# at-cg/PHI

Measured on AMD Instinct MI355X. Metric: read Gbases/s scored (49-hap MHC graph stand-in synMHC-49); reads resident in HBM, parsing and H2D excluded, higher is better.
Workload: dtype u64

## Files before the change

include/phi_amd.h:

```cpp
#ifndef PHI_AMD_H
#define PHI_AMD_H

#include <stddef.h>
#include <stdint.h>

#ifdef __cplusplus
extern "C" {
#endif

typedef struct phi_ctx phi_ctx;

typedef enum {
    PHI_OK = 0,
    PHI_ERR_INVALID = -1,
    PHI_ERR_NOMEM = -2,
    PHI_ERR_DEVICE = -3,
    PHI_ERR_STATE = -4,
    PHI_ERR_UNSUPPORTED = -5,
    PHI_ERR_WALK = -6,
    PHI_ERR_OVERFLOW = -7
} phi_status;

const char *phi_strerror(int status);
const char *phi_last_error(const phi_ctx *ctx);
// ... 144 lines not shown
    int64_t spectrum_size;
    int64_t filtered;
    int64_t retained;
    int64_t n_in_model;
} phi_result;

int phi_set_solve_budget(phi_ctx *ctx, int64_t max_dp_runs);

int phi_solve(phi_ctx *ctx, phi_result *out);

int phi_path_sequence(phi_ctx *ctx, char *buf, int64_t cap);

int phi_sketch(phi_ctx *ctx, const char *bases, const int64_t *seq_off, int64_t n_seq, int32_t k,
               int32_t w, uint64_t *out_hash, int64_t *out_pos, int32_t *out_seq, int64_t cap,
               int64_t *n_out);
typedef struct {
    int64_t n_entries, walk_bases;
    int64_t n_classes, class_bases, n_class_records;
    int64_t n_walk_minimizers, n_distinct_minimizers;
    double sketch_gpu_ms;
} phi_index_info;
int phi_index_stats(phi_ctx *ctx, phi_index_info *out);

typedef struct {
    int64_t n_dp_anchors, n_events;
    int32_t n_steps, n_blocks, dp_mode, max_classes;
    double mean_classes;
} phi_solve_info;
int phi_solve_stats(phi_ctx *ctx, phi_solve_info *out);

int phi_walk_minimizers(phi_ctx *ctx, int32_t walk, uint64_t *out_hash, int64_t *out_pos,
                        int64_t cap, int64_t *n_out);
int phi_walk_sharing(phi_ctx *ctx, int64_t *hist, int32_t cap, int64_t *n_distinct);

int phi_kept_anchors(phi_ctx *ctx, uint64_t *out_hash, int32_t *out_walk, int32_t *out_t0,
                     int32_t *out_t1, int64_t cap, int64_t *n_out);

int phi_host_register(phi_ctx *ctx, void *p, size_t bytes);
int phi_host_unregister(phi_ctx *ctx, void *p);

int phi_prof_enable(phi_ctx *ctx, int on);
int phi_prof_read(phi_ctx *ctx, int64_t *n_launches, double *total_ms, int64_t *total_bases);

typedef struct { const char *text; int64_t n; } phi_walk_text;
int phi_walk_text_upload(phi_ctx *ctx, const phi_walk_text *walks, int32_t n_walks);
int phi_walk_text_resolve(phi_ctx *ctx, const char *prefix, int32_t prefix_n, const int32_t *num2id, int64_t n_num, int32_t n_seg,
                          int64_t *walk_off_out, uint32_t *irregular);
int phi_walk_entries(phi_ctx *ctx, int32_t *out, int64_t cap, int64_t *n);

int phi_device_synchronize(phi_ctx *ctx);

int phi_prefix_sums(phi_ctx *ctx, int32_t kind, const void *d_in, int64_t n, void *d_out);

int phi_edit_distances(phi_ctx *ctx, const char *a, const int64_t *a_off, const char *b, const int64_t *b_off,
                       int64_t n_pairs, int64_t max_distance, int64_t *out);

int phi_edit_alignments(phi_ctx *ctx, const char *a, const int64_t *a_off, const char *b, const int64_t *b_off,
                        int64_t n_pairs, const int64_t *dist, int64_t *counts, char *cigar, const int64_t *cigar_off);


#define PHI_INFLATE_CHUNK_DEFAULT (64 << 10)
#define PHI_INFLATE_NO_FINDER 1
typedef struct {
    int64_t in_bytes;
    int64_t out_bytes;
    int64_t members;
    int64_t chunks;
    int64_t confirmed;
    int64_t redecoded;
    int64_t marker_bytes;
    double device_ms;
    char detail[192];
} phi_inflate_info;
int phi_inflate(int32_t device, const void *in, int64_t n, void *out, int64_t cap, int64_t chunk_bytes, int32_t flags,
                int64_t *out_size, phi_inflate_info *info);
int phi_inflate_alloc(int32_t device, const void *in, int64_t n, int64_t chunk_bytes, int32_t flags, void **out, int64_t *out_size,
                      phi_inflate_info *info);
void phi_inflate_free(void *p);
int phi_text_park_gzip_begin(phi_text_park *park, int64_t piece_bytes);
int phi_text_park_gzip_add(phi_text_park *park, const void *data, int64_t n);
int phi_text_park_gzip_end(phi_text_park *park, int32_t *first, int32_t *count, phi_inflate_info *info);
int phi_gzip_header(const void *data, int64_t n, int64_t pos, int64_t *deflate_start);
uint32_t phi_crc32_combine(uint32_t crc_a, uint32_t crc_b, int64_t len_b);

typedef struct {
    int64_t text_bytes;
    int64_t host_bytes;
    int64_t walk_bytes;
    int32_t n_walks;
    phi_inflate_info inflate;
} phi_gfa_gzip_info;
int phi_gfa_gzip_split(phi_ctx *ctx, const void *gz, int64_t n, int64_t chunk_bytes, char **host_text, int64_t *host_n,
                       phi_gfa_gzip_info *info);
void phi_gfa_gzip_free(char *host_text);

#define PHI_LADDER_MAX_LEVELS 16
typedef struct {
    int32_t n_levels;
    int32_t one_length;
    int64_t n_reads, n_bases;
    int64_t n_kept_reads, n_kept_bases;
    int64_t band_reads[PHI_LADDER_MAX_LEVELS], band_bases[PHI_LADDER_MAX_LEVELS];
    uint64_t threshold[PHI_LADDER_MAX_LEVELS];
    double count_gpu_ms, scan_gpu_ms, scatter_gpu_ms, copy_gpu_ms;
} phi_ladder_info;
int phi_reads_collect_begin(phi_ctx *ctx, int64_t first_ordinal);
// ... 53 lines not shown
```

phi_amd/_capi.py:

```python
import ctypes as C
import os

_HERE = os.path.dirname(os.path.abspath(__file__))
LIB_PATH = os.environ.get("PHI_AMD_LIB") or os.path.join(_HERE, "libphi_amd.so")

PHI_OK = 0
PHI_ERR_INVALID, PHI_ERR_NOMEM, PHI_ERR_DEVICE, PHI_ERR_STATE = -1, -2, -3, -4
PHI_ERR_UNSUPPORTED, PHI_ERR_WALK, PHI_ERR_OVERFLOW = -5, -6, -7
PHI_FLAG_QCLP, PHI_FLAG_MIXED = 1, 2
PHI_COMM_ID_BYTES = 128

SYMBOLS = [
    "phi_strerror", "phi_last_error", "phi_ctx_create", "phi_ctx_destroy", "phi_set_stream", "phi_set_params",
    "phi_set_graph", "phi_add_reads", "phi_add_reads_device", "phi_reset_reads", "phi_reads_stats", "phi_hits_buffer", "phi_read_table",
    "phi_spectrum_export", "phi_spectrum_import", "phi_spectrum_set_size", "phi_solve", "phi_path_sequence",
    "phi_sketch", "phi_walk_minimizers", "phi_walk_sharing", "phi_kept_anchors", "phi_prof_enable", "phi_prof_read",
    "phi_host_register", "phi_host_unregister", "phi_set_solve_budget", "phi_device_synchronize", "phi_walk_text_upload", "phi_walk_text_resolve", "phi_walk_entries",
    "phi_index_stats", "phi_solve_stats", "phi_comm_unique_id", "phi_comm_init", "phi_comm_info", "phi_comm_allreduce_hits", "phi_comm_exchange", "phi_comm_destroy",
    "phi_reads_text_begin", "phi_add_reads_text", "phi_reads_text_end", "phi_reads_text_detach_carry", "phi_reads_text_last_batch",
    "phi_text_park_create", "phi_text_park_pin", "phi_text_park_add", "phi_text_park_add_async", "phi_text_park_wait", "phi_text_park_bytes", "phi_text_park_fetch", "phi_text_park_release", "phi_text_park_destroy",
    "phi_add_reads_text_parked",
    "phi_peers_create", "phi_peers_join", "phi_peers_allreduce_hits", "phi_peers_exchange", "phi_peers_destroy",
    "phi_ipc_unique_id", "phi_ipc_init", "phi_ipc_info", "phi_ipc_allreduce_hits", "phi_ipc_flush", "phi_ipc_exchange", "phi_ipc_check", "phi_ipc_destroy",
    "phi_edit_distances", "phi_edit_alignments",
    "phi_inflate", "phi_inflate_alloc", "phi_inflate_free", "phi_gzip_header", "phi_crc32_combine",
    "phi_text_park_gzip_begin", "phi_text_park_gzip_add", "phi_text_park_gzip_end",
    "phi_gfa_gzip_split", "phi_gfa_gzip_free",
    "phi_set_graph_chopped", "phi_chop_origin", "phi_chop_stats",
    "phi_vcf_genotypes", "phi_vcf_walks", "phi_vcf_stats",
    "phi_reads_collect_begin", "phi_reads_collect_end", "phi_reads_collect_release", "phi_ladder_plan", "phi_ladder_advance", "phi_ladder_band",
    "phi_set_graph_panel", "phi_panel_origin", "phi_panel_walks", "phi_panel_stats", "phi_panel_release",
    "phi_scout_graph", "phi_scout_scores", "phi_scout_choose", "phi_reads_collect_score", "phi_vcf_walks_wide",
    "phi_prefix_sums",
    "phi_reads_bam_begin", "phi_add_reads_bam", "phi_add_reads_bam_parked", "phi_reads_bam_end", "phi_reads_bam_last_batch",
    "phi_calls_path", "phi_calls_walk", "phi_calls_stats",
]
PHI_PANEL_RETAIN = 1
PHI_PANEL_KEEP_READS = 2
PHI_SCOUT_MAX_WALKS = 65535
PHI_LADDER_MAX_LEVELS = 16
PHI_INFLATE_NO_FINDER = 1
PHI_INFLATE_CHUNK_DEFAULT = 64 << 10


class PhiIndexInfo(C.Structure):
    _fields_ = [(n, C.c_int64) for n in ("n_entries", "walk_bases", "n_classes", "class_bases", "n_class_records",
                                         "n_walk_minimizers", "n_distinct_minimizers")] + [("sketch_gpu_ms", C.c_double)]


class PhiSolveInfo(C.Structure):
    _fields_ = [("n_dp_anchors", C.c_int64), ("n_events", C.c_int64), ("n_steps", C.c_int32), ("n_blocks", C.c_int32),
                ("dp_mode", C.c_int32), ("max_classes", C.c_int32), ("mean_classes", C.c_double)]


class PhiChopInfo(C.Structure):
    _fields_ = [("n_vtx_in", C.c_int64), ("n_vtx_out", C.c_int64), ("n_entries_in", C.c_int64), ("n_entries_out", C.c_int64),
                ("max_len", C.c_int32), ("expand_gpu_ms", C.c_double)]


class PhiPanelInfo(C.Structure):
    _fields_ = [("n_walks_in", C.c_int32), ("n_walks_out", C.c_int32), ("n_vtx_in", C.c_int64), ("n_vtx_out", C.c_int64),
                ("n_edges_in", C.c_int64), ("n_edges_out", C.c_int64), ("n_entries_in", C.c_int64), ("n_entries_out", C.c_int64),
                ("mark_gpu_ms", C.c_double), ("scan_gpu_ms", C.c_double), ("remap_gpu_ms", C.c_double),
                ("reduce_host_s", C.c_double), ("kahn_host_s", C.c_double)]


class PhiScoutInfo(C.Structure):
    _fields_ = [("n_blocks", C.c_int32), ("n_walks", C.c_int32), ("n_classes_flagged", C.c_int64), ("n_nonzero", C.c_int64),
                ("record_gpu_ms", C.c_double), ("class_gpu_ms", C.c_double), ("entry_gpu_ms", C.c_double), ("walk_sum_gpu_ms", C.c_double)]


class PhiVcfInfo(C.Structure):
    _fields_ = [("text_bytes", C.c_int64), ("n_records", C.c_int64), ("n_samples", C.c_int32), ("n_flagged", C.c_int64),
                ("n_units", C.c_int64), ("n_entries", C.c_int64), ("genotype_gpu_ms", C.c_double), ("walks_gpu_ms", C.c_double)]


class PhiLadderInfo(C.Structure):
    _fields_ = [("n_levels", C.c_int32), ("one_length", C.c_int32), ("n_reads", C.c_int64), ("n_bases", C.c_int64),
                ("n_kept_reads", C.c_int64), ("n_kept_bases", C.c_int64),
                ("band_reads", C.c_int64 * PHI_LADDER_MAX_LEVELS), ("band_bases", C.c_int64 * PHI_LADDER_MAX_LEVELS),
                ("threshold", C.c_uint64 * PHI_LADDER_MAX_LEVELS),
                ("count_gpu_ms", C.c_double), ("scan_gpu_ms", C.c_double), ("scatter_gpu_ms", C.c_double), ("copy_gpu_ms", C.c_double)]


class PhiBamInfo(C.Structure):
    _fields_ = [(n, C.c_int64) for n in ("n_records", "n_kept", "n_secondary_supplementary", "n_empty", "n_reverse", "n_bases", "header_bytes",
# ... 114 lines not shown
    L.phi_spectrum_set_size.argtypes = [vp, i64]
    L.phi_solve.argtypes = [vp, C.POINTER(PhiResult)]
    L.phi_set_solve_budget.argtypes = [vp, i64]
    L.phi_index_stats.argtypes = [vp, C.POINTER(PhiIndexInfo)]
    L.phi_solve_stats.argtypes = [vp, C.POINTER(PhiSolveInfo)]
    L.phi_comm_unique_id.argtypes = [vp, C.c_size_t]
    L.phi_comm_init.argtypes = [vp, vp, i32, i32]
    L.phi_comm_info.argtypes = [vp, C.POINTER(i32), C.POINTER(i32)]
    L.phi_comm_allreduce_hits.argtypes = [vp]
    L.phi_comm_exchange.argtypes = [vp]
    L.phi_comm_destroy.argtypes = [vp]
    L.phi_peers_create.argtypes = [i32, C.POINTER(vp)]
    L.phi_peers_join.argtypes = [vp, vp, i32]
    L.phi_peers_allreduce_hits.argtypes = [vp]
    L.phi_peers_exchange.argtypes = [vp]
    L.phi_peers_destroy.argtypes = [vp]
    L.phi_ipc_unique_id.argtypes = [vp, C.c_size_t]
    L.phi_ipc_init.argtypes = [vp, C.c_char_p, i32, i32]
    L.phi_ipc_info.argtypes = [vp, C.POINTER(i32), C.POINTER(i32)]
    L.phi_ipc_allreduce_hits.argtypes = [vp]
    L.phi_ipc_exchange.argtypes = [vp]
    L.phi_ipc_flush.argtypes = [vp]
    L.phi_ipc_check.argtypes = [vp]
    L.phi_ipc_destroy.argtypes = [vp]
    L.phi_path_sequence.argtypes = [vp, vp, i64]
    L.phi_sketch.argtypes = [vp, vp, vp, i64, i32, i32, vp, vp, vp, i64, C.POINTER(i64)]
    L.phi_walk_minimizers.argtypes = [vp, i32, vp, vp, i64, C.POINTER(i64)]
    L.phi_walk_sharing.argtypes = [vp, vp, i32, C.POINTER(i64)]
    L.phi_kept_anchors.argtypes = [vp, vp, vp, vp, vp, i64, C.POINTER(i64)]
    L.phi_prof_enable.argtypes = [vp, C.c_int]
    L.phi_host_register.argtypes = [vp, vp, C.c_size_t]
    L.phi_host_unregister.argtypes = [vp, vp]
    L.phi_prof_read.argtypes = [vp, C.POINTER(i64), C.POINTER(C.c_double), C.POINTER(i64)]
    L.phi_device_synchronize.argtypes = [vp]
    L.phi_prefix_sums.argtypes = [vp, i32, vp, i64, vp]
    L.phi_walk_text_upload.argtypes = [vp, vp, i32]
    L.phi_walk_text_resolve.argtypes = [vp, C.c_char_p, i32, vp, i64, i32, vp, C.POINTER(C.c_uint32)]
    L.phi_walk_entries.argtypes = [vp, vp, i64, C.POINTER(i64)]
    L.phi_edit_distances.argtypes = [vp, vp, vp, vp, vp, i64, i64, vp]
    L.phi_edit_alignments.argtypes = [vp, vp, vp, vp, vp, i64, vp, vp, vp, vp]
    L.phi_inflate.argtypes = [i32, vp, i64, vp, i64, i64, i32, C.POINTER(i64), C.POINTER(PhiInflateInfo)]
    L.phi_inflate_alloc.argtypes = [i32, vp, i64, i64, i32, C.POINTER(vp), C.POINTER(i64), C.POINTER(PhiInflateInfo)]
    L.phi_inflate_free.argtypes = [vp]
    L.phi_inflate_free.restype = None
    L.phi_text_park_gzip_begin.argtypes = [vp, i64]
    L.phi_text_park_gzip_add.argtypes = [vp, vp, i64]
    L.phi_text_park_gzip_end.argtypes = [vp, C.POINTER(i32), C.POINTER(i32), C.POINTER(PhiInflateInfo)]
    L.phi_gzip_header.argtypes = [vp, i64, i64, C.POINTER(i64)]
    L.phi_crc32_combine.argtypes = [C.c_uint32, C.c_uint32, i64]
    L.phi_crc32_combine.restype = C.c_uint32
    L.phi_gfa_gzip_split.argtypes = [vp, vp, i64, i64, C.POINTER(vp), C.POINTER(i64), C.POINTER(PhiGfaGzipInfo)]
    L.phi_gfa_gzip_free.argtypes = [vp]
    L.phi_gfa_gzip_free.restype = None
    for name in SYMBOLS:
        f = getattr(L, name)
        if f.restype is C.c_int and name not in ("phi_strerror", "phi_last_error", "phi_ctx_destroy", "phi_crc32_combine", "phi_inflate_free", "phi_gfa_gzip_free"):
            f.restype = C.c_int
    _lib = L
    return L
```

phi_amd/context.py:

```python
import ctypes as C
from typing import NamedTuple

import numpy as np

from . import _capi


class PhiError(RuntimeError):
    def __init__(self, status, detail):
        self.status = status
        self.detail = detail
        super().__init__(f"{_capi.load().phi_strerror(status).decode()} ({status}): {detail}")


def _ptr(a):
    return a.ctypes.data if a is not None and a.size else None


class Alignments(NamedTuple):
    distance: np.ndarray
    counts: np.ndarray
    cigar: list
    identity: np.ndarray

# ... 587 lines not shown
        self._chk(self._L.phi_walk_minimizers(self._h, walk, None, None, 0, C.byref(n)))
        h = np.zeros(n.value, np.uint64)
        p = np.zeros(n.value, np.int64)
        if n.value:
            self._chk(self._L.phi_walk_minimizers(self._h, walk, _ptr(h), _ptr(p), n.value, C.byref(n)))
        return h, p

    def walk_sharing(self, n_walks):
        hist = np.zeros(n_walks + 1, np.int64)
        n = C.c_int64()
        self._chk(self._L.phi_walk_sharing(self._h, _ptr(hist), n_walks + 1, C.byref(n)))
        return hist, n.value

    def kept_anchors(self):
        n = C.c_int64()
        self._chk(self._L.phi_kept_anchors(self._h, None, None, None, None, 0, C.byref(n)))
        h = np.zeros(n.value, np.uint64)
        wk = np.zeros(n.value, np.int32)
        t0 = np.zeros(n.value, np.int32)
        t1 = np.zeros(n.value, np.int32)
        if n.value:
            self._chk(self._L.phi_kept_anchors(self._h, _ptr(h), _ptr(wk), _ptr(t0), _ptr(t1), n.value, C.byref(n)))
        return h, wk, t0, t1

    def walk_entries(self):
        n = C.c_int64()
        self._chk(self._L.phi_walk_entries(self._h, None, 0, C.byref(n)))
        out = np.zeros(n.value, np.int32)
        if n.value:
            self._chk(self._L.phi_walk_entries(self._h, _ptr(out), n.value, C.byref(n)))
        return out

    def gfa_gzip_split(self, data, chunk_bytes=0):
        p, n, info = self._gfa_gzip_split_raw(data, chunk_bytes)
        try:
            return C.string_at(p, n) if n else b"", info
        finally:
            self._L.phi_gfa_gzip_free(p)

    def _gfa_gzip_split_raw(self, data, chunk_bytes=0):
        buf = np.frombuffer(data, np.uint8) if not isinstance(data, np.ndarray) else data
        p, n, info = C.c_void_p(), C.c_int64(), _capi.PhiGfaGzipInfo()
        self._chk(self._L.phi_gfa_gzip_split(self._h, _ptr(buf), len(buf), chunk_bytes, C.byref(p), C.byref(n), C.byref(info)))
        d = {k: getattr(info, k) for k in ("text_bytes", "host_bytes", "walk_bytes", "n_walks")}
        d["inflate"] = _info(info.inflate)
        return p, n.value, d

    def device_synchronize(self):
        self._chk(self._L.phi_device_synchronize(self._h))

    def prefix_sums(self, kind, d_in, n, d_out):
        self._chk(self._L.phi_prefix_sums(self._h, kind, C.c_void_p(d_in), n, C.c_void_p(d_out)))

    def prof_enable(self, on=True):
        self._chk(self._L.phi_prof_enable(self._h, int(on)))

    def prof_read(self):
        n, ms, b = C.c_int64(), C.c_double(), C.c_int64()
        self._chk(self._L.phi_prof_read(self._h, C.byref(n), C.byref(ms), C.byref(b)))
        return n.value, ms.value, b.value


def _parse_reads_tail(text):
    lines = [ln.rstrip(b"\r") for ln in text.split(b"\n")]
    while lines and not lines[-1]:
        lines.pop()
    if not lines:
        return []
    if lines[0][:1] == b"@":
        if len(lines) % 4:
            raise ValueError("the reads text ends inside a FASTQ record")
        return lines[1::4]
    if lines[0][:1] != b">":
        raise ValueError("the reads text is neither FASTA nor FASTQ")
    seqs = []
    for ln in lines:
        if ln[:1] == b">":
            seqs.append([])
        else:
            seqs[-1].append(ln)
    return [b"".join(s) for s in seqs]


def _info(info):
    return {n: getattr(info, n) for n, _ in _capi.PhiInflateInfo._fields_ if n != "detail"}


def inflate(data, device=0, chunk_bytes=0, finder=True, as_array=False):
    L = _capi.load()
    buf = np.frombuffer(data, np.uint8) if not isinstance(data, np.ndarray) else data
    flags = 0 if finder else _capi.PHI_INFLATE_NO_FINDER
    p, size, info = C.c_void_p(), C.c_int64(), _capi.PhiInflateInfo()
    rc = L.phi_inflate_alloc(device, _ptr(buf), len(buf), chunk_bytes, flags, C.byref(p), C.byref(size), C.byref(info))
    if rc:
        raise PhiError(rc, info.detail.decode())
    try:
        out = np.empty(size.value, np.uint8)
        if size.value:
            C.memmove(out.ctypes.data, p, size.value)
    finally:
        L.phi_inflate_free(p)
    return (out if as_array else out.tobytes()), _info(info)


def gzip_header(data, pos=0):
    L = _capi.load()
# ... 70 lines not shown
```

phi_amd/csrc/anchors.hip:

```cpp
#include <hip/hip_runtime.h>
#include "phi_dev.h"
#include "phi_kernels.h"
#include "phi_wave.h"

static inline unsigned grid_for(int64_t n, int tpb)
{
    int64_t nb = (n + tpb - 1) / tpb;
    if (nb > 256 * 16) nb = 256 * 16;
    if (nb < 1) nb = 1;
    return (unsigned)nb;
}

#define GRID_STRIDE(i, n) \
    for (int64_t i = (int64_t)blockIdx.x * blockDim.x + threadIdx.x; i < (n); i += (int64_t)gridDim.x * blockDim.x)

__global__ void __launch_bounds__(256) phi_walk_edges_kernel(const int32_t *__restrict__ walk_vtx, const int64_t *__restrict__ walk_off,
                                                             int32_t n_walks, int64_t n_entries, int32_t n_vtx, const int64_t *__restrict__ adj_off,
                                                             const int32_t *__restrict__ adj, const int64_t *__restrict__ seq_off,
                                                             const int32_t *__restrict__ topo_rank, uint8_t *__restrict__ e_out,
                                                             int32_t *__restrict__ cnt_edge, unsigned long long *__restrict__ st_mask,
                                                             int32_t nw64, int32_t *__restrict__ err)
{
    GRID_STRIDE(e, n_entries) {
        int32_t lo = 0, hi = n_walks;
// ... 111 lines not shown
    if (a1 - a0 != b1 - b0) return false;
    for (uint32_t d = 0; d <= a1 - a0; d++)
        if (A.walk_vtx[a0 + d] != A.walk_vtx[b0 + d]) return false;
    return true;
}

__global__ void __launch_bounds__(256) phi_group_insert_kernel(PhiFilterArgs A, int64_t n_matched)
{
    GRID_STRIDE(j, n_matched) {
        const int32_t r = A.m_rec[j];
        const uint64_t key = group_key(A.rec_slot[r], A.walk_vtx, A.rec_e0[r], A.rec_e1[r], A.seed);
        uint64_t gs = key & A.g_mask;
        int probes = 0;
        for (;;) {
            const unsigned long long prev = atomicCAS((unsigned long long *)&A.g_keys[gs], PHI_EMPTY_KEY, key);
            if (prev == PHI_EMPTY_KEY || prev == key) break;
            gs = (gs + 1) & A.g_mask;
            if (++probes > PHI_MAX_PROBE) { atomicOr(A.err, PHI_KERR_TABLE_FULL); break; }
        }
        atomicMin((uint32_t *)&A.g_rep[gs], (uint32_t)r);
        A.m_group[j] = (int32_t)gs;
    }
}

__global__ void __launch_bounds__(256) phi_group_count_kernel(PhiFilterArgs A, int64_t n_matched)
{
    GRID_STRIDE(j, n_matched) {
        const int32_t r = A.m_rec[j];
        const int32_t gs = A.m_group[j];
        if (!same_group(A, r, A.g_rep[gs])) { atomicOr(A.err, PHI_KERR_FP_COLLISION); continue; }
        atomicAdd(&A.g_cnt[gs], (uint32_t)A.cls_mult[A.rec_cls[r]]);
    }
}

__global__ void __launch_bounds__(256) phi_group_max_kernel(PhiFilterArgs A, int64_t n_matched)
{
    GRID_STRIDE(j, n_matched) {
        const int32_t r = A.m_rec[j];
        const uint32_t id = A.u_uid[A.rec_slot[r]];
        atomicMax(&A.slot_maxcnt[id], A.g_cnt[A.m_group[j]]);
        if (A.rec_e1[r] > A.rec_e0[r]) A.slot_multi[id] = 1;
    }
}

__global__ void __launch_bounds__(256) phi_slot_count_kernel(PhiFilterArgs A, int64_t n_ids)
{
    int n_filtered = 0, n_model = 0;
    GRID_STRIDE(s, n_ids) {
        const uint32_t c = A.slot_maxcnt[s];
        if (c == 0) continue;
        if ((float)c >= A.limit) n_filtered++;
        else if (A.slot_multi[s]) n_model++;
    }
    n_filtered = phi_wave_sum(n_filtered);
    n_model = phi_wave_sum(n_model);
    if ((threadIdx.x & 63) == 0) {
        if (n_filtered) atomicAdd(&A.counters[0], (unsigned long long)n_filtered);
        if (n_model) atomicAdd(&A.counters[1], (unsigned long long)n_model);
    }
}

__global__ void __launch_bounds__(256) phi_kept_flags_kernel(PhiFilterArgs A, int64_t n_matched,
                                                             uint8_t *__restrict__ kept, uint8_t *__restrict__ dp)
{
    GRID_STRIDE(j, n_matched) {
        const int32_t r = A.m_rec[j];
        const bool keep = !((float)A.slot_maxcnt[A.u_uid[A.rec_slot[r]]] >= A.limit);
        kept[j] = keep;
        dp[j] = keep && A.rec_e1[r] > A.rec_e0[r];
    }
}

void phi_launch_group_insert(hipStream_t st, const PhiFilterArgs &A, int64_t n)
{
    if (n > 0) hipLaunchKernelGGL(phi_group_insert_kernel, dim3(grid_for(n, 256)), dim3(256), 0, st, A, n);
}
void phi_launch_group_count(hipStream_t st, const PhiFilterArgs &A, int64_t n)
{
    if (n > 0) hipLaunchKernelGGL(phi_group_count_kernel, dim3(grid_for(n, 256)), dim3(256), 0, st, A, n);
}
void phi_launch_group_max(hipStream_t st, const PhiFilterArgs &A, int64_t n)
{
    if (n > 0) hipLaunchKernelGGL(phi_group_max_kernel, dim3(grid_for(n, 256)), dim3(256), 0, st, A, n);
}
void phi_launch_slot_count(hipStream_t st, const PhiFilterArgs &A, int64_t u_cap)
{
    if (u_cap > 0) hipLaunchKernelGGL(phi_slot_count_kernel, dim3(grid_for(u_cap, 256)), dim3(256), 0, st, A, u_cap);
}
void phi_launch_kept_flags(hipStream_t st, const PhiFilterArgs &A, int64_t n, uint8_t *kept, uint8_t *dp)
{
    if (n > 0) hipLaunchKernelGGL(phi_kept_flags_kernel, dim3(grid_for(n, 256)), dim3(256), 0, st, A, n, kept, dp);
}

__global__ void phi_gather_i32_kernel(const int32_t *__restrict__ src, const uint32_t *__restrict__ idx, int64_t n,
                                      int32_t *__restrict__ out)
{
    GRID_STRIDE(j, n) out[j] = src[idx[j]];
}
void phi_launch_gather_i32(hipStream_t st, const int32_t *src, const uint32_t *idx, int64_t n, int32_t *out)
{
    if (n > 0) hipLaunchKernelGGL(phi_gather_i32_kernel, dim3(grid_for(n, 256)), dim3(256), 0, st, src, idx, n, out);
}

__global__ void phi_gather_u64_kernel(const uint64_t *__restrict__ src, const int32_t *__restrict__ idx, int64_t n,
                                      uint64_t *__restrict__ out)
{
    GRID_STRIDE(j, n) out[j] = src[idx[j]];
}
void phi_launch_gather_u64(hipStream_t st, const uint64_t *src, const int32_t *idx, int64_t n, uint64_t *out)
{
    if (n > 0) hipLaunchKernelGGL(phi_gather_u64_kernel, dim3(grid_for(n, 256)), dim3(256), 0, st, src, idx, n, out);
}

__global__ void phi_entry_csr_kernel(const phi_ent_t *__restrict__ a_e1, int64_t n_a, int64_t n_entries,
                                     int64_t *__restrict__ g_off)
{
    GRID_STRIDE(j, n_a + 1) {
        const int64_t lo = j == 0 ? 0 : (int64_t)a_e1[j - 1] + 1;
        const int64_t hi = j == n_a ? n_entries : (int64_t)a_e1[j];
        for (int64_t e = lo; e <= hi; e++) g_off[e] = j;
    }
}
void phi_launch_entry_csr(hipStream_t st, const phi_ent_t *a_e1, int64_t n_a, int64_t n_entries, int64_t *g_off)
{
    hipLaunchKernelGGL(phi_entry_csr_kernel, dim3(grid_for(n_a + 1, 256)), dim3(256), 0, st, a_e1, n_a, n_entries,
                       g_off);
}

__global__ void phi_warm_anchors_kernel() {}
void phi_warm_anchors(hipStream_t st) { hipLaunchKernelGGL(phi_warm_anchors_kernel, dim3(1), dim3(64), 0, st); }
```

phi_amd/csrc/dp_events.hip:

```cpp
#include <hip/hip_runtime.h>
#include <type_traits>
#include "phi_kernels.h"

#define NEG (-(1 << 28))
#define NEGK (-(1 << 30))
#define CHK PHI_DP_CHUNK
#define RING PHI_DP_RING
enum { DP_SEQ = 0, DP_ROW = 1, DP_PATH = 2 };

__global__ void __launch_bounds__(256) phi_event_flags_kernel(const int32_t *__restrict__ walk_vtx, int64_t n_entries,
                                                              const int32_t *__restrict__ cvtx, uint8_t *__restrict__ flags)
{
    for (int64_t e = (int64_t)blockIdx.x * blockDim.x + threadIdx.x; e < n_entries; e += (int64_t)gridDim.x * blockDim.x)
        flags[e] = cvtx[walk_vtx[e]] >= 0;
}

__global__ void phi_event_off_kernel(const phi_ent_t *__restrict__ ev_e, int64_t n_ev, const int64_t *__restrict__ walk_off,
                                     int32_t n_walks, int64_t *__restrict__ ev_off)
{
    const int h = blockIdx.x * blockDim.x + threadIdx.x;
    if (h > n_walks) return;
    const int64_t key = walk_off[h];
    int64_t lo = 0, hi = n_ev;
    while (lo < hi) {
// ... 491 lines not shown
            }
        }
        int32_t wl = min(ve, vb + D);
        int32_t vprev = vb;
        __syncthreads();
        for (int p = 0;; p++) {
            const int32_t vi = has_walk ? s_vi[p & 1][h] : 0;
            if (MODE != DP_ROW) {
#pragma unroll
                for (int n = 0; n < P / NPW; n++) {
                    const int32_t x = vprev + pw + n * NPW;
                    if (x < vi) {
                        const int4 r = s_res[x & (D - 1)][h];
                        A.dmax[(phi_ent_t)r.z] = r.x; A.bstart[(phi_ent_t)r.z] = r.y;
                    }
                }
                if (pw == 0 && p > 0 && h < P) {
                    const int32_t r = (p - 1) * P + h;
                    if (r < n_steps) {
                        const int32_t k = k0 + r;
                        reinterpret_cast<int4 *>(A.tops)[k] = s_top[k & (RINGT - 1)];
                        const int2 en = s_ent[r & (2 * P - 1)];
                        A.ent_src[k] = en.x; A.ent_h[k] = en.y;
                    }
                }
            }
            if (p == n_per) break;
            const int32_t hi = min(ve, vi + D);
            uint4 t0[P / NPW], t1[P / NPW], t2[P / NPW];
#pragma unroll
            for (int n = 0; n < P / NPW; n++) {
                const int64_t xc = (ve > v0) ? min(wl + pw + n * NPW, ve - 1) : 0;
                t0[n] = evg[xc * 3 + 0]; t1[n] = evg[xc * 3 + 1]; t2[n] = evg[xc * 3 + 2];
            }
#pragma unroll
            for (int n = 0; n < P / NPW; n++) {
                const int32_t x = wl + pw + n * NPW;
                if (x < hi) { s_ev[x & (D - 1)][0][h] = t0[n]; s_ev[x & (D - 1)][1][h] = t1[n]; s_ev[x & (D - 1)][2][h] = t2[n]; }
            }
            wl = max(wl, min(hi, wl + P));
            if (p % PER_CHUNK == 0 && (p / PER_CHUNK + 1) * CK < n_steps) stage(p / PER_CHUNK + 1);
            vprev = vi;
            __syncthreads();
        }
        return;
    }

    int32_t vi = vb;
    s_vi[0][h] = vi;
    __syncthreads();
    uint4 cA = make_uint4(0xFFFFFFFFu, 0, 0, 0);
    if (vi < ve) cA = s_ev[vi & (D - 1)][0][h];
    int32_t qh = 0, qn = 0, hs = 0, hE = 0, tk = 0;
    int32_t M = NEGK, sL = MODE == DP_SEQ ? 0 : -1, Emax = NEG;
    if (MODE == DP_ROW && h == row_j) M = 0;
    if (MODE == DP_PATH && has_walk) M = A.blk_S[(int64_t)sb * A.lane_stride + h];
    const bool starts_on = MODE != DP_ROW || start_row;
    int32_t endbest = NEG;
    int32_t Kn = NEGK;
    int4 ra = s_rec[0][0], rb = s_rec[0][1];
    int4 lastq = make_int4(NEG, NEG, 0, 0);
    int32_t lastk = -1;

    auto eval_entry = [&](const int4 xa, const int4 xb, int32_t k, int32_t &E, int32_t &Eh, int32_t &Esrc) {
        E = NEG; Eh = -1; Esrc = -1;
        const int32_t flags = xa.x;
        const int n_in = (flags >> 8) & 0xFF;
        auto consider = [&](const int4 q, int32_t oj, int32_t src) {
            const int32_t t1h = (q.z & 0x3FF) - 1, t1n = ((q.z >> 10) & 0x3FF) - 1, t2h = ((q.z >> 20) & 0x3FF) - 1;
            const bool cont = t1n == oj;
            const int32_t val = cont ? q.y : q.x, hh = cont ? t2h : t1h;
            if (hh < 0) return;
            if (val > E || (val == E && (hh < Eh || (hh == Eh && src < Esrc)))) { E = val; Eh = hh; Esrc = src; }
        };
        const uint32_t b0 = (uint32_t)xa.z >> 8, b1 = (uint32_t)xa.w >> 8, b2 = (uint32_t)xb.x >> 8;
        if (n_in == 1 && b0 < RINGT) {
            const int32_t src = k - (int32_t)b0;
            const int4 q = src == lastk ? lastq : s_top[src & (RINGT - 1)];
            const int32_t t1h = (q.z & 0x3FF) - 1, t1n = ((q.z >> 10) & 0x3FF) - 1, t2h = ((q.z >> 20) & 0x3FF) - 1;
            const bool cont = t1n == (xa.z & 0xFF);
            const int32_t hh = cont ? t2h : t1h;
            if (hh >= 0) { E = cont ? q.y : q.x; Eh = hh; Esrc = k - (int32_t)b0; }
        } else if (n_in <= 3 && (b0 | b1 | b2) < RINGT) {
            const int4 q0 = s_top[(k - b0) & (RINGT - 1)];
            const int4 q1 = s_top[(k - b1) & (RINGT - 1)];
            const int4 q2 = s_top[(k - b2) & (RINGT - 1)];
            consider(q0, xa.z & 0xFF, k - (int32_t)b0);
            if (n_in > 1) consider(q1, xa.w & 0xFF, k - (int32_t)b1);
            if (n_in > 2) consider(q2, xb.x & 0xFF, k - (int32_t)b2);
        } else {
            for (int j = 0; j < n_in; j++) {
                const int32_t pk = j == 0 ? xa.z : j == 1 ? xa.w : j == 2 ? xb.x : A.k_in_packed[xa.y + j - 3];
                const int32_t back = (int32_t)((uint32_t)pk >> 8);
                const int32_t src = k - back;
                const int4 q = (back < RINGT || MODE == DP_ROW) ? s_top[src & (RINGT - 1)] : reinterpret_cast<const int4 *>(A.tops)[src];
                consider(q, pk & 0xFF, src);
            }
        }
        if (Eh >= 0) E -= A.cost;
        if (h == 0) s_ent[(k - k0) & (2 * P - 1)] = make_int2(Esrc, Eh);
    };

    for (int p = 0; p < n_per; p++) {
        const int32_t r_end = min(n_steps, (p + 1) * P);
        if (vi < ve) cA = s_ev[vi & (D - 1)][0][h];
        for (int32_t r = p * P; r < r_end;) {
            const int32_t k = k0 + r;
            const int4 na = s_rec[(r + 1) & (2 * CK - 1)][0], nb = s_rec[(r + 1) & (2 * CK - 1)][1];
            const int4 n2a = s_rec[(r + 2) & (2 * CK - 1)][0], n2b = s_rec[(r + 2) & (2 * CK - 1)][1];
            const bool pair = (ra.x & PHI_DP_PAIR) && r + 1 < r_end;
            const int32_t stepk = (int32_t)(cA.x & 0x7FFFFFFFu);
            const bool second = pair && stepk == k + 1;
            const bool active = stepk == k || second;
            const int32_t flags = second ? na.x : ra.x;

            int32_t E = NEG, Eh = -1, Esrc = -1;
            if (ra.x & PHI_DP_NEED_ENTRY) eval_entry(ra, rb, k, E, Eh, Esrc);
            if (pair && (na.x & PHI_DP_NEED_ENTRY)) {
                int32_t E1, Eh1, Esrc1;
                eval_entry(na, nb, k + 1, E1, Eh1, Esrc1);
                if (second) { E = E1; Eh = Eh1; Esrc = Esrc1; }
            } else if (second) { E = NEG; Eh = -1; }

            int32_t dmax = NEG;
            int32_t oidx = 255;
            if (active) {
                const int sl = (int)(vi & (D - 1));
                const phi_ent_t e = cA.y;
                const bool ovf = (cA.x >> 31) != 0;
                const int32_t t = (int32_t)(e - eb);
                const int32_t End = (int32_t)cA.z, SB = (int32_t)cA.w;
                const uint8_t *gb = reinterpret_cast<const uint8_t *>(&s_ev[sl][1][h]);
                oidx = gb[15 + 1024];
                while (qn > 0 && t - hs >= 31) {
                    const int32_t key = qn == 1 ? tk : s_qK[qh & (QD - 1)][h];
                    if (key > M) { M = key; sL = hs; }
                    qh++; qn--;
                    if (qn > 0) { hs = s_qs[qh & (QD - 1)][h]; hE = s_qE[qh & (QD - 1)][h]; }
                }
                int32_t newE = NEG;
                if (t == 0) { newE = starts_on ? 0 : NEG; qn = 0; M = NEGK; Emax = NEG; }
                else if ((flags & PHI_DP_NEED_ENTRY) && Eh >= 0) newE = E;
                if (newE > Emax) {
                    Emax = newE;
                    const int32_t key = newE - SB;
                    while (qn > 0 && tk < key) {
                        qn--;
                        if (qn > 0) tk = s_qK[(qh + qn - 1) & (QD - 1)][h];
                    }
                    if (QD < 32 && qn == QD) { atomicOr(A.err, PHI_KERR_DP_QUEUE); qn--; }
                    const int slq = (qh + qn) & (QD - 1);
                    s_qs[slq][h] = t; s_qE[slq][h] = newE; s_qK[slq][h] = key;
                    if (qn == 0) { hs = t; hE = newE; }
                    tk = key;
                    qn++;
                    if (MODE == DP_ROW && key > Kn) Kn = key;
                }
                int32_t bs = 0;
                if ((flags & PHI_DP_NEED_TOPS) || e == e_last) {
                    int32_t best = M > NEGK / 2 ? M + End : NEG;
                    bs = sL;
                    for (int32_t j = 0; j < qn; j++) {
                        const int32_t s = j == 0 ? hs : s_qs[(qh + j) & (QD - 1)][h];
                        const int32_t Es = j == 0 ? hE : s_qE[(qh + j) & (QD - 1)][h];
                        const int a = t - s;
                        const int32_t inside = !ovf ? (int32_t)gb[(a & 15) + (a >> 4) * 1024] : ev_count_inside(A, (int64_t)eb + s, e);
                        const int32_t val = Es + inside;
                        if (val > best) { best = val; bs = s; }
                    }
                    if (best > NEG / 2) dmax = best; else bs = 0;
                    if (MODE == DP_ROW && e == e_last) endbest = max(endbest, dmax);
                }
                s_res[sl][h] = make_int4(dmax, bs, (int32_t)e, 0);
                vi++;
                cA = make_uint4(0xFFFFFFFFu, 0, 0, 0);
                if (vi < ve) cA = s_ev[vi & (D - 1)][0][h];
            }

            if (!pair && (ra.x & PHI_DP_NEED_TOPS)) {
                const bool leaving = active && oidx != 255 && dmax > NEG / 2;
                int32_t t1v = NEG, t1h = -1, t1n = -1, t2v = NEG, t2h = -1;
                if (__ballot(leaving && oidx > 1) == 0ull) {
                    const bool on0 = leaving && oidx == 0, on1 = leaving && oidx == 1;
                    unsigned long long K0, K1;
                    ev_wave_max2_key(on0 ? ev_key(dmax, h) : 0ull, on1 ? ev_key(dmax, h) : 0ull, K0, K1);
                    const bool first0 = K0 >= K1;
                    const unsigned long long Kf = first0 ? K0 : K1, Ks = first0 ? K1 : K0;
                    t1v = Kf ? (int32_t)(uint32_t)(Kf >> 8) + NEG : NEG;
                    t1h = Kf ? 255 - (int32_t)(Kf & 255) : -1;
                    t1n = Kf ? (first0 ? 0 : 1) : -1;
                    t2v = Ks ? (int32_t)(uint32_t)(Ks >> 8) + NEG : NEG;
                    t2h = Ks ? 255 - (int32_t)(Ks & 255) : -1;
                } else {
                    const int32_t m1 = ev_wave_max_i32(leaving ? dmax : NEG);
                    if (m1 > NEG / 2) {
                        const int l1 = __ffsll((long long)__ballot(leaving && dmax == m1)) - 1;
                        t1v = m1; t1h = l1;
                        t1n = __builtin_amdgcn_readlane(oidx, l1);
                        const bool other = leaving && oidx != t1n;
                        const int32_t m2 = ev_wave_max_i32(other ? dmax : NEG);
                        if (m2 > NEG / 2) { t2v = m2; t2h = __ffsll((long long)__ballot(other && dmax == m2)) - 1; }
                    }
                }
// ... 318 lines not shown
                if (d > NEGK / 2 && d - dx > best) best = d - dx;
                if (with_starts[u]) { const int32_t r = s_start[p][lx]; if (r > NEGK / 2 && r - dx > best) best = r - dx; }
            }
            S[u] = best > NEGK / 2 ? best : NEGK;
        }
    };
    if (x < 64) {
#pragma unroll
        for (int u = 0; u < U; u++) { s_b1[b_lo & 1][u][x] = NONE; s_b2[b_lo & 1][u][x] = NONE; s_n1[b_lo & 1][u][x] = 0; }
    }
    using I0 = std::integral_constant<int, 0>; using I1 = std::integral_constant<int, 1>;
    using I2 = std::integral_constant<int, 2>; using I3 = std::integral_constant<int, 3>;
    issue(I0{}, min(b_lo, nb - 1));
    issue(I1{}, min(b_lo + 1, nb - 1));
    issue(I2{}, min(b_lo + 2, nb - 1));
    issue(I3{}, min(b_lo + 3, nb - 1));
    __syncthreads();
    int32_t b = b_lo;
    for (; b + DEPTH <= nb; b += DEPTH) {
        step(I0{}, b);
        step(I1{}, b + 1);
        step(I2{}, b + 2);
        step(I3{}, b + 3);
    }
    if (b < nb) step(I0{}, b);
    if (b + 1 < nb) step(I1{}, b + 1);
    if (b + 2 < nb) step(I2{}, b + 2);
    if (MODE == 1 && has_walk) {
#pragma unroll
        for (int u = 0; u < U; u++)
            if (unit0 + u <= G.n_walks) seg_row[((int64_t)seg * (G.n_walks + 1) + unit0 + u) * LS + x] = S[u];
    }
}

__global__ void __launch_bounds__(256) phi_seg_chain_kernel(int32_t n_seg, int32_t n_walks, int32_t LS, const int32_t *__restrict__ seg_row,
                                                            int32_t *__restrict__ seg_S)
{
    __shared__ int32_t s_S[256];
    const int x = threadIdx.x;
    int32_t S = NEGK;
    for (int32_t g = 0; g < n_seg; g++) {
        seg_S[(int64_t)g * LS + x] = S;
        s_S[x] = S;
        __syncthreads();
        const int32_t *R = seg_row + (int64_t)g * (n_walks + 1) * LS + x;
        int32_t best = R[(int64_t)n_walks * LS];
#pragma unroll 8
        for (int32_t u = 0; u < n_walks; u++) best = max(best, s_S[u] + R[(int64_t)u * LS]);
        S = best > NEGK / 2 ? best : NEGK;
        __syncthreads();
    }
}

__global__ void __launch_bounds__(256) phi_blk_check_kernel(const int32_t *__restrict__ keys, const int32_t *__restrict__ S, int32_t n_blk,
                                                            int32_t LS, int32_t n_walks, int32_t *__restrict__ bad)
{
    const int64_t n = (int64_t)(n_blk - 1) * LS;
    for (int64_t i = (int64_t)blockIdx.x * blockDim.x + threadIdx.x; i < n; i += (int64_t)gridDim.x * blockDim.x) {
        const int32_t h = (int32_t)(i % LS);
        if (h >= n_walks) continue;
        const int32_t got = keys[i], want = S[i + LS];
        if (got != want && !(got <= NEGK / 2 && want <= NEGK / 2)) { atomicAdd(&bad[0], 1); atomicMin(&bad[1], (int32_t)(i / LS)); }
    }
}

__global__ void __launch_bounds__(256) phi_carry_resolve_kernel(const int32_t *__restrict__ carry, int32_t LS, int32_t b_from, int32_t h,
                                                                int32_t *__restrict__ out)
{
    __shared__ int32_t s_best;
    for (int32_t hi = b_from - 1; hi >= 0; hi -= 256) {
        if (threadIdx.x == 0) s_best = -1;
        __syncthreads();
        const int32_t b = hi - (int32_t)threadIdx.x;
        const int32_t v = b >= 0 ? carry[(int64_t)b * LS + h] : -1;
        if (v >= 0) atomicMax(&s_best, b);
        __syncthreads();
        const int32_t bb = s_best;
        if (bb >= 0) {
            if (b == bb) { out[0] = bb; out[1] = v; }
            return;
        }
        __syncthreads();
    }
    if (threadIdx.x == 0) { out[0] = -1; out[1] = -1; }
}

void phi_launch_blk_classes(hipStream_t st, const PhiBlkClassArgs &G)
{
    if (G.n_blk > 0) hipLaunchKernelGGL(phi_blk_classes_kernel, dim3((unsigned)G.n_blk), dim3(256), 0, st, G);
}
void phi_launch_blk_chain(hipStream_t st, const PhiBlkClassArgs &G, const int32_t *rows, const int32_t *rownew, const int32_t *rowdiag, int32_t *blk_S)
{
    hipLaunchKernelGGL(phi_blk_chain_kernel<0>, dim3(1), dim3(256), 0, st, G, rows, rownew, rowdiag, blk_S, nullptr, nullptr, nullptr);
}
void phi_launch_blk_chain_segments(hipStream_t st, const PhiBlkClassArgs &G, const int32_t *rows, const int32_t *rownew, const int32_t *rowdiag, int32_t *blk_S,
                                   int32_t n_seg, const int32_t *d_seg_lo, int32_t *seg_row, int32_t *seg_S)
{
    const int units = getenv("PHI_DP_CHAIN_UNITS") ? atoi(getenv("PHI_DP_CHAIN_UNITS")) : 3;
    const unsigned nu = (unsigned)(G.n_walks + 1);
    if (units >= 4) hipLaunchKernelGGL((phi_blk_chain_kernel<1, 4>), dim3((unsigned)n_seg * ((nu + 3) / 4)), dim3(256), 0, st, G, rows, rownew, rowdiag, blk_S, d_seg_lo, seg_row, seg_S);
    else if (units == 3) hipLaunchKernelGGL((phi_blk_chain_kernel<1, 3>), dim3((unsigned)n_seg * ((nu + 2) / 3)), dim3(256), 0, st, G, rows, rownew, rowdiag, blk_S, d_seg_lo, seg_row, seg_S);
    else if (units == 2) hipLaunchKernelGGL((phi_blk_chain_kernel<1, 2>), dim3((unsigned)n_seg * ((nu + 1) / 2)), dim3(256), 0, st, G, rows, rownew, rowdiag, blk_S, d_seg_lo, seg_row, seg_S);
    else hipLaunchKernelGGL((phi_blk_chain_kernel<1, 1>), dim3((unsigned)n_seg * nu), dim3(256), 0, st, G, rows, rownew, rowdiag, blk_S, d_seg_lo, seg_row, seg_S);
    hipLaunchKernelGGL(phi_seg_chain_kernel, dim3(1), dim3(256), 0, st, n_seg, G.n_walks, G.lane_stride, seg_row, seg_S);
    hipLaunchKernelGGL(phi_blk_chain_kernel<2>, dim3((unsigned)n_seg), dim3(256), 0, st, G, rows, rownew, rowdiag, blk_S, d_seg_lo, seg_row, seg_S);
}
void phi_launch_blk_check(hipStream_t st, const int32_t *keys, const int32_t *S, int32_t n_blk, int32_t LS, int32_t n_walks, int32_t *bad)
{
    int64_t nb = ((int64_t)(n_blk - 1) * LS + 255) / 256;
    if (nb < 1) nb = 1;
    if (nb > 2048) nb = 2048;
    hipLaunchKernelGGL(phi_blk_check_kernel, dim3((unsigned)nb), dim3(256), 0, st, keys, S, n_blk, LS, n_walks, bad);
}
void phi_launch_carry_resolve(hipStream_t st, const int32_t *carry, int32_t LS, int32_t b_from, int32_t h, int32_t *out)
{
    hipLaunchKernelGGL(phi_carry_resolve_kernel, dim3(1), dim3(256), 0, st, carry, LS, b_from, h, out);
}
void phi_launch_dp_block_paths_wide(hipStream_t st, const PhiDpEventArgs &A)
{
    if (A.n_walks <= 128) hipLaunchKernelGGL((phi_dp_events_kernel<2, DP_PATH>), dim3((unsigned)A.n_blk), dim3(128), 0, st, A);
    else hipLaunchKernelGGL((phi_dp_events_kernel<4, DP_PATH>), dim3((unsigned)A.n_blk), dim3(256), 0, st, A);
}

void phi_launch_dp_events(hipStream_t st, const PhiDpEventArgs &A)
{
    if (A.n_walks <= 64) hipLaunchKernelGGL((phi_dp_events_pc_kernel<2, DP_SEQ, 8, RING, 32>), dim3(1), dim3(64 * 3), 0, st, A);
    else if (A.n_walks <= 128) hipLaunchKernelGGL((phi_dp_events_kernel<2, DP_SEQ>), dim3(1), dim3(128), 0, st, A);
    else hipLaunchKernelGGL((phi_dp_events_kernel<4, DP_SEQ>), dim3(1), dim3(256), 0, st, A);
}

void phi_launch_dp_block_rows(hipStream_t st, const PhiDpEventArgs &A)
{
    const unsigned grid = (unsigned)A.n_blk * (A.lane_walk ? 65u : (unsigned)(A.n_walks + 1));
    if (A.blk_ring <= 256 && A.blk_max_len > 0 && A.blk_max_len <= 64 && !getenv("PHI_DP_ROWS_LARGE"))
        hipLaunchKernelGGL((phi_dp_events_pc_kernel<2, DP_ROW, 2, 64, 8, 32>), dim3(grid), dim3(64 * 3), 0, st, A);
    else if (A.blk_ring <= 256) hipLaunchKernelGGL((phi_dp_events_pc_kernel<2, DP_ROW, 2, 256, 8>), dim3(grid), dim3(64 * 3), 0, st, A);
    else if (A.blk_ring <= 1024) hipLaunchKernelGGL((phi_dp_events_pc_kernel<2, DP_ROW, 4, 1024, 16>), dim3(grid), dim3(64 * 3), 0, st, A);
    else hipLaunchKernelGGL((phi_dp_events_pc_kernel<2, DP_ROW, 4, 2048, 16>), dim3(grid), dim3(64 * 3), 0, st, A);
}
void phi_launch_dp_block_paths(hipStream_t st, const PhiDpEventArgs &A)
{
    if (A.blk_ring <= 256) hipLaunchKernelGGL((phi_dp_events_pc_kernel<2, DP_PATH, 4, 256, 8>), dim3((unsigned)A.n_blk), dim3(64 * 3), 0, st, A);
    else if (A.blk_ring <= 1024) hipLaunchKernelGGL((phi_dp_events_pc_kernel<2, DP_PATH, 4, 1024, 16>), dim3((unsigned)A.n_blk), dim3(64 * 3), 0, st, A);
    else hipLaunchKernelGGL((phi_dp_events_pc_kernel<2, DP_PATH, 4, 2048, 16>), dim3((unsigned)A.n_blk), dim3(64 * 3), 0, st, A);
}

__global__ void phi_warm_dp_events_kernel() {}
void phi_warm_dp_events(hipStream_t st) { hipLaunchKernelGGL(phi_warm_dp_events_kernel, dim3(1), dim3(64), 0, st); }
```

phi_amd/csrc/phi_abi.hip:

```cpp
#include <stdarg.h>
#include <stdio.h>
#include <string.h>
#include <algorithm>
#include <future>
#include "phi_ctx.h"
#include "phi_dev.h"

int phi_fail(phi_ctx *c, int code, const char *fmt, ...)
{
    char buf[512];
    va_list ap;
    va_start(ap, fmt);
    vsnprintf(buf, sizeof buf, fmt, ap);
    va_end(ap);
    if (c) {
        std::lock_guard<std::mutex> g(c->err_mu);
        c->last_error = buf;
    }
    return code;
}

int phi_hip_check(phi_ctx *c, hipError_t e, const char *what)
{
    if (e == hipSuccess) return PHI_OK;
// ... 55 lines not shown
        if (aux.valid()) (void)aux.get();
        if (c->own_stream) (void)hipStreamDestroy(c->own_stream);
        if (c->aux_stream) (void)hipStreamDestroy(c->aux_stream);
        phi_dev_free(c->d_scalars); phi_dev_free(c->d_stripes); phi_dev_free(c->alt.stripes);
        delete c;
        return code;
    };
    if (hipStreamCreateWithFlags(&c->own_stream, hipStreamNonBlocking) != hipSuccess) return bail(PHI_ERR_DEVICE);
    c->stream = c->own_stream;
    tm.lap("stream");
    if (phi_dev_ensure(c, c->d_scalars, S_N * 8) || hipMemsetAsync(c->d_scalars.p, 0, S_N * 8, c->stream) != hipSuccess ||
        phi_dev_ensure(c, c->d_stripes, 2 * STRIPE_BYTES) || hipMemsetAsync(c->d_stripes.p, 0, 2 * STRIPE_BYTES, c->stream) != hipSuccess ||
        phi_dev_ensure(c, c->alt.stripes, 2 * STRIPE_BYTES) || hipMemsetAsync(c->alt.stripes.p, 0, 2 * STRIPE_BYTES, c->stream) != hipSuccess)
        return bail(PHI_ERR_DEVICE);
    if (tm.on && getenv("PHI_TIMING_UNITS")) {
        (void)hipStreamSynchronize(c->stream); tm.lap("  scalars");
        phi_warm_sketch(c->stream); (void)hipStreamSynchronize(c->stream); tm.lap("  code object: sketch");
        phi_warm_table(c->stream); (void)hipStreamSynchronize(c->stream); tm.lap("  code object: table");
        phi_warm_anchors(c->stream); (void)hipStreamSynchronize(c->stream); tm.lap("  code object: anchors");
        phi_warm_contexts(c->stream); (void)hipStreamSynchronize(c->stream); tm.lap("  code object: contexts");
        phi_warm_dp(c->stream); (void)hipStreamSynchronize(c->stream); tm.lap("  code object: dp");
        phi_warm_dp_events(c->stream); (void)hipStreamSynchronize(c->stream); tm.lap("  code object: dp_events");
        phi_warm_solve_dev(c->stream); (void)hipStreamSynchronize(c->stream); tm.lap("  code object: solve_dev");
        phi_warm_reads_text(c->stream); (void)hipStreamSynchronize(c->stream); tm.lap("  code object: reads_text");
        phi_warm_scan(c->stream); (void)hipStreamSynchronize(c->stream); tm.lap("  code object: scan");
    }
    phi_warm_sketch(c->stream); phi_warm_table(c->stream); phi_warm_anchors(c->stream); phi_warm_contexts(c->stream);
    phi_warm_dp(c->stream); phi_warm_dp_events(c->stream); phi_warm_solve_dev(c->stream); phi_warm_reads_text(c->stream);
    phi_warm_walk_text(c->stream); phi_warm_scan(c->stream);
    if (hipStreamSynchronize(c->stream) != hipSuccess) return bail(PHI_ERR_DEVICE);
    tm.lap("scalars + code objects");
    if (aux.get() != hipSuccess) { c->aux_stream = nullptr; return bail(PHI_ERR_DEVICE); }
    c->last_error.clear();
    tm.lap("wait for the second stream + first host copies");
    *out = c;
    return PHI_OK;
}

void phi_ctx_destroy(phi_ctx *c)
{
    if (c && c->pin_future.valid()) c->pin_future.wait();
    if (c && c->dp_alloc_future.valid()) (void)c->dp_alloc_future.get();
    if (c && c->h_pin) { (void)hipSetDevice(c->device); (void)hipHostFree(c->h_pin); c->h_pin = nullptr; }
    if (c) { (void)hipSetDevice(c->device); stage_release(c); }
    if (!c) return;
    (void)phi_comm_destroy(c);
    (void)phi_ipc_destroy(c);
    (void)hipSetDevice(c->device);
    (void)hipStreamSynchronize(c->stream);
    phi_ladder_drop(c);
    DevBuf *all[] = {&c->d_anchors, &c->d_cov_all, &c->d_cov_w, &c->d_slots, &c->d_slots2, &c->d_segs, &c->d_ctr, &c->d_vmax, &c->d_lane_walk, &c->d_walk_lane, &c->d_coff, &c->d_blk_ncls, &c->d_rownew, &c->d_blk_bad, &c->d_seg_lo, &c->d_seg_row, &c->d_seg_S, &c->wtext.d_text, &c->panel.d_full, &c->scout.d_scores, &c->d_sel_off, &c->d_sel_tri, &c->d_blk_lo, &c->d_blk_ev, &c->d_blk_S, &c->d_row_out, &c->d_rowend, &c->d_blk_keys, &c->d_blk_carry, &c->d_cov, &c->d_cov2, &c->d_stepdiff, &c->alt.hit, &c->hit_extra[0], &c->hit_extra[1], &c->alt.stripes, &c->spset.d_sp_cnt, &c->rlog.d_novlog, &c->rlog.d_novcnt, &c->rlog.d_ovlist, &c->d_vlen, &c->d_ent_cls, &c->d_cls_rep, &c->d_cls_left, &c->d_cls_mult, &c->d_cls_base, &c->d_cls_rec_off, &c->d_rec_cls, &c->d_rec_rel, &c->d_u_replist, &c->d_adj_off, &c->d_adj, &c->d_topo_rank, &c->d_cnt_edge, &c->d_walk_err, &c->d_sa_cnt, &c->d_sa_cur, &c->d_sa_off, &c->d_sa_idx, &c->d_seq, &c->d_seq_off, &c->d_walk_vtx, &c->d_walk_off, &c->d_topo, &c->d_in_off,
                     &c->d_in_src, &c->d_e_out, &c->d_st_rec, &c->d_st_mask, &c->d_in_packed, &c->d_word, &c->d_wwords, &c->d_wbad,
                     &c->d_wascii, &c->d_wstarts, &c->d_rec_hash, &c->d_rec_pos, &c->d_rec_slot,
                     &c->d_rec_e0, &c->d_rec_e1, &c->d_u_keys, &c->d_u_rep, &c->d_u_uid, &c->d_rt, &c->d_kt, &c->d_in_s, &c->d_last_walk, &c->d_rowdiag, &c->d_wpre, &c->d_hit, &c->spset.d_sp_keys, &c->d_rbases,
                     &c->d_roff, &c->rlog.d_roff_made, &c->d_peer_send, &c->spset.d_export, &c->d_scalars, &c->d_stripes, &c->d_blk_cnt,
                     &c->d_blk_off, &c->d_flags, &c->d_flags2, &c->d_list, &c->d_list2, &c->d_list3, &c->d_walk_last, &c->d_m_rec, &c->d_m_group,
                     &c->d_g_keys, &c->d_g_rep, &c->d_g_cnt, &c->d_slot_maxcnt, &c->d_slot_multi, &c->d_a_e1,
                     &c->d_g_off, &c->d_g_span, &c->d_a_weight, &c->d_dmax, &c->d_bstart, &c->d_k_rec, &c->d_k_in, &c->d_cvtx, &c->d_ev_e, &c->d_ev_off, &c->d_ev,
                     &c->d_off_end, &c->d_off_start, &c->d_scan_blk, &c->d_scan_blk64, &c->d_scan_blkoff, &c->d_top,
                     &c->d_ent};
    phi_pool_flush(c->device);
    phi_pool_bypass(true);
    struct Bypass { ~Bypass() { phi_pool_bypass(false); } } bypass_guard;
    for (DevBuf *b : all) phi_dev_free(*b);
    for (auto &pr : c->prof_events) { (void)hipEventDestroy(pr.first); (void)hipEventDestroy(pr.second); }
    if (c->h_err) (void)hipHostFree(c->h_err);
    {
        auto &T = c->text;
        for (int i = 0; i < 2; i++) { phi_dev_free(T.text[i]); phi_dev_free(T.bases[i]); phi_dev_free(T.roff[i]); }
        phi_dev_free(T.tile_cnt); phi_dev_free(T.ls); phi_dev_free(T.pre); phi_dev_free(T.blk); phi_dev_free(T.sum);
        if (T.h_sum) (void)hipHostFree(T.h_sum);
        if (T.ev_copy) (void)hipEventDestroy(T.ev_copy);
    }
    phi_bam_drop(c);
    (void)hipStreamDestroy(c->own_stream);
    (void)hipStreamDestroy(c->aux_stream);
    delete c;
}

int phi_set_stream(phi_ctx *c, void *hip_stream)
{
    if (!c) return PHI_ERR_INVALID;
    HIPCHK(hipStreamSynchronize(c->stream));
    c->stream = hip_stream ? (hipStream_t)hip_stream : c->own_stream;
    return PHI_OK;
}

int phi_set_params(phi_ctx *c, int32_t k, int32_t w, float threshold, int32_t recombination, uint32_t flags)
{
    if (!c) return PHI_ERR_INVALID;
    if (c->have_graph) return phi_fail(c, PHI_ERR_STATE, "phi_set_params must precede phi_set_graph");
    if (k < 1 || k > PHI_MAX_K) return phi_fail(c, PHI_ERR_INVALID, "k=%d outside [1,%d]", k, PHI_MAX_K);
    if (w < 1 || w > PHI_MAX_W) return phi_fail(c, PHI_ERR_INVALID, "w=%d outside [1,%d]", w, PHI_MAX_W);
    if (recombination < 0) return phi_fail(c, PHI_ERR_INVALID, "recombination penalty must be >= 0");
    c->k = k; c->w = w; c->threshold = threshold; c->recombination = recombination; c->flags = flags;
    return PHI_OK;
}

}

int sketch_records(phi_ctx *c, const uint64_t *words, const unsigned long long *starts, int64_t n_bases,
                   int32_t k, int32_t w, const uint8_t *ascii_if_bad, DevBuf &out_hash, DevBuf &out_pos,
                   int64_t *n_out)
{
    *n_out = 0;
    const int64_t nb = phi_sketch_num_blocks(n_bases);
    if (nb == 0) return PHI_OK;
// ... 310 lines not shown
```

phi_amd/csrc/phi_ctx.h:

```cpp
#pragma once
#include <stdint.h>
#include <stdarg.h>
#include <stdio.h>
#include <stdlib.h>
#include <algorithm>
#include <atomic>
#include <chrono>
#include <future>
#include <mutex>
#include <string>
#include <thread>
#include <vector>
#include <hip/hip_runtime.h>
#include "../../include/phi_amd.h"
#include "phi_kernels.h"
#include "phi_host_par.h"
#include "solve_host.h"
#include "reads_host.h"

struct DevBuf {
    void *p = nullptr;
    size_t cap = 0;
    uint32_t gen = 0;
    template <class T> T *as() const { return reinterpret_cast<T *>(p); }
// ... 51 lines not shown
    struct PhiWalkText {
        bool ready = false;
        int32_t n_walks = 0;
        std::vector<int64_t> tile0, t_len;
        std::vector<int32_t> ends;
        DevBuf d_text;
    } wtext;
    bool walks_on_device = false;
    int64_t walks_on_device_n = 0;
    struct PhiChop {
        bool on = false;
        std::vector<int32_t> first;
        phi_chop_info info{};
    } chop;
    struct PhiPanel {
        bool on = false;
        std::vector<int32_t> origin;
        std::vector<int32_t> kept;
        phi_panel_info info{};
        DevBuf d_full;
        std::vector<int64_t> full_off;
    } panel;
    struct PhiScout {
        bool on = false;
        DevBuf d_scores;
        int32_t n_blocks = 0;
    } scout;
    struct PhiVcf {
        bool have = false;
        phi_vcf_info info{};
    } vcf;

    DevBuf d_seq, d_seq_off, d_walk_vtx, d_walk_off, d_topo, d_in_off, d_in_src;
    DevBuf d_e_out, d_st_rec, d_st_mask, d_in_packed;
    int dp_nw = 1;
    DevBuf d_wwords, d_wstarts, d_wbad, d_wascii;
    DevBuf d_vlen;
    DevBuf d_ent_cls;
    DevBuf d_cls_rep, d_cls_left, d_cls_mult, d_cls_base, d_cls_rec_off;
    int64_t n_cls = 0, cls_bases = 0;
    double index_gpu_ms = 0.0;
    DevBuf d_rec_hash, d_rec_pos, d_rec_cls, d_rec_rel, d_rec_slot, d_rec_e0, d_rec_e1;
    int64_t n_rec = 0;
    DevBuf d_u_keys, d_u_rep, d_u_uid, d_u_replist;
    DevBuf d_rt;
    uint64_t rt_buckets = 0, rt_mask = 0;
    DevBuf d_kt;
    uint64_t kt_buckets = 0, kt_mask = 0;
    int64_t kt_max_chunks = 0;
    void *h_stage[2] = {nullptr, nullptr};
    hipEvent_t stage_ev[2] = {nullptr, nullptr};
    DevBuf d_wpre;
    DevBuf d_rowdiag;
    DevBuf d_in_s, d_last_walk;
    int64_t n_unique = 0;
    uint64_t u_cap = 0;
    DevBuf d_hit;
    DevBuf hit_extra[PHI_HIT_RING - 2];
    int hit_n = 2, hit_idx = 0;

    struct PhiSpectrumSet {
        DevBuf d_sp_keys;
        uint64_t sp_cap = 0;
        DevBuf d_sp_cnt;
        DevBuf d_export;
        int64_t sp_set_gen = -1;
        int64_t sp_gen = 0;
        void new_generation() { sp_gen++; }
        void new_graph() { sp_set_gen = -1; }
    } spset;
    struct PhiReadLog {
        DevBuf d_novlog, d_novcnt;
        int32_t nov_shift = 6;
        int64_t log_chunks = 0, log_done = 0;
        int64_t logged_done = 0;
        int64_t last_log_chunks = 0;
        DevBuf d_ovlist;
        int64_t ov_cap = 0, ov_done = 0, ov_bound = 0;
        bool async_batches = false;
        bool next_flag_zeroed = false;
        DevBuf d_roff_made;
        void flushed() { log_chunks = log_done = 0; ov_done = 0; ov_bound = 0; }
        void new_generation() { flushed(); logged_done = 0; last_log_chunks = 0; next_flag_zeroed = false; }
    } rlog;
    int64_t reads_bases = 0, reads_count = 0;
    int64_t spectrum_override = -1;
    DevBuf d_rbases, d_roff, d_peer_send;
    DevBuf d_scalars;
    DevBuf d_stripes;
    struct PhiReadBufs {
        DevBuf hit, stripes;
        bool needs_clean = false;
    } alt;

    uint32_t *h_err = nullptr;
    struct PhiTextStream {
        bool active = false, irregular = false, started = false, detached = false;
        bool carry_stale = false;
        int mode = 0;
        int64_t fed = 0, taken = 0;
        uint32_t carry_cap = 0, chunk_cap = 0, line_cap = 0;
        DevBuf text[2], bases[2], roff[2], tile_cnt, ls, pre, blk, sum;
        int slot = 0;
        uint32_t carry_len = 0, carry_at = 0;
        std::vector<char> h_carry;
        PhiTextSummary *h_sum = nullptr;
        hipEvent_t ev_copy = nullptr;
// ... 198 lines not shown
```

phi_amd/csrc/phi_kernels.h:

```cpp
#pragma once
#include <stdint.h>
#include <hip/hip_runtime.h>
#include "phi_dp_flags.h"

#ifndef PHI_TPB
#define PHI_TPB 256

#endif
#define PHI_WCH 512
#define PHI_MAX_W 256
#define PHI_MAX_K 64
#define PHI_MAX_K_PACKED 32
#define PHI_MAX_PROBE 4096
#define PHI_RT_OVERFLOWED 1u
static inline int phi_nov_shift(int w)
{
    const int want = (3 * 2 * PHI_WCH) / (2 * (w + 1));
    int sh = 4;
    while ((1 << sh) < want && sh < 9) sh++;
    return sh;
}
#define PHI_STRIPES 256

typedef uint32_t phi_ent_t;
// ... 176 lines not shown
#define PHI_DP_RING 2048
#define PHI_SCOUT_MAX_WALKS 65535
#define PHI_DP_MAX_WALKS 1022

struct PhiDpArgs {
    int32_t n_vtx, n_walks;
    const int32_t *st_rec;
    const unsigned long long *st_mask;
    const int32_t *in_packed;
    const int64_t *walk_off;
    const uint64_t *word;
    const int64_t *g_off; const uint8_t *g_span; const uint8_t *a_weight;
    int32_t cost;
    int32_t *dmax;
    int32_t *bstart;
    int32_t *tops;
    int32_t *ent_src, *ent_h;
};
void phi_launch_dp(hipStream_t st, const PhiDpArgs &A);

#define PHI_DP_EVENT_MAX_WALKS 256
#define PHI_DP_EVENT_SAFE_WALKS 128
struct PhiDpEventArgs {
    int32_t n_k, n_walks;
    int64_t n_ev;
    const int32_t *k_rec;
    const int32_t *k_in_packed;
    const int64_t *walk_off;
    const phi_ent_t *ev_e;
    const int64_t *ev_off;
    void *ev;
    const int64_t *g_off; const uint8_t *g_span; const uint8_t *a_weight;
    int32_t cost;
    int32_t *dmax, *bstart;
    int32_t *tops;
    int32_t *ent_src, *ent_h;
    uint32_t *err;
    int32_t q_limit;
    int32_t n_blk, blk_ring;
    int32_t blk_max_len;
    int32_t lane_stride;
    const int32_t *lane_walk;
    int32_t *rownew_out;
    int32_t *rowdiag_out;
    const int32_t *blk_lo;
    const int32_t *blk_ev;
    const int32_t *blk_S;
    int32_t *row_out; int32_t *rowend_out;
    int32_t *blk_keys_out; int32_t *blk_carry;
};
void phi_launch_dp_events(hipStream_t st, const PhiDpEventArgs &A);
void phi_launch_dp_block_rows(hipStream_t st, const PhiDpEventArgs &A);
void phi_launch_dp_block_paths(hipStream_t st, const PhiDpEventArgs &A);
void phi_launch_anchor_prep(hipStream_t st, const uint32_t *tri, int64_t n, const int64_t *walk_off, int32_t n_walks, phi_ent_t *a_e1, uint8_t *a_span,
                            unsigned long long *walk_cnt, unsigned long long *out);
void phi_launch_vertex_most(hipStream_t st, const int64_t *g_off, int64_t n_entries, const int32_t *walk_vtx, int32_t *vmax);
void phi_launch_sum_i32(hipStream_t st, const int32_t *v, int64_t n, unsigned long long *out);
void phi_launch_repeat_walk(hipStream_t st, const uint32_t *tri, int64_t lo, int64_t hi, int32_t walk, int32_t *last, uint8_t *flags);
void phi_launch_weights(hipStream_t st, const uint32_t *tri, int64_t n, const uint8_t *in_s, uint8_t *wgt);
void phi_launch_path_cover(hipStream_t st, bool clear, const phi_ent_t *segs, int32_t n_seg, const int64_t *g_off, const uint32_t *tri, const uint8_t *wgt,
                           int32_t *cov_all, int32_t *cov_w, unsigned long long *ctr, uint32_t *twice, int64_t twice_cap);
void phi_launch_uncovered_slots(hipStream_t st, const uint32_t *slots, int64_t n, const int32_t *cov_all, unsigned long long *ctr, uint32_t *out);
struct PhiBlkClassArgs {
    int32_t n_blk, n_walks, lane_stride;
    const int32_t *blk_lo, *blk_ev;
    const int64_t *ev_off, *walk_off;
    const void *ev;
    int32_t *lane_walk;
    int32_t *walk_lane;
    int32_t *coff;
    int32_t *blk_ncls;
    uint32_t *err;
};
void phi_launch_blk_classes(hipStream_t st, const PhiBlkClassArgs &G);
void phi_launch_blk_chain(hipStream_t st, const PhiBlkClassArgs &G, const int32_t *rows, const int32_t *rownew, const int32_t *rowdiag, int32_t *blk_S);
void phi_launch_blk_chain_segments(hipStream_t st, const PhiBlkClassArgs &G, const int32_t *rows, const int32_t *rownew, const int32_t *rowdiag, int32_t *blk_S,
                                   int32_t n_seg, const int32_t *d_seg_lo, int32_t *seg_row, int32_t *seg_S);
void phi_launch_blk_check(hipStream_t st, const int32_t *keys, const int32_t *S, int32_t n_blk, int32_t LS, int32_t n_walks, int32_t *bad);
void phi_launch_carry_resolve(hipStream_t st, const int32_t *carry, int32_t LS, int32_t b_from, int32_t h, int32_t *out);
void phi_launch_dp_block_paths_wide(hipStream_t st, const PhiDpEventArgs &A);
void phi_launch_cut_cov(hipStream_t st, const phi_ent_t *a_e1, const uint8_t *a_span, int64_t n_a, int32_t *diff);
void phi_launch_cut_clean(hipStream_t st, const int32_t *cov_excl, int64_t n_entries, int32_t *clean);
void phi_launch_cut_clean_direct(hipStream_t st, const int64_t *g_off, const uint8_t *g_span, int64_t n_entries, int32_t *clean);
void phi_launch_cut_events(hipStream_t st, const phi_ent_t *ev_e, int64_t n_ev, const int64_t *ev_off, const int64_t *walk_off, int32_t n_walks,
                           const int32_t *walk_vtx, const int32_t *cvtx, const int32_t *ncl_excl, int32_t *stepdiff);
void phi_launch_blk_ev(hipStream_t st, const int32_t *blk_lo, int32_t n_blk, const phi_ent_t *ev_e, const int64_t *ev_off, int32_t n_walks,
                       const int32_t *walk_vtx, const int32_t *cvtx, int32_t *blk_ev);
void phi_launch_event_flags(hipStream_t st, const int32_t *walk_vtx, int64_t n_entries, const int32_t *cvtx, uint8_t *flags);
void phi_launch_event_off(hipStream_t st, const phi_ent_t *ev_e, int64_t n_ev, const int64_t *walk_off, int32_t n_walks,
                          int64_t *ev_off);
void phi_launch_dp_event_fill(hipStream_t st, const PhiDpEventArgs &A, const uint8_t *e_out, const int32_t *walk_vtx,
                              const int32_t *cvtx, const phi_ent_t *a_e1, const int32_t *wpre, int64_t n_entries);
int phi_dp_num_waves(int n_walks);
void phi_launch_dp_words(hipStream_t st, const uint8_t *e_out, const int64_t *g_off, const uint8_t *g_span,
                         const uint8_t *a_weight, int64_t n_entries, uint64_t *word);

#define PHI_TEXT_IRREGULAR_CR 1u
#define PHI_TEXT_IRREGULAR_LINES 2u
#define PHI_TEXT_IRREGULAR_LAYOUT 4u
struct PhiTextSummary {
    uint32_t n_nl;
    uint32_t n_rec;
    uint32_t err;
    uint32_t first_bad;
    uint64_t n_bases;
    uint32_t cons_end;
    uint32_t n_cons_lines;
    uint32_t not_uniform;
    uint32_t pad_;
};
struct PhiTextArgs {
// ... 40 lines not shown
```

phi_amd/csrc/phi_solve.hip:

```cpp
#include <stdio.h>
#include <string.h>
#include <algorithm>
#include <map>
#include <set>
#include <unordered_map>
#include "phi_ctx.h"
#include "phi_dev.h"

static bool have_host_walks(const phi_ctx *c) { return (int64_t)c->h_walk_vtx.size() == c->n_entries; }
static int walk_vtx_at(phi_ctx *c, int64_t e, int32_t *v)
{
    if (have_host_walks(c)) { *v = c->h_walk_vtx[(size_t)e]; return PHI_OK; }
    return phi_hip_check(c, phi_copy_sync(c, v, c->d_walk_vtx.as<int32_t>() + e, 4, hipMemcpyDeviceToHost), "walk entry D2H");
}
static int walk_vtx_range(phi_ctx *c, int64_t es, int64_t n, int32_t *dst)
{
    if (have_host_walks(c)) { memcpy(dst, c->h_walk_vtx.data() + es, (size_t)n * 4); return PHI_OK; }
    return phi_hip_check(c, phi_copy_sync(c, dst, c->d_walk_vtx.as<int32_t>() + es, (size_t)n * 4, hipMemcpyDeviceToHost), "walk entries D2H");
}
static int ensure_host_walks(phi_ctx *c)
{
    if (have_host_walks(c)) return PHI_OK;
    if (!c->h_walk_vtx.resize((size_t)c->n_entries)) return phi_fail(c, PHI_ERR_NOMEM, "host allocation failed");
    return phi_hip_check(c, phi_copy_sync(c, c->h_walk_vtx.data(), c->d_walk_vtx.p, (size_t)c->n_entries * 4, hipMemcpyDeviceToHost), "walk entries D2H");
// ... 40 lines not shown
    }
    PHICHK(phi_scan(c, d_a, ne + 1, d_b));
    phi_launch_cut_events(c->stream, c->d_ev_e.as<phi_ent_t>(), c->n_ev, c->d_ev_off.as<int64_t>(), c->d_walk_off.as<int64_t>(), c->n_walks,
                          c->d_walk_vtx.as<int32_t>(), c->d_cvtx.as<int32_t>(), d_b, c->d_stepdiff.as<int32_t>());
    std::vector<int32_t> closed((size_t)nk + 2);
    HIPCHK(hipMemcpyAsync(closed.data(), c->d_stepdiff.p, (size_t)(nk + 2) * 4, hipMemcpyDeviceToHost, c->stream));
    HIPCHK(hipStreamSynchronize(c->stream));
    for (int32_t k = 1; k <= nk + 1; k++) closed[(size_t)k] += closed[(size_t)k - 1];
    const PhiCutFlags cut_ok{c->h_k_cut_ok.data(), closed.data(), nk};
    if (getenv("PHI_TIMING")) {
        int64_t n_struct = 0, n_both = 0, longest = 0, run = 0, longest_s = 0, run_s = 0;
        for (int32_t k = 1; k < nk; k++) {
            n_struct += c->h_k_cut_ok[(size_t)k] != 0;
            if (cut_ok(k)) { n_both++; run = 0; } else longest = std::max(longest, ++run);
            if (c->h_k_cut_ok[(size_t)k]) run_s = 0; else longest_s = std::max(longest_s, ++run_s);
        }
        fprintf(stderr, "[phi timing] solve: cuts: %lld of %d steps allowed by the graph (longest closed stretch %lld), %lld also clean of anchors (longest closed stretch %lld)\n",
                (long long)n_struct, nk, (long long)longest_s, (long long)n_both, (long long)longest);
    }
    const int32_t rings_walk[] = {256, 1024, 2048}, rings_cls[] = {256, 512};
    static_assert(PHI_DP_BLOCK_MAX == 2048, "the largest ring of tops");
    const int32_t ring = phi_place_blocks(cut_ok, cls ? rings_cls : rings_walk, cls ? 2 : 3, c->blk_no_small, [&](int32_t ring_) {
        int64_t target = (int64_t)nk * (c->n_walks + 1) / 4096;
        target = std::max<int64_t>(64, std::min<int64_t>(ring_ / 2, target));
        if (cls) target = c->blk_cls_target;
        if (const char *e = getenv("PHI_DP_BLOCK_STEPS")) target = std::max(1, std::min(ring_, atoi(e)));
        return target;
    }, c->h_blk_lo);
    if (!ring) return PHI_OK;
    c->blk_ring = ring;
    c->n_blk = (int32_t)c->h_blk_lo.size() - 1;
    if (c->n_blk < 2) { c->n_blk = 0; return PHI_OK; }
    c->blk_max_len = 0;
    for (int32_t b = 0; b < c->n_blk; b++) c->blk_max_len = std::max(c->blk_max_len, c->h_blk_lo[(size_t)b + 1] - c->h_blk_lo[(size_t)b]);
    const size_t nbk = (size_t)c->n_blk, ls = (size_t)c->blk_ls, nrow = cls ? 65 : (size_t)(c->n_walks + 1);
    PHICHK(phi_dev_ensure(c, c->d_blk_lo, (nbk + 1) * 4));
    PHICHK(phi_dev_ensure(c, c->d_blk_ev, nbk * ls * 4));
    PHICHK(phi_dev_ensure(c, c->d_blk_S, nbk * ls * 4));
    PHICHK(phi_dev_ensure(c, c->d_blk_keys, nbk * ls * 4));
    PHICHK(phi_dev_ensure(c, c->d_blk_carry, nbk * ls * 4));
    {
        const uint32_t before = c->d_row_out.gen;
        PHICHK(phi_dev_ensure(c, c->d_row_out, nbk * nrow * 64 * 4));
        if (c->d_row_out.gen != before) HIPCHK(hipMemsetAsync(c->d_row_out.p, 0xC0, c->d_row_out.cap, c->stream));
    }
    PHICHK(phi_dev_ensure(c, c->d_rowend, nbk * nrow * 4));
    if (cls) {
        PHICHK(phi_dev_ensure(c, c->d_lane_walk, nbk * 64 * 4));
        PHICHK(phi_dev_ensure(c, c->d_walk_lane, nbk * ls * 4));
        PHICHK(phi_dev_ensure(c, c->d_coff, nbk * ls * 4));
        PHICHK(phi_dev_ensure(c, c->d_blk_ncls, nbk * 4));
        PHICHK(phi_dev_ensure(c, c->d_rownew, nbk * nrow * 4));
        PHICHK(phi_dev_ensure(c, c->d_rowdiag, nbk * 64 * 4));
        PHICHK(phi_dev_ensure(c, c->d_blk_bad, 64));
    }
    HIPCHK(hipMemcpyAsync(c->d_blk_lo.p, c->h_blk_lo.data(), (nbk + 1) * 4, hipMemcpyHostToDevice, c->stream));
    phi_launch_blk_ev(c->stream, c->d_blk_lo.as<int32_t>(), c->n_blk, c->d_ev_e.as<phi_ent_t>(), c->d_ev_off.as<int64_t>(), c->n_walks,
                      c->d_walk_vtx.as<int32_t>(), c->d_cvtx.as<int32_t>(), c->d_blk_ev.as<int32_t>());
    HIPCHK(hipStreamSynchronize(c->stream));
    c->dp_blocks = true;
    c->dp_cls = cls;
    if (getenv("PHI_TIMING")) fprintf(stderr, "[phi timing] solve: %d compact steps in %d blocks (rings of %d steps)%s\n", nk, c->n_blk, c->blk_ring, cls ? ", rows on class lanes" : "");
    return PHI_OK;
}

struct DpHost {
    std::vector<int32_t> ends, bstart, ent_u, ent_h;
    std::vector<int32_t> rows, rowend, S, keys, carry;
};

struct DpOut {
    int32_t n_ent;
    int32_t *dmax, *bstart, *ent_src, *ent_h;
};
static DpOut dp_out(const phi_ctx *c)
{
    const int32_t n_ent = c->dp_events ? c->n_k : c->n_vtx;
    return DpOut{n_ent, c->d_dmax.as<int32_t>(), c->d_bstart.as<int32_t>(), c->d_ent.as<int32_t>(), c->d_ent.as<int32_t>() + n_ent};
}

enum DpRetry {
    DP_DONE = 0,
    DP_HALVE_CLASS_TARGET,
    DP_NO_SMALL_BLOCKS,
    DP_GIVE_UP_BLOCKS,
    DP_DENSE
};

static int dp_event_records(phi_ctx *c, const DpOut &O, PhiDpEventArgs &A, PhiStageTimer &tr)
{
    const int64_t n_dp = c->n_dp;
    PHICHK(phi_dev_ensure(c, c->d_wpre, (size_t)(n_dp + 1) * 4));
    PHICHK(phi_scan(c, c->d_a_weight.as<uint8_t>(), n_dp, c->d_wpre.as<int32_t>()));
    A.n_k = c->n_k; A.n_walks = c->n_walks; A.n_ev = c->n_ev;
    A.k_rec = c->d_k_rec.as<int32_t>(); A.k_in_packed = c->d_k_in.as<int32_t>();
    A.walk_off = c->d_walk_off.as<int64_t>();
    A.ev_e = c->d_ev_e.as<phi_ent_t>(); A.ev_off = c->d_ev_off.as<int64_t>();
    A.ev = c->d_ev.p;
    A.g_off = c->d_g_off.as<int64_t>(); A.g_span = c->d_g_span.as<uint8_t>(); A.a_weight = c->d_a_weight.as<uint8_t>();
    A.cost = 2 * (c->recombination / 2);
    A.dmax = O.dmax; A.bstart = O.bstart;
    A.tops = c->d_top.as<int32_t>();
    A.ent_src = O.ent_src; A.ent_h = O.ent_h;
    A.err = (uint32_t *)(c->d_scalars.as<uint64_t>() + S_ERR);
    A.q_limit = getenv("PHI_DP_QLIMIT") ? atoi(getenv("PHI_DP_QLIMIT")) : 0;
    phi_launch_dp_event_fill(c->stream, A, c->d_e_out.as<uint8_t>(), c->d_walk_vtx.as<int32_t>(), c->d_cvtx.as<int32_t>(),
                             c->d_a_e1.as<phi_ent_t>(), c->d_wpre.as<int32_t>(), c->n_entries);
    if (tr.on) { (void)hipStreamSynchronize(c->stream); tr.lap("weights + per-run records"); }
    A.lane_stride = c->blk_ls;
    return PHI_OK;
}

static void dp_block_args(const phi_ctx *c, PhiDpEventArgs &A)
{
    A.n_blk = c->n_blk; A.blk_ring = c->blk_ring; A.blk_max_len = c->blk_max_len; A.blk_lo = c->d_blk_lo.as<int32_t>(); A.blk_ev = c->d_blk_ev.as<int32_t>(); A.blk_S = c->d_blk_S.as<int32_t>();
    A.row_out = c->d_row_out.as<int32_t>(); A.rowend_out = c->d_rowend.as<int32_t>();
    A.blk_keys_out = c->d_blk_keys.as<int32_t>(); A.blk_carry = c->d_blk_carry.as<int32_t>();
}

static int dp_blocks_fallback(phi_ctx *c, uint32_t kerr, uint32_t bit, DpRetry *want)
{
// ... 17 lines not shown
        PHICHK(phi_dev_ensure(c, c->d_seg_lo, ((size_t)n_seg + 1) * 4));
        PHICHK(phi_dev_ensure(c, c->d_seg_row, (size_t)n_seg * (size_t)(c->n_walks + 1) * (size_t)c->blk_ls * 4));
        PHICHK(phi_dev_ensure(c, c->d_seg_S, (size_t)n_seg * (size_t)c->blk_ls * 4));
        HIPCHK(phi_copy_sync(c, c->d_seg_lo.p, seg_lo.data(), seg_lo.size() * 4, hipMemcpyHostToDevice));
        phi_launch_blk_chain_segments(c->stream, G, A.row_out, A.rownew_out, A.rowdiag_out, c->d_blk_S.as<int32_t>(), n_seg,
                                      c->d_seg_lo.as<int32_t>(), c->d_seg_row.as<int32_t>(), c->d_seg_S.as<int32_t>());
    } else {
        phi_launch_blk_chain(c->stream, G, A.row_out, A.rownew_out, A.rowdiag_out, c->d_blk_S.as<int32_t>());
    }
    HIPCHK(hipGetLastError());
    return PHI_OK;
}

static int dp_blocks_on_class_lanes(phi_ctx *c, PhiDpEventArgs &A, PhiStageTimer &tr, DpRetry *want)
{
    const int32_t nb = c->n_blk;
    dp_block_args(c, A);
    A.rownew_out = c->d_rownew.as<int32_t>();
    A.rowdiag_out = c->d_rowdiag.as<int32_t>();
    A.lane_walk = c->d_lane_walk.as<int32_t>();
    PhiBlkClassArgs G{};
    G.n_blk = nb; G.n_walks = c->n_walks; G.lane_stride = c->blk_ls;
    G.blk_lo = A.blk_lo; G.blk_ev = A.blk_ev; G.ev_off = A.ev_off; G.walk_off = A.walk_off; G.ev = A.ev;
    G.lane_walk = c->d_lane_walk.as<int32_t>(); G.walk_lane = c->d_walk_lane.as<int32_t>(); G.coff = c->d_coff.as<int32_t>();
    G.blk_ncls = c->d_blk_ncls.as<int32_t>(); G.err = A.err;
    phi_launch_blk_classes(c->stream, G);
    uint32_t kerr = 0;
    if (tr.on) {
        HIPCHK(hipMemcpyAsync(&kerr, c->d_scalars.as<uint64_t>() + S_ERR, 4, hipMemcpyDeviceToHost, c->stream));
        HIPCHK(hipStreamSynchronize(c->stream));
        tr.lap("block classes");
        if (kerr & PHI_KERR_DP_CLASSES) return dp_blocks_fallback(c, kerr, PHI_KERR_DP_CLASSES, want);
    }
    phi_launch_dp_block_rows(c->stream, A);
    if (tr.on) { (void)hipStreamSynchronize(c->stream); tr.lap("block rows"); }
    PHICHK(dp_chain_class_rows(c, G, A));
    if (tr.on) { (void)hipStreamSynchronize(c->stream); tr.lap("block chain"); }
    A.lane_walk = nullptr;
    phi_launch_dp_block_paths_wide(c->stream, A);
    int32_t bad[2] = {0, INT32_MAX};
    HIPCHK(hipMemcpyAsync(c->d_blk_bad.p, bad, 8, hipMemcpyHostToDevice, c->stream));
    phi_launch_blk_check(c->stream, A.blk_keys_out, A.blk_S, nb, c->blk_ls, c->n_walks, c->d_blk_bad.as<int32_t>());
    HIPCHK(hipMemcpyAsync(bad, c->d_blk_bad.p, 8, hipMemcpyDeviceToHost, c->stream));
    HIPCHK(hipMemcpyAsync(&kerr, c->d_scalars.as<uint64_t>() + S_ERR, 4, hipMemcpyDeviceToHost, c->stream));
    HIPCHK(hipStreamSynchronize(c->stream));
    if (tr.on) tr.lap("block paths + check");
    if (kerr & PHI_KERR_DP_CLASSES) return dp_blocks_fallback(c, kerr, PHI_KERR_DP_CLASSES, want);
    if (kerr & PHI_KERR_DP_QUEUE) return dp_blocks_fallback(c, kerr, PHI_KERR_DP_QUEUE, want);
    if (bad[0])
        return phi_fail(c, PHI_ERR_DEVICE, "DP blocks: %d keys leaving blocks (first in block %d) differ from the chained class rows (internal error)", bad[0], bad[1]);
    return PHI_OK;
}

static int dp_blocks_on_walk_lanes(phi_ctx *c, PhiDpEventArgs &A, DpHost &H, PhiStageTimer &tr, DpRetry *want)
{
    const int32_t nb = c->n_blk, nwk = c->n_walks, nrow = nwk + 1;
    dp_block_args(c, A);
    phi_launch_dp_block_rows(c->stream, A);
    H.rows.resize((size_t)nb * nrow * 64); H.rowend.resize((size_t)nb * nrow);
    HIPCHK(hipMemcpyAsync(H.rows.data(), A.row_out, H.rows.size() * 4, hipMemcpyDeviceToHost, c->stream));
    HIPCHK(hipMemcpyAsync(H.rowend.data(), A.rowend_out, H.rowend.size() * 4, hipMemcpyDeviceToHost, c->stream));
    uint32_t kerr = 0;
    HIPCHK(hipMemcpyAsync(&kerr, c->d_scalars.as<uint64_t>() + S_ERR, 4, hipMemcpyDeviceToHost, c->stream));
    HIPCHK(hipStreamSynchronize(c->stream));
    if (tr.on) tr.lap("block rows");
    if (kerr & PHI_KERR_DP_QUEUE) return dp_blocks_fallback(c, kerr, PHI_KERR_DP_QUEUE, want);
    (void)phi_chain_blocks(H.rows.data(), H.rowend.data(), nb, nwk, H.S);
    HIPCHK(hipMemcpyAsync(c->d_blk_S.p, H.S.data(), H.S.size() * 4, hipMemcpyHostToDevice, c->stream));
    phi_launch_dp_block_paths(c->stream, A);
    H.keys.resize((size_t)nb * 64); H.carry.resize((size_t)nb * 64);
    HIPCHK(hipMemcpyAsync(H.keys.data(), A.blk_keys_out, H.keys.size() * 4, hipMemcpyDeviceToHost, c->stream));
    HIPCHK(hipMemcpyAsync(H.carry.data(), A.blk_carry, H.carry.size() * 4, hipMemcpyDeviceToHost, c->stream));
    HIPCHK(hipMemcpyAsync(&kerr, c->d_scalars.as<uint64_t>() + S_ERR, 4, hipMemcpyDeviceToHost, c->stream));
    HIPCHK(hipStreamSynchronize(c->stream));
    if (kerr & PHI_KERR_DP_QUEUE) return dp_blocks_fallback(c, kerr, PHI_KERR_DP_QUEUE, want);
    int32_t b = 0, h = 0, got = 0, wanted = 0;
    if (!phi_chain_agrees(H.S.data(), H.keys.data(), nb, nwk, &b, &h, &got, &wanted))
        return phi_fail(c, PHI_ERR_DEVICE, "DP blocks: block %d leaves key %d on walk %d, the chained matrices say %d (internal error)", b, got, h, wanted);
    return PHI_OK;
}

static int dp_dense(phi_ctx *c, const DpOut &O)
{
    PHICHK(phi_dev_ensure(c, c->d_word, (size_t)c->n_entries * 8));
    phi_launch_dp_words(c->stream, c->d_e_out.as<uint8_t>(), c->d_g_off.as<int64_t>(), c->d_g_span.as<uint8_t>(),
                        c->d_a_weight.as<uint8_t>(), c->n_entries, c->d_word.as<uint64_t>());
    PhiDpArgs A{};
    A.n_vtx = c->n_vtx; A.n_walks = c->n_walks;
    A.st_rec = c->d_st_rec.as<int32_t>(); A.st_mask = c->d_st_mask.as<unsigned long long>();
    A.in_packed = c->d_in_packed.as<int32_t>();
    A.walk_off = c->d_walk_off.as<int64_t>();
    A.word = c->d_word.as<uint64_t>();
    A.g_off = c->d_g_off.as<int64_t>(); A.g_span = c->d_g_span.as<uint8_t>(); A.a_weight = c->d_a_weight.as<uint8_t>();
    A.cost = 2 * (c->recombination / 2);
    A.dmax = O.dmax; A.bstart = O.bstart;
    A.tops = c->d_top.as<int32_t>();
    A.ent_src = O.ent_src; A.ent_h = O.ent_h;
    phi_launch_dp(c->stream, A);
    return PHI_OK;
}

static int dp_fetch_ends(phi_ctx *c, const DpOut &O, bool events, DpHost &H, PhiStageTimer &tr, DpRetry *want)
{
    H.ends.resize(c->n_walks);
    phi_launch_gather_i32(c->stream, O.dmax, c->d_walk_last.as<phi_ent_t>(), c->n_walks, c->d_list3.as<int32_t>());
    HIPCHK(hipMemcpyAsync(H.ends.data(), c->d_list3.p, (size_t)c->n_walks * 4, hipMemcpyDeviceToHost, c->stream));
    uint32_t kerr = 0;
    if (events) HIPCHK(hipMemcpyAsync(&kerr, c->d_scalars.as<uint64_t>() + S_ERR, 4, hipMemcpyDeviceToHost, c->stream));
    HIPCHK(hipStreamSynchronize(c->stream));
    tr.lap("kernel");
    if (kerr & PHI_KERR_DP_QUEUE) {
        kerr &= ~PHI_KERR_DP_QUEUE;
        HIPCHK(phi_copy_sync(c, c->d_scalars.as<uint64_t>() + S_ERR, &kerr, 4, hipMemcpyHostToDevice));
        if (!c->dp_dense_ready) return phi_fail(c, PHI_ERR_DEVICE, "event DP queue overflow without a dense fallback (internal error)");
        *want = DP_DENSE;
    }
    return PHI_OK;
}

static int dp_pick_end(phi_ctx *c, const DpHost &H, int32_t *bh_, int64_t *value)
{
    int32_t bh = -1;
    int64_t best = INT64_MIN;
    for (int32_t h = 0; h < c->n_walks; h++) {
        const int32_t d = H.ends[h];
        if (d > -(1 << 28) && d > best) { best = d; bh = h; }
    }
    if (bh < 0) return phi_fail(c, PHI_ERR_DEVICE, "DP found no s->e path (internal error)");
    *bh_ = bh;
    *value = best;
    return PHI_OK;
}

static int entry_on_vertex(phi_ctx *c, int32_t h, int32_t rank, int32_t u, int64_t *e_)
{
    int64_t lo = c->h_walk_off[h], hi = c->h_walk_off[h + 1];
    while (lo < hi) {
        const int64_t mid = (lo + hi) >> 1;
        int32_t vm = 0;
        PHICHK(walk_vtx_at(c, mid, &vm));
        if (c->h_topo_rank[vm] < rank) lo = mid + 1; else hi = mid;
    }
    *e_ = -1;
    if (lo < c->h_walk_off[h + 1]) {
        int32_t vl = 0;
        PHICHK(walk_vtx_at(c, lo, &vl));
        if (vl == u) *e_ = lo;
    }
    return PHI_OK;
}

static int dp_backtrack(phi_ctx *c, const DpOut &O, bool events, DpHost &H, int32_t h, std::vector<Seg> *segs)
{
    bool bulk = false;
    auto fetch_bulk = [&]() -> int {
        H.bstart.resize(c->n_entries); H.ent_u.resize(O.n_ent); H.ent_h.resize(O.n_ent);
        HIPCHK(hipMemcpyAsync(H.bstart.data(), O.bstart, (size_t)c->n_entries * 4, hipMemcpyDeviceToHost, c->stream));
        HIPCHK(hipMemcpyAsync(H.ent_u.data(), O.ent_src, (size_t)O.n_ent * 4, hipMemcpyDeviceToHost, c->stream));
        HIPCHK(hipMemcpyAsync(H.ent_h.data(), O.ent_h, (size_t)O.n_ent * 4, hipMemcpyDeviceToHost, c->stream));
        HIPCHK(hipStreamSynchronize(c->stream));
        bulk = true;
        return PHI_OK;
    };
// ... 7 lines not shown
        if (bs < 0 && c->dp_blocks && events) {
            int32_t vq = 0;
            PHICHK(walk_vtx_at(c, e, &vq));
            const int32_t kq = c->h_cstep[c->h_topo_rank[vq]];
            int32_t b = (int32_t)(std::upper_bound(c->h_blk_lo.begin(), c->h_blk_lo.end(), kq) - c->h_blk_lo.begin()) - 1;
            if (c->dp_cls) {
                int32_t out[2] = {-1, -1};
                phi_launch_carry_resolve(c->stream, c->d_blk_carry.as<int32_t>(), c->blk_ls, b, h, c->d_blk_bad.as<int32_t>() + 2);
                HIPCHK(hipMemcpyAsync(out, c->d_blk_bad.as<int32_t>() + 2, 8, hipMemcpyDeviceToHost, c->stream));
                HIPCHK(hipStreamSynchronize(c->stream));
                bs = out[1];
            } else {
                while (bs < 0 && --b >= 0) bs = H.carry[(size_t)b * 64 + h];
            }
            if (bs < 0) return phi_fail(c, PHI_ERR_DEVICE, "DP backtrack: a carried run has no beginning (internal error)");
        }
        const int64_t es = c->h_walk_off[h] + bs;
        if (es < c->h_walk_off[h] || es > e) return phi_fail(c, PHI_ERR_DEVICE, "DP backtrack left the walk (internal error)");
        segs->push_back(Seg{h, es, e});
        if (es == c->h_walk_off[h]) break;
        int32_t v = 0;
        PHICHK(walk_vtx_at(c, es, &v));
        const int32_t step = events ? c->h_cstep[c->h_topo_rank[v]] : c->h_topo_rank[v];
        if (step < 0) return phi_fail(c, PHI_ERR_DEVICE, "DP backtrack: run begins on a vertex without events (internal error)");
        int32_t src, h2;
        if (bulk) { src = H.ent_u[step]; h2 = H.ent_h[step]; }
        else {
            HIPCHK(phi_copy_sync(c, &src, O.ent_src + step, 4, hipMemcpyDeviceToHost));
            HIPCHK(phi_copy_sync(c, &h2, O.ent_h + step, 4, hipMemcpyDeviceToHost));
        }
        if (events && src >= 0) src = c->h_kstep[src];
        const int32_t u = src >= 0 ? c->h_topo[src] : -1;
        if (u < 0 || h2 < 0) return phi_fail(c, PHI_ERR_DEVICE, "DP backtrack hit a vertex without an entry (internal error)");
        int64_t e2 = -1;
        PHICHK(entry_on_vertex(c, h2, src, u, &e2));
        if (e2 < 0) return phi_fail(c, PHI_ERR_DEVICE, "DP backtrack: walk %d is not on vertex %d (internal error)", h2, u);
        h = h2; e = e2;
    }
    std::reverse(segs->begin(), segs->end());
    return PHI_OK;
}

static int run_dp(phi_ctx *c, const std::vector<uint8_t> *wgt, DpHost &H, int64_t *value, std::vector<Seg> *segs)
{
    for (DpRetry want = DP_DONE;;) {
        switch (want) {
        case DP_DONE: break;
        case DP_HALVE_CLASS_TARGET: c->blk_cls_target /= 2; PHICHK(dp_prepare_blocks(c, c->n_dp)); break;
        case DP_NO_SMALL_BLOCKS: c->blk_no_small = true; PHICHK(dp_prepare_blocks(c, c->n_dp)); break;
        case DP_GIVE_UP_BLOCKS: c->dp_blocks = false; c->dp_cls = false; break;
        case DP_DENSE: c->dp_events = false; break;
        }
        want = DP_DONE;
        const bool events = c->dp_events;
        const DpOut O = dp_out(c);
        PhiStageTimer tr("dp run");
        if (c->n_dp && wgt) HIPCHK(hipMemcpyAsync(c->d_a_weight.p, wgt->data(), (size_t)c->n_dp, hipMemcpyHostToDevice, c->stream));
        if (events) {
            PhiDpEventArgs A{};
            PHICHK(dp_event_records(c, O, A, tr));
            if (c->dp_blocks && c->dp_cls) PHICHK(dp_blocks_on_class_lanes(c, A, tr, &want));
            else if (c->dp_blocks) PHICHK(dp_blocks_on_walk_lanes(c, A, H, tr, &want));
            else phi_launch_dp_events(c->stream, A);
            if (want != DP_DONE) continue;
        } else {
            PHICHK(dp_dense(c, O));
        }
        HIPCHK(hipGetLastError());
        PHICHK(dp_fetch_ends(c, O, events, H, tr, &want));
        if (want != DP_DONE) continue;
        int32_t bh = -1;
        PHICHK(dp_pick_end(c, H, &bh, value));
        PHICHK(dp_backtrack(c, O, events, H, bh, segs));
        tr.lap("backtrack");
        return PHI_OK;
    }
}

template <class F> static void for_covered(const phi_ctx *c, const std::vector<Seg> &segs, F f)
{
    const PhiAnchorSpan &A = c->h_dp;
    for (const Seg &s : segs) {
        auto lo = std::lower_bound(A.begin(), A.end(), s.es, [](const PhiAnchorHost &a, int64_t e) { return (int64_t)a.e1 < e; });
        for (auto it = lo; it != A.end() && (int64_t)it->e1 <= s.ee; ++it)
            if ((int64_t)it->e0 >= s.es) f((int64_t)(it - A.begin()));
    }
}

struct Node {
    std::vector<std::pair<uint32_t, int32_t>> assign;
    int64_t ub = INT64_MAX;
};

struct Search {
    std::vector<Node> stack;
    std::vector<int64_t> open_ub;
    int64_t incumbent = INT64_MIN, global_ub = INT64_MIN, best_cov = 0;
    int n_runs = 0;
    bool exhausted = false;
};

struct Solve {
    phi_ctx *const c;
    PhiStageTimer tm{"solve"};
    int64_t n_matched = 0, n_kept_rec = 0, n_kept = 0, n_dp = 0;
    int64_t filtered = 0, in_model = 0, spectrum = 0;
    bool anchors_prepped = false;
    bool dev = false;
    PhiAnchorArrays arr;
    std::vector<int32_t> sa_off, sa_idx;
    std::vector<uint8_t> wgt;
    std::vector<int32_t> cov_all, cov_w;
    std::vector<uint32_t> touched;
    std::set<uint32_t> S0;
    DpHost H;
    Search bb;
    std::vector<Seg> best_segs;
    explicit Solve(phi_ctx *c_) : c(c_) {}
};

static int read_spectrum(Solve &S)
{
    phi_ctx *c = S.c;
    if (c->dp_alloc_future.valid()) PHICHK(c->dp_alloc_future.get());
    PHICHK(phi_sync_check(c));
    S.tm = PhiStageTimer("solve");
    uint64_t sc[S_N];
    HIPCHK(phi_copy_sync(c, sc, c->d_scalars.p, sizeof sc, hipMemcpyDeviceToHost));
    uint64_t n_distinct = 0;
    PHICHK(phi_spectrum_count(c, &n_distinct));
    S.tm.lap("read spectrum (set from the log)");
    S.spectrum = c->spectrum_override >= 0 ? c->spectrum_override : (int64_t)n_distinct;
    return PHI_OK;
}

static int match_and_compact(Solve &S)
{
    phi_ctx *c = S.c;
    const int64_t n_rec = c->n_rec;
    PHICHK(phi_dev_ensure(c, c->d_flags, (size_t)std::max<int64_t>(n_rec, 1)));
    phi_launch_match_flags(c->stream, c->d_rec_slot.as<uint32_t>(), n_rec, c->d_u_uid.as<uint32_t>(),
                           c->d_hit.as<uint8_t>(), c->d_flags.as<uint8_t>());
    PHICHK(phi_compact(c, c->d_flags.as<uint8_t>(), n_rec, c->d_m_rec, &S.n_matched));
    S.tm.lap("match + compact");
    return PHI_OK;
}

static int filter_shared_anchors(Solve &S)
{
    phi_ctx *c = S.c;
    const int64_t n_rec = c->n_rec, n_matched = S.n_matched;
    PhiFilterArgs F{};
    F.rec_slot = c->d_rec_slot.as<uint32_t>(); F.rec_e0 = c->d_rec_e0.as<phi_ent_t>(); F.rec_e1 = c->d_rec_e1.as<phi_ent_t>();
    F.walk_vtx = c->d_walk_vtx.as<int32_t>();
    F.rec_cls = c->d_rec_cls.as<int32_t>(); F.cls_mult = c->d_cls_mult.as<int32_t>();
    F.m_rec = c->d_m_rec.as<int32_t>();
    const uint64_t g_cap = pow2_at_least(std::max<uint64_t>(1024, 2 * (uint64_t)n_matched));
    PHICHK(phi_dev_ensure(c, c->d_g_keys, g_cap * 8));
    PHICHK(phi_dev_ensure(c, c->d_g_rep, g_cap * 4));
    PHICHK(phi_dev_ensure(c, c->d_g_cnt, g_cap * 4));
    PHICHK(phi_dev_ensure(c, c->d_m_group, (size_t)std::max<int64_t>(n_matched, 1) * 4));
    const size_t n_slot_ids = (size_t)std::max<int64_t>(c->n_unique, 1);
    PHICHK(phi_dev_ensure(c, c->d_slot_maxcnt, n_slot_ids * 4));
    PHICHK(phi_dev_ensure(c, c->d_slot_multi, n_slot_ids));
    F.g_keys = c->d_g_keys.as<uint64_t>(); F.g_rep = c->d_g_rep.as<int32_t>(); F.g_cnt = c->d_g_cnt.as<uint32_t>();
    F.g_mask = g_cap - 1;
    F.m_group = c->d_m_group.as<int32_t>();
    F.u_uid = c->d_u_uid.as<uint32_t>();
    F.slot_maxcnt = c->d_slot_maxcnt.as<uint32_t>(); F.slot_multi = c->d_slot_multi.as<uint8_t>();
    F.limit = c->threshold * (float)(uint32_t)c->n_walks;
    F.counters = (unsigned long long *)scalar(c, S_FILTERED);
    F.err = (uint32_t *)scalar(c, S_ERR);
    for (int attempt = 0;; attempt++) {
        F.seed = 0x243F6A8885A308D3ull + 0x9E3779B97F4A7C15ull * (uint64_t)attempt;
        phi_launch_fill_u64(c->stream, F.g_keys, (int64_t)g_cap, PHI_EMPTY_KEY);
        phi_launch_fill_u32(c->stream, (uint32_t *)F.g_rep, (int64_t)g_cap, 0xFFFFFFFFu);
        HIPCHK(hipMemsetAsync(F.g_cnt, 0, g_cap * 4, c->stream));
        phi_launch_group_insert(c->stream, F, n_matched);
        phi_launch_group_count(c->stream, F, n_matched);
        HIPCHK(hipStreamSynchronize(c->stream));
        uint32_t err = 0;
// ... 30 lines not shown
    PhiExpandArgs X{};
    X.ent_cls = c->d_ent_cls.as<int32_t>(); X.e_lo = 0; X.e_hi = c->n_entries;
    X.cls_rec_off = c->d_cls_rec_off.as<int32_t>(); X.cls_rep = c->d_cls_rep.as<phi_ent_t>();
    X.sel = c->d_flags2.as<uint8_t>(); X.sel_cnt = c->d_list3.as<int32_t>();
    X.rec_slot = c->d_rec_slot.as<uint32_t>(); X.u_uid = c->d_u_uid.as<uint32_t>();
    X.rec_e0 = c->d_rec_e0.as<phi_ent_t>(); X.rec_e1 = c->d_rec_e1.as<phi_ent_t>();
    const int64_t nb = phi_expand_num_blocks(c->n_entries);
    PHICHK(phi_dev_ensure(c, c->d_blk_cnt, (size_t)nb * 4));
    PHICHK(phi_dev_ensure(c, c->d_blk_off, (size_t)(nb + 1) * 8));
    X.block_cnt = c->d_blk_cnt.as<int32_t>(); X.block_off = c->d_blk_off.as<int64_t>();
    phi_launch_expand_count(c->stream, X);
    PHICHK(phi_scan(c, c->d_blk_cnt.as<int32_t>(), nb, c->d_blk_off.as<int64_t>()));
    int64_t n_kept = 0;
    HIPCHK(hipMemcpyAsync(&n_kept, c->d_blk_off.as<int64_t>() + nb, 8, hipMemcpyDeviceToHost, c->stream));
    HIPCHK(hipStreamSynchronize(c->stream));
    if (n_kept >= (int64_t)1 << 31) return phi_fail(c, PHI_ERR_UNSUPPORTED, "more than 2^31 anchors in the model");
    S.n_kept = n_kept;
    c->h_kept = PhiAnchorSpan{}; c->h_dp = PhiAnchorSpan{}; c->anchors_host = false;
    c->n_kept = n_kept; c->n_dp = 0;
    c->h_kept_hash.clear();
    PHICHK(phi_dev_ensure(c, c->d_anchors, (size_t)std::max<int64_t>(n_kept, 1) * 12));
    static_assert(sizeof(PhiAnchorHost) == 12, "PhiAnchorHost is the device triple");
    PHICHK(phi_dev_ensure(c, c->d_a_e1, (size_t)std::max<int64_t>(n_kept, 1) * 4));
    PHICHK(phi_dev_ensure(c, c->d_g_span, (size_t)std::max<int64_t>(n_kept, 1)));
    PHICHK(phi_dev_ensure(c, c->d_ctr, (size_t)(nw + 8) * 8));
    HIPCHK(hipMemsetAsync(c->d_ctr.p, 0, (size_t)(nw + 8) * 8, c->stream));
    if (n_kept && getenv("PHI_EXPAND_GENERIC")) {
        X.out_tri = c->d_anchors.as<uint32_t>();
        phi_launch_expand_write(c->stream, X, 1);
    } else if (n_kept) {
        PHICHK(phi_dev_ensure(c, c->d_sel_off, (size_t)(c->n_cls + 1) * 4));
        PHICHK(phi_dev_ensure(c, c->d_sel_tri, (size_t)std::max<int64_t>(n_kept_rec, 1) * 12));
        PHICHK(phi_scan(c, c->d_list3.as<int32_t>(), c->n_cls, c->d_sel_off.as<int32_t>()));
        phi_launch_class_sel_tri(c->stream, c->d_flags2.as<uint8_t>(), c->d_cls_rec_off.as<int32_t>(), c->n_cls, c->d_sel_off.as<int32_t>(), c->d_cls_rep.as<phi_ent_t>(),
                                 c->d_rec_slot.as<uint32_t>(), c->d_u_uid.as<uint32_t>(), c->d_rec_e0.as<phi_ent_t>(), c->d_rec_e1.as<phi_ent_t>(), c->d_sel_tri.as<int32_t>());
        unsigned long long *d_ctr = c->d_ctr.as<unsigned long long>();
        phi_launch_expand_tri(c->stream, c->d_ent_cls.as<int32_t>(), 0, c->n_entries, c->d_sel_off.as<int32_t>(), c->d_sel_tri.as<int32_t>(),
                              c->d_blk_off.as<int64_t>(), c->d_anchors.as<uint32_t>(), c->d_a_e1.as<phi_ent_t>(), c->d_g_span.as<uint8_t>(),
                              c->d_walk_off.as<int64_t>(), nw, d_ctr + 8, d_ctr, n_kept);
        S.anchors_prepped = true;
    }
    return PHI_OK;
}

static int check_anchors_choose_mode(Solve &S)
{
    phi_ctx *c = S.c;
    const int32_t nw = c->n_walks;
    const int64_t n_kept = S.n_kept;
    unsigned long long *d_ctr = c->d_ctr.as<unsigned long long>();
    if (!S.anchors_prepped)
        phi_launch_anchor_prep(c->stream, c->d_anchors.as<uint32_t>(), n_kept, c->d_walk_off.as<int64_t>(), nw, c->d_a_e1.as<phi_ent_t>(), c->d_g_span.as<uint8_t>(), d_ctr + 8, d_ctr);
    std::vector<unsigned long long> hc((size_t)nw + 8);
    HIPCHK(hipMemcpyAsync(hc.data(), d_ctr, hc.size() * 8, hipMemcpyDeviceToHost, c->stream));
    HIPCHK(hipStreamSynchronize(c->stream));
    if (hc[1] & 1) return phi_fail(c, PHI_ERR_DEVICE, "dp anchors not sorted by last entry (internal error)");
    if (hc[1] & 2)
        return phi_fail(c, c->k > PHI_RCAP ? PHI_ERR_UNSUPPORTED : PHI_ERR_DEVICE, "an anchor spans %d edges or more%s", PHI_RCAP,
                        c->k > PHI_RCAP ? ": with k > 32 the graph's vertices must be long enough for a k-mer to cover at most 32 of them" : " (internal error)");
    c->h_n_anchors.assign(nw, 0);
    for (int32_t h = 0; h < nw; h++) c->h_n_anchors[h] = (int64_t)hc[(size_t)h + 8];
    int64_t dev_min = (int64_t)1 << 16;
    if (const char *e = getenv("PHI_SOLVE_DEVICE")) dev_min = atoi(e) ? 0 : INT64_MAX;
    S.dev = hc[0] == 0 && n_kept >= dev_min && n_kept > 0;
    uint64_t sc[S_N];
    HIPCHK(phi_copy_sync(c, sc, c->d_scalars.p, sizeof sc, hipMemcpyDeviceToHost));
    S.filtered = (int64_t)sc[S_FILTERED]; S.in_model = (int64_t)sc[S_INMODEL];
    return PHI_OK;
}

static int anchors_to_host(Solve &S)
{
    phi_ctx *c = S.c;
    const int64_t n_kept = S.n_kept;
    if (S.dev) {
        S.tm.lap("anchor arrays (device)");
        c->n_dp = n_kept;
    } else {
        PHICHK(phi_pin_ensure(c, (size_t)std::max<int64_t>(n_kept, 1) * sizeof(PhiAnchorHost)));
        c->h_kept = PhiAnchorSpan{static_cast<PhiAnchorHost *>(c->h_pin), n_kept};
        if (n_kept) HIPCHK(hipMemcpyAsync(c->h_kept.p, c->d_anchors.p, (size_t)n_kept * 12, hipMemcpyDeviceToHost, c->stream));
        HIPCHK(hipStreamSynchronize(c->stream));
        c->anchors_host = true;
        S.tm.lap("anchors D2H");
        PhiHostError herr;
        if (phi_anchor_arrays(c->h_kept, c->h_walk_off.data(), c->n_walks, c->k, c->h_dp_own, S.arr, c->h_n_anchors, herr))
            return phi_fail(c, herr.code, "%s", herr.msg.c_str());
        c->h_dp = S.arr.dp;
        c->n_dp = (int64_t)c->h_dp.size();
    }
    S.n_dp = c->n_dp;
    if (S.tm.on) fprintf(stderr, "[phi timing] solve: class records %lld, matched %lld, kept %lld -> anchors kept %lld, dp %lld\n", (long long)c->n_rec, (long long)S.n_matched, (long long)S.n_kept_rec, (long long)n_kept, (long long)S.n_dp);
    S.tm.lap("filter (GPU) + anchors D2H");
    return PHI_OK;
}

static int anchor_entry_csr(Solve &S)
{
    phi_ctx *c = S.c;
    const int64_t n_dp = S.n_dp;
    PHICHK(phi_dev_ensure(c, c->d_a_weight, (size_t)std::max<int64_t>(n_dp, 1)));
    PHICHK(phi_dev_ensure(c, c->d_g_off, (size_t)(c->n_entries + 1) * 8));
    if (n_dp && !S.dev) {
        HIPCHK(hipMemcpyAsync(c->d_a_e1.p, S.arr.a_e1.data(), (size_t)n_dp * 4, hipMemcpyHostToDevice, c->stream));
        HIPCHK(hipMemcpyAsync(c->d_g_span.p, S.arr.a_span.data(), (size_t)n_dp, hipMemcpyHostToDevice, c->stream));
    }
    phi_launch_entry_csr(c->stream, c->d_a_e1.as<phi_ent_t>(), n_dp, c->n_entries, c->d_g_off.as<int64_t>());
    return PHI_OK;
}

static int score_bound_host(Solve &S, int64_t *bound)
{
    phi_ctx *c = S.c;
    PHICHK(ensure_host_walks(c));
    *bound = phi_score_bound(S.arr.a_e1.data(), S.n_dp, c->h_walk_vtx.data(), c->n_vtx);
    return PHI_OK;
}
static int score_bound_dev(Solve &S, int64_t *bound)
{
    phi_ctx *c = S.c;
    PHICHK(phi_dev_ensure(c, c->d_vmax, (size_t)c->n_vtx * 4));
    HIPCHK(hipMemsetAsync(c->d_vmax.p, 0, (size_t)c->n_vtx * 4, c->stream));
    HIPCHK(hipMemsetAsync(c->d_ctr.p, 0, 8, c->stream));
    phi_launch_vertex_most(c->stream, c->d_g_off.as<int64_t>(), c->n_entries, c->d_walk_vtx.as<int32_t>(), c->d_vmax.as<int32_t>());
    phi_launch_sum_i32(c->stream, c->d_vmax.as<int32_t>(), c->n_vtx, c->d_ctr.as<unsigned long long>());
    unsigned long long sum = 0;
    HIPCHK(hipMemcpyAsync(&sum, c->d_ctr.p, 8, hipMemcpyDeviceToHost, c->stream));
    HIPCHK(hipStreamSynchronize(c->stream));
    *bound = (int64_t)sum;
    return PHI_OK;
}
static int check_score_range(Solve &S)
{
    phi_ctx *c = S.c;
    if (S.n_dp < ((int64_t)1 << 27)) return PHI_OK;
    int64_t bound = 0;
    PHICHK(S.dev ? score_bound_dev(S, &bound) : score_bound_host(S, &bound));
    if (bound >= ((int64_t)1 << 27)) return phi_fail(c, PHI_ERR_UNSUPPORTED, "a path could score %lld >= 2^27 anchors", (long long)bound);
    return PHI_OK;
}

static int dp_inputs(Solve &S)
{
    phi_ctx *c = S.c;
    const int32_t nw = c->n_walks;
    HIPCHK(hipStreamSynchronize(c->stream));
    {
        std::vector<phi_ent_t> last(nw);
        for (int32_t h = 0; h < nw; h++) last[h] = (phi_ent_t)(c->h_walk_off[h + 1] - 1);
        PHICHK(phi_dev_ensure(c, c->d_walk_last, (size_t)nw * 4));
        PHICHK(phi_dev_ensure(c, c->d_list3, (size_t)nw * 4));
        HIPCHK(phi_copy_sync(c, c->d_walk_last.p, last.data(), (size_t)nw * 4, hipMemcpyHostToDevice));
    }
    PHICHK(phi_dev_ensure(c, c->d_dmax, (size_t)c->n_entries * 4));
    PHICHK(phi_dev_ensure(c, c->d_bstart, (size_t)c->n_entries * 4));
    if (c->dp_events) {
        const int64_t ne1 = c->n_entries + 1;
        PHICHK(phi_dev_ensure(c, c->d_off_end, (size_t)(ne1 + 2) * 4));
        PHICHK(phi_dev_ensure(c, c->d_off_start, (size_t)(ne1 + 2) * 4));
        PHICHK(phi_dev_ensure(c, c->d_ev, (size_t)std::max<int64_t>(c->n_ev, 1) * 48));
    }
    PHICHK(phi_dev_ensure(c, c->d_top, (size_t)c->n_vtx * 5 * 4));
    PHICHK(phi_dev_ensure(c, c->d_ent, (size_t)c->n_vtx * 2 * 4));
    c->blk_no_small = false;
    c->blk_cls_target = 16;
    PHICHK(dp_prepare_blocks(c, S.n_dp));
    S.tm.lap("DP inputs");
    return PHI_OK;
}

static int anchor_csr_dev(Solve &S, bool fetch)
{
    phi_ctx *c = S.c;
    const int64_t n_ids = c->n_unique, n_dp = S.n_dp;
    const uint32_t *tri = c->d_anchors.as<uint32_t>();
    PHICHK(phi_dev_ensure(c, c->d_sa_cnt, (size_t)(n_ids + 1) * 4));
    PHICHK(phi_dev_ensure(c, c->d_sa_cur, (size_t)(n_ids + 1) * 4));
    PHICHK(phi_dev_ensure(c, c->d_sa_off, (size_t)(n_ids + 2) * 4));
    PHICHK(phi_dev_ensure(c, c->d_sa_idx, (size_t)n_dp * 4));
    HIPCHK(hipMemsetAsync(c->d_sa_cnt.p, 0, (size_t)(n_ids + 1) * 4, c->stream));
    HIPCHK(hipMemsetAsync(c->d_sa_cur.p, 0, (size_t)(n_ids + 1) * 4, c->stream));
    phi_launch_csr_count(c->stream, tri, n_dp, n_ids, c->d_sa_cnt.as<int32_t>(), (uint32_t *)scalar(c, S_ERR));
    PHICHK(phi_scan(c, c->d_sa_cnt.as<int32_t>(), n_ids, c->d_sa_off.as<int32_t>()));
    phi_launch_csr_scatter(c->stream, tri, n_dp, n_ids, c->d_sa_off.as<int32_t>(), c->d_sa_cur.as<int32_t>(), c->d_sa_idx.as<int32_t>());
    phi_launch_csr_sort(c->stream, c->d_sa_off.as<int32_t>(), n_ids, c->d_sa_idx.as<int32_t>());
    int32_t total = 0;
    if (fetch) {
        S.sa_off.resize((size_t)n_ids + 1); S.sa_idx.resize((size_t)std::max<int64_t>(n_dp, 1));
        HIPCHK(hipMemcpyAsync(S.sa_off.data(), c->d_sa_off.p, (size_t)(n_ids + 1) * 4, hipMemcpyDeviceToHost, c->stream));
        HIPCHK(hipMemcpyAsync(S.sa_idx.data(), c->d_sa_idx.p, (size_t)n_dp * 4, hipMemcpyDeviceToHost, c->stream));
    }
    HIPCHK(hipMemcpyAsync(&total, c->d_sa_off.as<int32_t>() + n_ids, 4, hipMemcpyDeviceToHost, c->stream));
    uint32_t kerr = 0;
    HIPCHK(hipMemcpyAsync(&kerr, scalar(c, S_ERR), 4, hipMemcpyDeviceToHost, c->stream));
    HIPCHK(hipStreamSynchronize(c->stream));
    if ((kerr & PHI_KERR_CSR_ID) || total != (int32_t)n_dp)
        return phi_fail(c, PHI_ERR_DEVICE, "minimiser id out of range (internal error)");
    return PHI_OK;
}

static int anchors_of_minimisers(Solve &S)
{
    phi_ctx *c = S.c;
    const int64_t n_ids = c->n_unique, n_dp = S.n_dp;
    if (!S.dev) {
        const bool dp_is_kept = c->h_dp.p == c->h_kept.p && c->h_dp.size() == c->h_kept.size();
        if (dp_is_kept && n_dp > 0) PHICHK(anchor_csr_dev(S, true));
        else if (!phi_anchor_csr(c->h_dp, n_ids, S.sa_off, S.sa_idx)) return phi_fail(c, PHI_ERR_DEVICE, "minimiser id out of range (internal error)");
    }
    S.tm.lap("minimiser -> anchors map");
    return PHI_OK;
}

static int repeat_set_dev(Solve &S)
{
    phi_ctx *c = S.c;
    const int64_t n_ids = c->n_unique;
    PHICHK(phi_dev_ensure(c, c->d_flags, (size_t)std::max<int64_t>(n_ids, 1)));
    PHICHK(phi_dev_ensure(c, c->d_last_walk, (size_t)std::max<int64_t>(n_ids, 1) * 4));
    HIPCHK(hipMemsetAsync(c->d_flags.p, 0, (size_t)std::max<int64_t>(n_ids, 1), c->stream));
    HIPCHK(hipMemsetAsync(c->d_last_walk.p, 0xFF, (size_t)std::max<int64_t>(n_ids, 1) * 4, c->stream));
    int64_t lo = 0;
    for (int32_t h = 0; h < c->n_walks; h++) {
        phi_launch_repeat_walk(c->stream, c->d_anchors.as<uint32_t>(), lo, lo + c->h_n_anchors[h], h, c->d_last_walk.as<int32_t>(), c->d_flags.as<uint8_t>());
        lo += c->h_n_anchors[h];
    }
    if (lo != S.n_dp) return phi_fail(c, PHI_ERR_DEVICE, "anchors per walk do not add up (internal error)");
    int64_t n_rep = 0;
    PHICHK(phi_compact(c, c->d_flags.as<uint8_t>(), n_ids, c->d_list, &n_rep));
    std::vector<uint32_t> rep((size_t)n_rep);
    if (n_rep) HIPCHK(phi_copy_sync(c, rep.data(), c->d_list.p, (size_t)n_rep * 4, hipMemcpyDeviceToHost));
    S.S0.insert(rep.begin(), rep.end());
    return PHI_OK;
}
static int repeat_set(Solve &S)
{
    if (!getenv("PHI_NO_S0")) {
        if (S.dev) PHICHK(repeat_set_dev(S));
        else phi_repeat_set(S.sa_off, S.sa_idx, S.arr.dp_walk, S.c->n_unique, S.S0);
        if (S.tm.on) fprintf(stderr, "[phi timing] solve: %zu minimisers repeat along a walk\n", S.S0.size());
    }
    S.tm.lap("repeat set");
    return PHI_OK;
}

struct Span {
    const int32_t *p; int32_t n;
    const int32_t *begin() const { return p; }
    const int32_t *end() const { return p + n; }
    int32_t operator[](int32_t i) const { return p[i]; }
};
static Span anchors_of(const Solve &S, uint32_t s) { return Span{S.sa_idx.data() + S.sa_off[s], S.sa_off[s + 1] - S.sa_off[s]}; }

static std::vector<std::vector<int32_t>> clusters_of(const Solve &S, uint32_t slot)
{
    const phi_ctx *c = S.c;
    std::vector<PhiAnchorIv> iv;
    for (int32_t a : anchors_of(S, slot)) {
        const PhiAnchorHost &A = c->h_dp[a];
        iv.push_back(PhiAnchorIv{c->h_topo_rank[c->h_walk_vtx[A.e0]], c->h_topo_rank[c->h_walk_vtx[A.e1]], phi_entry_walk(c, A.e0), a});
    }
    return phi_clusters(std::move(iv));
}

static int to_host(Solve &S)
{
    phi_ctx *c = S.c;
    const int64_t n_ids = c->n_unique, n_dp = S.n_dp;
    PHICHK(ensure_host_walks(c));
    if (!S.dev) return PHI_OK;
    PhiStageTimer th("solve");
    PHICHK(phi_host_anchors(c));
    if (n_dp) PHICHK(anchor_csr_dev(S, true));
    else { S.sa_off.assign((size_t)n_ids + 1, 0); S.sa_idx.assign(1, 0); }
    S.wgt.assign((size_t)n_dp, 1);
    S.cov_all.assign((size_t)n_ids, 0); S.cov_w.assign((size_t)n_ids, 0);
    S.touched.clear();
    S.dev = false;
// ... 225 lines not shown
            for (int64_t i = 0; i <= s.ee - s.es; i++) { const int32_t v = c->h_path_vtx[(size_t)(o + i)]; hap_len += c->h_seq_off[v + 1] - c->h_seq_off[v]; }
            o += s.ee - s.es + 1;
        }
    }
    int32_t recomb = 0;
    for (size_t i = 1; i < best_segs.size(); i++) recomb += best_segs[i].h != best_segs[i - 1].h;

    phi_result &R = c->result;
    R.objective = S.bb.incumbent;
    R.upper_bound = upper_bound;
    R.optimal = upper_bound == S.bb.incumbent;
    R.n_dp_runs = S.bb.n_runs;
    R.n_covered = S.bb.best_cov;
    R.n_path = (int64_t)c->h_path_vtx.size();
    R.path_vtx = c->h_path_vtx.data();
    R.path_hap = c->h_path_hap.data();
    R.recombination_count = recomb;
    R.n_switches = (int32_t)best_segs.size() - 1;
    R.hap_len = hap_len;
    R.n_walks = c->n_walks;
    R.n_minimizers = c->h_n_minimizers.data();
    R.n_anchors = c->h_n_anchors.data();
    R.spectrum_size = S.spectrum;
    R.filtered = S.filtered;
    R.retained = S.spectrum - S.filtered;
    R.n_in_model = S.in_model;
    S.tm.lap("decode");
    c->path_segs.clear();
    for (const Seg &s : best_segs) c->path_segs.push_back({s.h, s.es, s.ee});
    c->calls.have = false;
    c->solved = true;
    return PHI_OK;
}

int phi_solve_impl(phi_ctx *c)
{
    c->solved = false;
    Solve S(c);
    PHICHK(read_spectrum(S));
    PHICHK(match_and_compact(S));
    PHICHK(filter_shared_anchors(S));
    PHICHK(expand_kept_records(S));
    PHICHK(check_anchors_choose_mode(S));
    PHICHK(anchors_to_host(S));
    PHICHK(anchor_entry_csr(S));
    PHICHK(check_score_range(S));
    PHICHK(dp_inputs(S));
    PHICHK(anchors_of_minimisers(S));
    PHICHK(repeat_set(S));
    int64_t upper_bound = 0;
    PHICHK(search(S, &upper_bound));
    return decode(S, upper_bound);
}
```

phi_amd/csrc/phi_wave.h:

```cpp
#pragma once
#include <hip/hip_runtime.h>
#include <stdint.h>
#include <type_traits>

template <class T>
using phi_shfl_t = std::conditional_t<sizeof(T) == 8, std::conditional_t<std::is_signed<T>::value, long long, unsigned long long>, T>;

template <class T>
__device__ __forceinline__ T phi_wave_incl_scan(T x)
{
    static_assert(std::is_integral<T>::value && (sizeof(T) == 4 || sizeof(T) == 8), "int, uint32_t, int64_t, uint64_t");
    const int lane = threadIdx.x & 63;
#pragma unroll
    for (int d = 1; d < 64; d <<= 1) {
        const T y = (T)__shfl_up((phi_shfl_t<T>)x, d, 64);
        if (lane >= d) x += y;
    }
    return x;
}

template <class T>
__device__ __forceinline__ T phi_wave_sum(T x)
{
    static_assert(std::is_integral<T>::value && (sizeof(T) == 4 || sizeof(T) == 8), "int, uint32_t, int64_t, uint64_t");
#pragma unroll
    for (int d = 32; d >= 1; d >>= 1) x += (T)__shfl_xor((phi_shfl_t<T>)x, d, 64);
    return x;
}

template <int NW, class T>
__device__ __forceinline__ T phi_block_excl_scan(T mine, T *s_w, T *total = nullptr)
{
    const int lane = threadIdx.x & 63, wid = threadIdx.x >> 6;
    const T inc = phi_wave_incl_scan(mine);
    if (lane == 63) s_w[wid] = inc;
    __syncthreads();
    T woff = 0;
    for (int i = 0; i < wid; i++) woff += s_w[i];
    if (total) {
        T t = 0;
#pragma unroll
        for (int i = 0; i < NW; i++) t += s_w[i];
        *total = t;
    }
    return woff + inc - mine;
}
```

phi_amd/csrc/set_graph.hip:

```cpp
#include <string.h>
#include <algorithm>
#include <future>
#include <memory>
#include "phi_ctx.h"
#include "phi_dev.h"
#include "dp_steps.h"

static int build_read_table(phi_ctx *c)
{
    uint64_t nb = pow2_at_least(std::max<uint64_t>(64, (16 * (uint64_t)c->n_unique + 2) / 3));
    if (const char *e = getenv("PHI_READ_TABLE_BUCKETS")) nb = pow2_at_least(std::max<long long>(atoll(e), 1));
    uint32_t err0 = 0;
    HIPCHK(hipMemcpyAsync(&err0, scalar(c, S_ERR), 4, hipMemcpyDeviceToHost, c->stream));
    HIPCHK(hipStreamSynchronize(c->stream));
    for (int attempt = 0;; attempt++) {
        PHICHK(phi_dev_ensure(c, c->d_rt, nb * 32));
        phi_launch_read_table(c->stream, c->d_u_keys.as<uint64_t>(), c->d_u_uid.as<uint32_t>(), (int64_t)c->u_cap,
                              c->d_rt.as<uint64_t>(), (int64_t)nb, (uint32_t *)scalar(c, S_ERR));
        uint32_t err = 0;
        HIPCHK(hipMemcpyAsync(&err, scalar(c, S_ERR), 4, hipMemcpyDeviceToHost, c->stream));
        HIPCHK(hipStreamSynchronize(c->stream));
        if ((err0 & PHI_KERR_TABLE_FULL) || !(err & PHI_KERR_TABLE_FULL)) break;
        if (attempt >= 40) return phi_fail(c, PHI_ERR_OVERFLOW, "read table overflow at %llu buckets (internal error)", (unsigned long long)nb);
        err &= ~PHI_KERR_TABLE_FULL;
// ... 203 lines not shown
    HIPCHK(hipGetLastError());
    return PHI_OK;
}

int set_graph_check_args(phi_ctx *c, int32_t n_vtx, const char *seq_concat, const int64_t *seq_off, const int64_t *adj_off,
                         const int32_t *adj, int32_t n_walks, const int64_t *walk_off, const int32_t *walk_vtx, const int32_t *topo_rank)
{
    const bool dev_walks = walk_vtx == nullptr;
    if (dev_walks && c && walk_off && n_walks > 0 && !(c->walks_on_device && c->walks_on_device_n == walk_off[n_walks] && (int32_t)(c->wtext.ends.size() / 2) == n_walks))
        return phi_fail(c, PHI_ERR_STATE, "phi_set_graph without walk_vtx: phi_walk_text_resolve must have resolved exactly these walks on this context");
    if (n_vtx <= 0 || n_walks <= 0 || !seq_concat || !seq_off || !adj_off || !walk_off || !topo_rank)
        return phi_fail(c, PHI_ERR_INVALID, "phi_set_graph: null pointer or empty graph");
    if (adj_off[n_vtx] > 0 && !adj) return phi_fail(c, PHI_ERR_INVALID, "phi_set_graph: adj is null");
    HIPCHK(hipSetDevice(c->device));
    if (c->ipc) return phi_fail(c, PHI_ERR_STATE, "phi_set_graph on a context in a group of processes: phi_ipc_destroy first (the peers have this context's hit vectors mapped)");
    c->have_graph = false;
    c->chop.on = false;
    c->panel.on = false;
    phi_scout_end(c);
    c->solved = false;
    phi_ladder_drop(c);
    return PHI_OK;
}
int set_graph_check_offsets(phi_ctx *c, int32_t n_vtx, const int64_t *seq_off, const int64_t *adj_off, int32_t n_walks, const int64_t *walk_off)
{
    if (seq_off[0] != 0 || adj_off[0] != 0 || walk_off[0] != 0) return phi_fail(c, PHI_ERR_INVALID, "offset arrays must start at 0");
    for (int32_t v = 0; v < n_vtx; v++)
        if (seq_off[v + 1] < seq_off[v] || adj_off[v + 1] < adj_off[v]) return phi_fail(c, PHI_ERR_INVALID, "offsets not monotone at vertex %d", v);
    for (int32_t h = 0; h < n_walks; h++)
        if (walk_off[h + 1] <= walk_off[h]) return phi_fail(c, PHI_ERR_INVALID, "walk %d is empty", h);
    if (walk_off[n_walks] > PHI_MAX_ENTRIES) return phi_fail(c, PHI_ERR_UNSUPPORTED, "more than 2^32 - 64 walk entries");
    return PHI_OK;
}

struct SetGraph {
    phi_ctx *const c;
    const int32_t n_vtx;
    const char *const seq_concat;
    const int64_t *const seq_off, *const adj_off;
    const int32_t *const adj;
    const int32_t n_walks;
    const int64_t *const walk_off;
    const int32_t *const walk_vtx, *const topo_rank;
    int64_t n_edges = 0, n_entries = 0;
    const bool dev_walks;
    bool want_masks = false;
    bool keep_host_walks = false;
    PhiStageTimer tm{"set_graph"};
    std::vector<int64_t> indeg;
    std::vector<int32_t> cnt_edge;
    int32_t walk_err[4] = {0, 0, 0, 0};
    std::vector<int32_t> ends_own;
    const int32_t *walk_ends = nullptr;
    PhiDpSteps steps;
    std::promise<int> edges_promise;
    std::future<int> edges_future = edges_promise.get_future();
    std::future<int> uploads, gpu;
    std::future<void> wv_copy;

    SetGraph(phi_ctx *c_, int32_t n_vtx_, const char *seq_concat_, const int64_t *seq_off_, const int64_t *adj_off_, const int32_t *adj_,
             int32_t n_walks_, const int64_t *walk_off_, const int32_t *walk_vtx_, const int32_t *topo_rank_)
        : c(c_), n_vtx(n_vtx_), seq_concat(seq_concat_), seq_off(seq_off_), adj_off(adj_off_), adj(adj_), n_walks(n_walks_), walk_off(walk_off_),
          walk_vtx(walk_vtx_), topo_rank(topo_rank_), dev_walks(walk_vtx_ == nullptr) {}
    ~SetGraph()
    {
        if (gpu.valid()) gpu.wait();
        if (wv_copy.valid()) wv_copy.wait();
        if (uploads.valid()) uploads.wait();
    }
};

static void start_pinning(SetGraph &S)
{
    phi_ctx *c = S.c;
    if (c->pin_future.valid()) c->pin_future.wait();
    int64_t ne = S.walk_off[S.n_walks];
    ne = ne < 0 ? 0 : (ne > PHI_MAX_ENTRIES ? PHI_MAX_ENTRIES : ne);
    const size_t want = ((size_t)ne / 4 + 4096) * sizeof(PhiAnchorHost);
    if (want > c->h_pin_cap && ne / 4 < ((int64_t)1 << 16) && !getenv("PHI_PREPIN")) {
        c->h_kept = PhiAnchorSpan{}; c->h_dp = PhiAnchorSpan{}; c->anchors_host = false;
        c->pin_future = std::async(std::launch::async, [c, want]() {
            (void)hipSetDevice(c->device);
            if (c->h_pin) (void)hipHostFree(c->h_pin);
            c->h_pin = nullptr; c->h_pin_cap = 0;
            void *p = nullptr;
            if (hipHostMalloc(&p, want, hipHostMallocDefault) == hipSuccess) { c->h_pin = p; c->h_pin_cap = want; }
        });
    }
}

static void start_dp_buffers(SetGraph &S)
{
    phi_ctx *c = S.c;
    if (c->dp_alloc_future.valid()) (void)c->dp_alloc_future.get();
    if (S.n_entries >= ((int64_t)1 << 24) && S.n_walks <= PHI_DP_EVENT_MAX_WALKS) {
        c->dp_alloc_future = std::async(std::launch::async, [c, n_entries = S.n_entries]() -> int {
            if (hipSetDevice(c->device) != hipSuccess) return PHI_ERR_DEVICE;
            const size_t ne = (size_t)n_entries;
            PHICHK(phi_dev_ensure(c, c->d_g_off, (ne + 1) * 8));
            PHICHK(phi_dev_ensure(c, c->d_dmax, ne * 4));
            PHICHK(phi_dev_ensure(c, c->d_bstart, ne * 4));
            PHICHK(phi_dev_ensure(c, c->d_off_end, (ne + 3) * 4));
            PHICHK(phi_dev_ensure(c, c->d_off_start, (ne + 3) * 4));
            return PHI_OK;
        });
    }
}

static void start_uploads(SetGraph &S)
{
    S.uploads = std::async(std::launch::async, [&S]() -> int {
        phi_ctx *c = S.c;
        HIPCHK(hipSetDevice(c->device));
        PHICHK(upload(c, c->d_seq, S.seq_concat, (size_t)S.seq_off[S.n_vtx]));
        PHICHK(upload(c, c->d_seq_off, S.seq_off, (size_t)S.n_vtx + 1));
        if (!S.dev_walks) PHICHK(upload(c, c->d_walk_vtx, S.walk_vtx, (size_t)S.n_entries));
        PHICHK(upload(c, c->d_walk_off, S.walk_off, (size_t)S.n_walks + 1));
        PHICHK(upload(c, c->d_adj_off, S.adj_off, (size_t)S.n_vtx + 1));
        if (S.n_edges == 0) PHICHK(phi_dev_ensure(c, c->d_adj, 4));
        else PHICHK(upload(c, c->d_adj, S.adj, (size_t)S.n_edges));
        PHICHK(upload(c, c->d_topo_rank, S.topo_rank, (size_t)S.n_vtx));
        return PHI_OK;
    });
}

static int validate_topology(SetGraph &S)
{
    phi_ctx *c = S.c;
    PhiHostError verr;
    S.indeg.assign((size_t)S.n_vtx, 0);
    if (phi_topo_from_ranks(S.n_vtx, S.topo_rank, c->h_topo, verr) ||
        phi_check_edges(S.n_vtx, S.adj_off, S.adj, S.topo_rank, S.indeg.data(), verr))
        return phi_fail(c, verr.code, "%s", verr.msg.c_str());
    return PHI_OK;
}

static int start_host_walk_copy(SetGraph &S)
{
    phi_ctx *c = S.c;
    int64_t host_walks_max = (int64_t)1 << 26;
    if (const char *e = getenv("PHI_HOST_WALKS_MAX")) host_walks_max = atoll(e);
    S.keep_host_walks = S.n_entries <= host_walks_max;
    if (!c->h_walk_vtx.resize(S.keep_host_walks ? S.n_entries : 0)) return phi_fail(c, PHI_ERR_NOMEM, "host allocation failed");
    if (!S.keep_host_walks) return PHI_OK;
    S.wv_copy = std::async(std::launch::async, [c, dev_walks = S.dev_walks, n_entries = S.n_entries, walk_vtx = S.walk_vtx]() {
        int32_t *dst = c->h_walk_vtx.data();
        if (dev_walks) {
            (void)hipSetDevice(c->device);
            if (n_entries && hipMemcpyAsync(dst, c->d_walk_vtx.p, (size_t)n_entries * 4, hipMemcpyDeviceToHost, c->aux_stream) == hipSuccess)
                (void)hipStreamSynchronize(c->aux_stream);
            return;
        }
        const int nt = 4;
        std::vector<std::thread> th;
        for (int t = 0; t < nt; t++)
            th.emplace_back([=]() {
                const int64_t lo = n_entries * t / nt, hi = n_entries * (t + 1) / nt;
                memcpy(dst + lo, walk_vtx + lo, (size_t)(hi - lo) * 4);
            });
        for (auto &x : th) x.join();
    });
    return PHI_OK;
}

static int walk_entry_pass(SetGraph &S)
{
    phi_ctx *c = S.c;
    const int nw64 = c->dp_nw;
    PHICHK(phi_dev_ensure(c, c->d_e_out, (size_t)S.n_entries));
    PHICHK(phi_dev_ensure(c, c->d_cnt_edge, S.cnt_edge.size() * 4));
// ... 315 lines not shown
```

phi_amd/csrc/solve_dev.hip:

```cpp
#include <hip/hip_runtime.h>
#include "phi_dev.h"
#include "phi_kernels.h"

static inline unsigned grid_for(int64_t n, int tpb)
{
    int64_t nb = (n + tpb - 1) / tpb;
    if (nb > 256 * 16) nb = 256 * 16;
    if (nb < 1) nb = 1;
    return (unsigned)nb;
}
#define GRID_STRIDE(i, n) \
    for (int64_t i = (int64_t)blockIdx.x * blockDim.x + threadIdx.x; i < (n); i += (int64_t)gridDim.x * blockDim.x)

__device__ __forceinline__ int32_t walk_of_entry(const int64_t *__restrict__ walk_off, int32_t n_walks, int64_t e)
{
    int lo = 0, hi = n_walks;
    while (hi - lo > 1) {
        const int mid = (lo + hi) >> 1;
        if (walk_off[mid] <= e) lo = mid; else hi = mid;
    }
    return lo;
}
__device__ __forceinline__ void wave_count(bool pred, unsigned long long *ctr)
{
    const unsigned long long b = __ballot(pred);
    if (b && (threadIdx.x & 63) == (unsigned)(__ffsll((long long)b) - 1)) atomicAdd(ctr, (unsigned long long)__popcll(b));
}

__global__ void __launch_bounds__(256) phi_anchor_prep_kernel(const uint32_t *__restrict__ tri, int64_t n, const int64_t *__restrict__ walk_off,
                                                              int32_t n_walks, phi_ent_t *__restrict__ a_e1, uint8_t *__restrict__ a_span,
                                                              unsigned long long *__restrict__ walk_cnt, unsigned long long *__restrict__ out)
{
    GRID_STRIDE(i0, (n + 63) & ~(int64_t)63) {
        const bool in = i0 < n;
        const int64_t i = in ? i0 : n - 1;
        const phi_ent_t e0 = tri[i * 3 + 1], e1 = tri[i * 3 + 2];
        wave_count(in && e1 <= e0, &out[0]);
        uint32_t bad = 0;
        if (in && i > 0 && e1 < tri[(i - 1) * 3 + 2]) bad |= 1u;
        if (in && e1 > e0 && e1 - e0 >= PHI_RCAP) bad |= 2u;
        if (bad) atomicOr(&out[1], (unsigned long long)bad);
        if (in) { a_e1[i] = e1; a_span[i] = (uint8_t)(e1 > e0 ? e1 - e0 : 0); }
        const int32_t h = walk_of_entry(walk_off, n_walks, e0);
        const int32_t h0 = __builtin_amdgcn_readfirstlane(h);
        if (__ballot(in && h != h0) == 0) wave_count(in, &walk_cnt[h0]);
        else if (in) atomicAdd(&walk_cnt[h], 1ull);
    }
}
void phi_launch_anchor_prep(hipStream_t st, const uint32_t *tri, int64_t n, const int64_t *walk_off, int32_t n_walks, phi_ent_t *a_e1, uint8_t *a_span,
                            unsigned long long *walk_cnt, unsigned long long *out)
{
    if (n > 0) hipLaunchKernelGGL(phi_anchor_prep_kernel, dim3(grid_for(n, 256)), dim3(256), 0, st, tri, n, walk_off, n_walks, a_e1, a_span, walk_cnt, out);
}

__global__ void __launch_bounds__(256) phi_vertex_most_kernel(const int64_t *__restrict__ g_off, int64_t n_entries, const int32_t *__restrict__ walk_vtx,
                                                              int32_t *__restrict__ vmax)
{
    GRID_STRIDE(e, n_entries) {
        const int64_t cnt = g_off[e + 1] - g_off[e];
        if (cnt > 0) atomicMax(&vmax[walk_vtx[e]], (int32_t)(cnt > INT32_MAX ? INT32_MAX : cnt));
    }
}
__global__ void __launch_bounds__(256) phi_sum_i32_kernel(const int32_t *__restrict__ v, int64_t n, unsigned long long *__restrict__ out)
{
    unsigned long long s = 0;
    GRID_STRIDE(i, n) s += (unsigned long long)v[i];
    for (int o = 32; o > 0; o >>= 1) s += __shfl_down(s, o);
    if ((threadIdx.x & 63) == 0 && s) atomicAdd(out, s);
}
void phi_launch_vertex_most(hipStream_t st, const int64_t *g_off, int64_t n_entries, const int32_t *walk_vtx, int32_t *vmax)
{
    if (n_entries > 0) hipLaunchKernelGGL(phi_vertex_most_kernel, dim3(grid_for(n_entries, 256)), dim3(256), 0, st, g_off, n_entries, walk_vtx, vmax);
}
void phi_launch_sum_i32(hipStream_t st, const int32_t *v, int64_t n, unsigned long long *out)
{
    if (n > 0) hipLaunchKernelGGL(phi_sum_i32_kernel, dim3(grid_for(n, 256)), dim3(256), 0, st, v, n, out);
}

__global__ void __launch_bounds__(256) phi_repeat_walk_kernel(const uint32_t *__restrict__ tri, int64_t lo, int64_t hi, int32_t walk,
                                                              int32_t *__restrict__ last, uint8_t *__restrict__ flags)
{
    for (int64_t a = lo + (int64_t)blockIdx.x * blockDim.x + threadIdx.x; a < hi; a += (int64_t)gridDim.x * blockDim.x) {
        const uint32_t id = tri[a * 3];
        if (atomicExch(&last[id], walk) == walk) flags[id] = 1;
    }
}
void phi_launch_repeat_walk(hipStream_t st, const uint32_t *tri, int64_t lo, int64_t hi, int32_t walk, int32_t *last, uint8_t *flags)
{
    if (hi > lo) hipLaunchKernelGGL(phi_repeat_walk_kernel, dim3(grid_for(hi - lo, 256)), dim3(256), 0, st, tri, lo, hi, walk, last, flags);
}
__global__ void __launch_bounds__(256) phi_weights_kernel(const uint32_t *__restrict__ tri, int64_t n, const uint8_t *__restrict__ in_s, uint8_t *__restrict__ wgt)
{
    GRID_STRIDE(a, n) wgt[a] = in_s[tri[a * 3]] ? 0 : 1;
}
void phi_launch_weights(hipStream_t st, const uint32_t *tri, int64_t n, const uint8_t *in_s, uint8_t *wgt)
{
    if (n > 0) hipLaunchKernelGGL(phi_weights_kernel, dim3(grid_for(n, 256)), dim3(256), 0, st, tri, n, in_s, wgt);
}

template <bool CLEAR>
__global__ void __launch_bounds__(256) phi_path_cover_kernel(const phi_ent_t *__restrict__ segs, int32_t n_seg, const int64_t *__restrict__ g_off,
                                                             const uint32_t *__restrict__ tri, const uint8_t *__restrict__ wgt,
                                                             int32_t *__restrict__ cov_all, int32_t *__restrict__ cov_w,
                                                             unsigned long long *__restrict__ ctr, uint32_t *__restrict__ twice, int64_t twice_cap)
{
    for (int32_t q = blockIdx.y; q < n_seg; q += gridDim.y) {
        const phi_ent_t es = segs[2 * q], ee = segs[2 * q + 1];
        const int64_t lo = g_off[es], hi = g_off[(int64_t)ee + 1];
        const int64_t span = (hi - lo + 63) & ~(int64_t)63;
        for (int64_t i0 = (int64_t)blockIdx.x * blockDim.x + threadIdx.x; i0 < span; i0 += (int64_t)gridDim.x * blockDim.x) {
            const int64_t a = lo + i0;
            const bool in = a < hi && tri[a * 3 + 1] >= es;
            const uint32_t s = in ? tri[a * 3] : 0;
            if (CLEAR) {
                if (in) { cov_all[s] = 0; cov_w[s] = 0; }
                continue;
            }
            const bool first = in && atomicAdd(&cov_all[s], 1) == 0;
            const bool w = in && wgt[a] != 0;
            const int32_t before = w ? atomicAdd(&cov_w[s], 1) : -1;
            wave_count(w, &ctr[0]);
            wave_count(first, &ctr[1]);
            if (before == 1) {
                const unsigned long long at = atomicAdd(&ctr[2], 1ull);
                if ((int64_t)at < twice_cap) twice[at] = s;
            }
        }
    }
}
void phi_launch_path_cover(hipStream_t st, bool clear, const phi_ent_t *segs, int32_t n_seg, const int64_t *g_off, const uint32_t *tri, const uint8_t *wgt,
                           int32_t *cov_all, int32_t *cov_w, unsigned long long *ctr, uint32_t *twice, int64_t twice_cap)
{
    if (n_seg <= 0) return;
    const dim3 grid(n_seg <= 8 ? 512 : n_seg <= 256 ? 32 : 2, (unsigned)(n_seg < 16384 ? n_seg : 16384));
    if (clear) hipLaunchKernelGGL(phi_path_cover_kernel<true>, grid, dim3(256), 0, st, segs, n_seg, g_off, tri, wgt, cov_all, cov_w, ctr, twice, twice_cap);
    else hipLaunchKernelGGL(phi_path_cover_kernel<false>, grid, dim3(256), 0, st, segs, n_seg, g_off, tri, wgt, cov_all, cov_w, ctr, twice, twice_cap);
}

__global__ void __launch_bounds__(256) phi_uncovered_slots_kernel(const uint32_t *__restrict__ slots, int64_t n, const int32_t *__restrict__ cov_all,
                                                                  unsigned long long *__restrict__ ctr, uint32_t *__restrict__ out)
{
    GRID_STRIDE(i, n) {
        const uint32_t s = slots[i];
        if (cov_all[s] == 0) out[atomicAdd(&ctr[3], 1ull)] = s;
    }
}
void phi_launch_uncovered_slots(hipStream_t st, const uint32_t *slots, int64_t n, const int32_t *cov_all, unsigned long long *ctr, uint32_t *out)
{
    if (n > 0) hipLaunchKernelGGL(phi_uncovered_slots_kernel, dim3(grid_for(n, 256)), dim3(256), 0, st, slots, n, cov_all, ctr, out);
}

__global__ void phi_warm_solve_dev_kernel() {}
void phi_warm_solve_dev(hipStream_t st) { hipLaunchKernelGGL(phi_warm_solve_dev_kernel, dim3(1), dim3(64), 0, st); }
```

phi_amd/csrc/table.hip:

```cpp
#include <hip/hip_runtime.h>
#include "phi_dev.h"
#include "phi_kernels.h"
#include "phi_wave.h"

__global__ void phi_fill_u64_kernel(uint64_t *p, int64_t n, uint64_t v)
{
    for (int64_t i = (int64_t)blockIdx.x * blockDim.x + threadIdx.x; i < n; i += (int64_t)gridDim.x * blockDim.x)
        p[i] = v;
}
__global__ void phi_fill_u32_kernel(uint32_t *p, int64_t n, uint32_t v)
{
    for (int64_t i = (int64_t)blockIdx.x * blockDim.x + threadIdx.x; i < n; i += (int64_t)gridDim.x * blockDim.x)
        p[i] = v;
}

static inline unsigned grid_for(int64_t n, int tpb)
{
    int64_t nb = (n + tpb - 1) / tpb;
    if (nb > 256 * 16) nb = 256 * 16;
    if (nb < 1) nb = 1;
    return (unsigned)nb;
}

__global__ void __launch_bounds__(256) phi_read_table_clear_kernel(ulonglong2 *__restrict__ rt, int64_t n_slots)
// ... 285 lines not shown
                           sp_keys, sp_mask, sp_count, k, u_keys, u_mask, err);
}

__global__ void __launch_bounds__(256) phi_kmer_keys_kernel(const int32_t *__restrict__ rec_cls, const int32_t *__restrict__ rec_rel,
                                                            const uint64_t *__restrict__ rec_hash, const uint32_t *__restrict__ rec_slot,
                                                            int64_t n_rec, const int64_t *__restrict__ cls_base, const uint8_t *__restrict__ cls_left,
                                                            const uint64_t *__restrict__ words, const uint32_t *__restrict__ badbits, int32_t k,
                                                            uint64_t *__restrict__ kkeys, unsigned long long *__restrict__ ctr)
{
    for (int64_t i = (int64_t)blockIdx.x * blockDim.x + threadIdx.x; i < n_rec; i += (int64_t)gridDim.x * blockDim.x) {
        const int32_t c = rec_cls[i];
        const int64_t p = cls_base[c] + cls_left[c] + rec_rel[i];
        const int64_t wi = p >> 5;
        const int s = (int)(p & 31);
        const uint64_t bad = (((uint64_t)badbits[wi + 1] << 32) | badbits[wi]) >> s;
        if (bad & ((1ull << k) - 1)) { atomicAdd(&ctr[0], 1ull); continue; }
        const uint64_t f = phi_extract64(words, p) >> (64 - 2 * k), r = phi_revcomp(f, k);
        const uint64_t v = f < r ? f : r;
        if (phi_kmer_hash(v, k) != rec_hash[i]) { atomicAdd(&ctr[1], 1ull); continue; }
        const uint64_t key = phi_kmer_mix(v);
        unsigned long long *slot = (unsigned long long *)&kkeys[rec_slot[i]];
        unsigned long long prev = __builtin_nontemporal_load(slot);
        if (prev == PHI_EMPTY_KEY) prev = atomicCAS(slot, PHI_EMPTY_KEY, key);
        if (prev != PHI_EMPTY_KEY && prev != key) atomicAdd(&ctr[2], 1ull);
    }
}
void phi_launch_kmer_keys(hipStream_t st, const int32_t *rec_cls, const int32_t *rec_rel, const uint64_t *rec_hash, const uint32_t *rec_slot,
                          int64_t n_rec, const int64_t *cls_base, const uint8_t *cls_left, const uint64_t *words, const uint32_t *badbits,
                          int32_t k, uint64_t *kkeys, unsigned long long *ctr)
{
    if (n_rec > 0)
        hipLaunchKernelGGL(phi_kmer_keys_kernel, dim3(grid_for(n_rec, 256)), dim3(256), 0, st, rec_cls, rec_rel, rec_hash, rec_slot, n_rec,
                           cls_base, cls_left, words, badbits, k, kkeys, ctr);
}

__global__ void __launch_bounds__(256) phi_rt_overflowed_kernel(const uint64_t *__restrict__ rt, int64_t n_buckets,
                                                                unsigned long long *__restrict__ n_out)
{
    int cnt = 0;
    for (int64_t b = (int64_t)blockIdx.x * blockDim.x + threadIdx.x; b < n_buckets; b += (int64_t)gridDim.x * blockDim.x)
        cnt += (int)((rt[4 * b + 1] >> 32) & PHI_RT_OVERFLOWED);
    cnt = phi_wave_sum(cnt);
    if ((threadIdx.x & 63) == 0 && cnt) atomicAdd(n_out, (unsigned long long)cnt);
}
void phi_launch_rt_overflowed(hipStream_t st, const uint64_t *rt, int64_t n_buckets, unsigned long long *n_out)
{
    if (n_buckets > 0)
        hipLaunchKernelGGL(phi_rt_overflowed_kernel, dim3(grid_for(n_buckets, 256)), dim3(256), 0, st, rt, n_buckets, n_out);
}

__global__ void __launch_bounds__(256) phi_count_flags_kernel(const uint8_t *__restrict__ flags, int64_t n,
                                                              unsigned long long *__restrict__ n_out)
{
    int cnt = 0;
    for (int64_t i = (int64_t)blockIdx.x * blockDim.x + threadIdx.x; i < n; i += (int64_t)gridDim.x * blockDim.x)
        cnt += flags[i] != 0;
    cnt = phi_wave_sum(cnt);
    if ((threadIdx.x & 63) == 0 && cnt) atomicAdd(n_out, (unsigned long long)cnt);
}

void phi_launch_count_flags(hipStream_t st, const uint8_t *flags, int64_t n, unsigned long long *n_out)
{
    if (n > 0) hipLaunchKernelGGL(phi_count_flags_kernel, dim3(grid_for(n, 256)), dim3(256), 0, st, flags, n, n_out);
}

__global__ void __launch_bounds__(256) phi_spectrum_export_kernel(const uint64_t *__restrict__ sp_keys, int64_t cap,
                                                                  uint64_t *__restrict__ out,
                                                                  unsigned long long *__restrict__ n_out)
{
    for (int64_t i0 = (int64_t)blockIdx.x * blockDim.x; i0 < cap; i0 += (int64_t)gridDim.x * blockDim.x) {
        const int64_t i = i0 + threadIdx.x;
        const uint64_t key = i < cap ? sp_keys[i] : PHI_EMPTY_KEY;
        const bool occ = key != PHI_EMPTY_KEY;
        const unsigned long long bal = __ballot(occ);
        const int lane = threadIdx.x & 63;
        unsigned long long base = 0;
        if (lane == 0 && bal) base = atomicAdd(n_out, (unsigned long long)__popcll(bal));
        base = __shfl(base, 0, 64);
        if (occ) out[base + __popcll(bal & ((1ull << lane) - 1))] = key;
    }
}

void phi_launch_spectrum_export(hipStream_t st, const uint64_t *sp_keys, int64_t cap, uint64_t *out,
                                unsigned long long *n_out)
{
    if (cap > 0)
        hipLaunchKernelGGL(phi_spectrum_export_kernel, dim3(grid_for(cap, 256)), dim3(256), 0, st, sp_keys, cap, out,
                           n_out);
}

__global__ void phi_warm_table_kernel() {}
void phi_warm_table(hipStream_t st) { hipLaunchKernelGGL(phi_warm_table_kernel, dim3(1), dim3(64), 0, st); }
```

Before: 482.8.

## Chain DP block rows on device and batch repeat detection, block-level counters

Moves the per-block row chaining of the walk-lane DP from a host round trip to a single-workgroup device kernel with prefetched rows, keeping the host chain behind an environment flag. Replaces per-walk repeat detection launches with a grouped kernel using a 64-bit walk mask per id. Also switches several counter kernels to block-level reductions with fewer atomics, vectorises the flag count with 16-byte loads, caps grid sizes, and removes an unused scalar readback. The device chain is serial over blocks in one workgroup, so it may lose to the host when there are many blocks.

```diff
diff --git a/include/phi_amd.h b/include/phi_amd.h
--- a/include/phi_amd.h
+++ b/include/phi_amd.h
@@ -220,6 +220,8 @@
 
 int phi_prefix_sums(phi_ctx *ctx, int32_t kind, const void *d_in, int64_t n, void *d_out);
 
+int phi_chain_walk_rows(phi_ctx *ctx, const void *d_rows, int32_t n_blk, int32_t n_walks, void *d_S);
+
 int phi_edit_distances(phi_ctx *ctx, const char *a, const int64_t *a_off, const char *b, const int64_t *b_off,
                        int64_t n_pairs, int64_t max_distance, int64_t *out);
 
diff --git a/phi_amd/_capi.py b/phi_amd/_capi.py
--- a/phi_amd/_capi.py
+++ b/phi_amd/_capi.py
@@ -31,7 +31,7 @@
     "phi_reads_collect_begin", "phi_reads_collect_end", "phi_reads_collect_release", "phi_ladder_plan", "phi_ladder_advance", "phi_ladder_band",
     "phi_set_graph_panel", "phi_panel_origin", "phi_panel_walks", "phi_panel_stats", "phi_panel_release",
     "phi_scout_graph", "phi_scout_scores", "phi_scout_choose", "phi_reads_collect_score", "phi_vcf_walks_wide",
-    "phi_prefix_sums",
+    "phi_prefix_sums", "phi_chain_walk_rows",
     "phi_reads_bam_begin", "phi_add_reads_bam", "phi_add_reads_bam_parked", "phi_reads_bam_end", "phi_reads_bam_last_batch",
     "phi_calls_path", "phi_calls_walk", "phi_calls_stats",
 ]
@@ -252,7 +252,12 @@
     L.phi_gfa_gzip_split.argtypes = [vp, vp, i64, i64, C.POINTER(vp), C.POINTER(i64), C.POINTER(PhiGfaGzipInfo)]
     L.phi_gfa_gzip_free.argtypes = [vp]
     L.phi_gfa_gzip_free.restype = None
+    older = {"phi_chain_walk_rows"} if os.environ.get("PHI_AMD_LIB") and not hasattr(L, "phi_chain_walk_rows") else set()
+    if not older:
+        L.phi_chain_walk_rows.argtypes = [vp, vp, i32, i32, vp]
     for name in SYMBOLS:
+        if name in older:
+            continue
         f = getattr(L, name)
         if f.restype is C.c_int and name not in ("phi_strerror", "phi_last_error", "phi_ctx_destroy", "phi_crc32_combine", "phi_inflate_free", "phi_gfa_gzip_free"):
             f.restype = C.c_int
diff --git a/phi_amd/context.py b/phi_amd/context.py
--- a/phi_amd/context.py
+++ b/phi_amd/context.py
@@ -663,6 +663,9 @@
     def prefix_sums(self, kind, d_in, n, d_out):
         self._chk(self._L.phi_prefix_sums(self._h, kind, C.c_void_p(d_in), n, C.c_void_p(d_out)))
 
+    def chain_walk_rows(self, d_rows, n_blk, n_walks, d_S):
+        self._chk(self._L.phi_chain_walk_rows(self._h, C.c_void_p(d_rows), n_blk, n_walks, C.c_void_p(d_S)))
+
     def prof_enable(self, on=True):
         self._chk(self._L.phi_prof_enable(self._h, int(on)))
 
diff --git a/phi_amd/csrc/anchors.hip b/phi_amd/csrc/anchors.hip
--- a/phi_amd/csrc/anchors.hip
+++ b/phi_amd/csrc/anchors.hip
@@ -187,9 +187,11 @@
         if ((float)c >= A.limit) n_filtered++;
         else if (A.slot_multi[s]) n_model++;
     }
-    n_filtered = phi_wave_sum(n_filtered);
-    n_model = phi_wave_sum(n_model);
-    if ((threadIdx.x & 63) == 0) {
+    __shared__ int s_w[4];
+    n_filtered = phi_block_sum<4>(n_filtered, s_w);
+    __syncthreads();
+    n_model = phi_block_sum<4>(n_model, s_w);
+    if (threadIdx.x == 0) {
         if (n_filtered) atomicAdd(&A.counters[0], (unsigned long long)n_filtered);
         if (n_model) atomicAdd(&A.counters[1], (unsigned long long)n_model);
     }
@@ -220,7 +222,7 @@
 }
 void phi_launch_slot_count(hipStream_t st, const PhiFilterArgs &A, int64_t u_cap)
 {
-    if (u_cap > 0) hipLaunchKernelGGL(phi_slot_count_kernel, dim3(grid_for(u_cap, 256)), dim3(256), 0, st, A, u_cap);
+    if (u_cap > 0) hipLaunchKernelGGL(phi_slot_count_kernel, dim3(std::min(grid_for(u_cap, 1024), 512u)), dim3(256), 0, st, A, u_cap);
 }
 void phi_launch_kept_flags(hipStream_t st, const PhiFilterArgs &A, int64_t n, uint8_t *kept, uint8_t *dp)
 {
diff --git a/phi_amd/csrc/dp_events.hip b/phi_amd/csrc/dp_events.hip
--- a/phi_amd/csrc/dp_events.hip
+++ b/phi_amd/csrc/dp_events.hip
@@ -567,6 +567,7 @@
     uint4 cA = make_uint4(0xFFFFFFFFu, 0, 0, 0);
     if (vi < ve) cA = s_ev[vi & (D - 1)][0][h];
     int32_t qh = 0, qn = 0, hs = 0, hE = 0, tk = 0;
+    const int32_t q_cap = A.q_limit > 0 && A.q_limit < QD ? A.q_limit : QD;
     int32_t M = NEGK, sL = MODE == DP_SEQ ? 0 : -1, Emax = NEG;
     if (MODE == DP_ROW && h == row_j) M = 0;
     if (MODE == DP_PATH && has_walk) M = A.blk_S[(int64_t)sb * A.lane_stride + h];
@@ -663,7 +664,7 @@
                         qn--;
                         if (qn > 0) tk = s_qK[(qh + qn - 1) & (QD - 1)][h];
                     }
-                    if (QD < 32 && qn == QD) { atomicOr(A.err, PHI_KERR_DP_QUEUE); qn--; }
+                    if (QD < 32 && qn >= q_cap) { atomicOr(A.err, PHI_KERR_DP_QUEUE); qn--; }
                     const int slq = (qh + qn) & (QD - 1);
                     s_qs[slq][h] = t; s_qE[slq][h] = newE; s_qK[slq][h] = key;
                     if (qn == 0) { hs = t; hE = newE; }
@@ -1088,6 +1089,62 @@
     }
 }
 
+__global__ void __launch_bounds__(256) phi_walk_chain_kernel(const int32_t *__restrict__ rows, int32_t n_blk, int32_t n_walks, int32_t *__restrict__ blk_S)
+{
+    constexpr int DEPTH = 4, NJ = 17;
+    __shared__ int32_t s_part[2][4][64];
+    const int lane = threadIdx.x & 63, wid = __builtin_amdgcn_readfirstlane(threadIdx.x >> 6);
+    const int32_t nrow = n_walks + 1;
+    const bool has_walk = lane < n_walks;
+    int32_t st_row[DEPTH][NJ];
+    int32_t off[NJ];
+#pragma unroll
+    for (int i = 0; i < NJ; i++) off[i] = (wid + min(4 * i, n_walks - wid)) * 64 + lane;
+    auto issue = [&](auto J, int32_t b) {
+        constexpr int d = decltype(J)::value;
+        const int32_t *src = rows + (int64_t)b * nrow * 64;
+#pragma unroll
+        for (int i = 0; i < NJ; i++) st_row[d][i] = src[off[i]];
+    };
+    int32_t S = NEGK;
+    const int32_t base64 = wid + 64 == n_walks ? 0 : NEGK;
+    auto step = [&](auto J, int32_t b) {
+        constexpr int d = decltype(J)::value;
+        const int p = b & 1;
+        if (wid == 0) blk_S[(int64_t)b * 64 + lane] = S;
+        int32_t part = NEGK;
+        const int32_t Sx = lane == n_walks ? 0 : S;
+#pragma unroll
+        for (int i = 0; i < NJ; i++) {
+            const int32_t base = i < 16 ? __builtin_amdgcn_readlane(Sx, wid + 4 * i) : base64;
+            const int32_t r = st_row[d][i] > NEGK / 2 ? st_row[d][i] : NEGK;
+            part = max(part, (int32_t)((uint32_t)base + (uint32_t)r));
+        }
+        s_part[p][wid][lane] = part;
+        issue(J, min(b + DEPTH, n_blk - 1));
+        __syncthreads();
+        const int32_t best = max(max(s_part[p][0][lane], s_part[p][1][lane]), max(s_part[p][2][lane], s_part[p][3][lane]));
+        S = (has_walk && best > NEGK / 2) ? best : NEGK;
+    };
+    using I0 = std::integral_constant<int, 0>; using I1 = std::integral_constant<int, 1>;
+    using I2 = std::integral_constant<int, 2>; using I3 = std::integral_constant<int, 3>;
+    if (n_blk <= 0) return;
+    issue(I0{}, 0);
+    issue(I1{}, min(1, n_blk - 1));
+    issue(I2{}, min(2, n_blk - 1));
+    issue(I3{}, min(3, n_blk - 1));
+    int32_t b = 0;
+    for (; b + DEPTH <= n_blk; b += DEPTH) {
+        step(I0{}, b);
+        step(I1{}, b + 1);
+        step(I2{}, b + 2);
+        step(I3{}, b + 3);
+    }
+    if (b < n_blk) step(I0{}, b);
+    if (b + 1 < n_blk) step(I1{}, b + 1);
+    if (b + 2 < n_blk) step(I2{}, b + 2);
+}
+
 __global__ void __launch_bounds__(256) phi_blk_check_kernel(const int32_t *__restrict__ keys, const int32_t *__restrict__ S, int32_t n_blk,
                                                             int32_t LS, int32_t n_walks, int32_t *__restrict__ bad)
 {
@@ -1141,6 +1198,10 @@
     hipLaunchKernelGGL(phi_seg_chain_kernel, dim3(1), dim3(256), 0, st, n_seg, G.n_walks, G.lane_stride, seg_row, seg_S);
     hipLaunchKernelGGL(phi_blk_chain_kernel<2>, dim3((unsigned)n_seg), dim3(256), 0, st, G, rows, rownew, rowdiag, blk_S, d_seg_lo, seg_row, seg_S);
 }
+void phi_launch_walk_chain(hipStream_t st, const int32_t *rows, int32_t n_blk, int32_t n_walks, int32_t *blk_S)
+{
+    if (n_blk > 0) hipLaunchKernelGGL(phi_walk_chain_kernel, dim3(1), dim3(256), 0, st, rows, n_blk, n_walks, blk_S);
+}
 void phi_launch_blk_check(hipStream_t st, const int32_t *keys, const int32_t *S, int32_t n_blk, int32_t LS, int32_t n_walks, int32_t *bad)
 {
     int64_t nb = ((int64_t)(n_blk - 1) * LS + 255) / 256;
diff --git a/phi_amd/csrc/phi_abi.hip b/phi_amd/csrc/phi_abi.hip
--- a/phi_amd/csrc/phi_abi.hip
+++ b/phi_amd/csrc/phi_abi.hip
@@ -131,7 +131,7 @@
     DevBuf *all[] = {&c->d_anchors, &c->d_cov_all, &c->d_cov_w, &c->d_slots, &c->d_slots2, &c->d_segs, &c->d_ctr, &c->d_vmax, &c->d_lane_walk, &c->d_walk_lane, &c->d_coff, &c->d_blk_ncls, &c->d_rownew, &c->d_blk_bad, &c->d_seg_lo, &c->d_seg_row, &c->d_seg_S, &c->wtext.d_text, &c->panel.d_full, &c->scout.d_scores, &c->d_sel_off, &c->d_sel_tri, &c->d_blk_lo, &c->d_blk_ev, &c->d_blk_S, &c->d_row_out, &c->d_rowend, &c->d_blk_keys, &c->d_blk_carry, &c->d_cov, &c->d_cov2, &c->d_stepdiff, &c->alt.hit, &c->hit_extra[0], &c->hit_extra[1], &c->alt.stripes, &c->spset.d_sp_cnt, &c->rlog.d_novlog, &c->rlog.d_novcnt, &c->rlog.d_ovlist, &c->d_vlen, &c->d_ent_cls, &c->d_cls_rep, &c->d_cls_left, &c->d_cls_mult, &c->d_cls_base, &c->d_cls_rec_off, &c->d_rec_cls, &c->d_rec_rel, &c->d_u_replist, &c->d_adj_off, &c->d_adj, &c->d_topo_rank, &c->d_cnt_edge, &c->d_walk_err, &c->d_sa_cnt, &c->d_sa_cur, &c->d_sa_off, &c->d_sa_idx, &c->d_seq, &c->d_seq_off, &c->d_walk_vtx, &c->d_walk_off, &c->d_topo, &c->d_in_off,
                      &c->d_in_src, &c->d_e_out, &c->d_st_rec, &c->d_st_mask, &c->d_in_packed, &c->d_word, &c->d_wwords, &c->d_wbad,
                      &c->d_wascii, &c->d_wstarts, &c->d_rec_hash, &c->d_rec_pos, &c->d_rec_slot,
-                     &c->d_rec_e0, &c->d_rec_e1, &c->d_u_keys, &c->d_u_rep, &c->d_u_uid, &c->d_rt, &c->d_kt, &c->d_in_s, &c->d_last_walk, &c->d_rowdiag, &c->d_wpre, &c->d_hit, &c->spset.d_sp_keys, &c->d_rbases,
+                     &c->d_rec_e0, &c->d_rec_e1, &c->d_u_keys, &c->d_u_rep, &c->d_u_uid, &c->d_rt, &c->d_kt, &c->d_in_s, &c->d_rep_mask, &c->d_rowdiag, &c->d_wpre, &c->d_hit, &c->spset.d_sp_keys, &c->d_rbases,
                      &c->d_roff, &c->rlog.d_roff_made, &c->d_peer_send, &c->spset.d_export, &c->d_scalars, &c->d_stripes, &c->d_blk_cnt,
                      &c->d_blk_off, &c->d_flags, &c->d_flags2, &c->d_list, &c->d_list2, &c->d_list3, &c->d_walk_last, &c->d_m_rec, &c->d_m_group,
                      &c->d_g_keys, &c->d_g_rep, &c->d_g_cnt, &c->d_slot_maxcnt, &c->d_slot_multi, &c->d_a_e1,
diff --git a/phi_amd/csrc/phi_ctx.h b/phi_amd/csrc/phi_ctx.h
--- a/phi_amd/csrc/phi_ctx.h
+++ b/phi_amd/csrc/phi_ctx.h
@@ -127,7 +127,7 @@
     hipEvent_t stage_ev[2] = {nullptr, nullptr};
     DevBuf d_wpre;
     DevBuf d_rowdiag;
-    DevBuf d_in_s, d_last_walk;
+    DevBuf d_in_s, d_rep_mask;
     int64_t n_unique = 0;
     uint64_t u_cap = 0;
     DevBuf d_hit;
diff --git a/phi_amd/csrc/phi_kernels.h b/phi_amd/csrc/phi_kernels.h
--- a/phi_amd/csrc/phi_kernels.h
+++ b/phi_amd/csrc/phi_kernels.h
@@ -252,11 +252,14 @@
 void phi_launch_dp_events(hipStream_t st, const PhiDpEventArgs &A);
 void phi_launch_dp_block_rows(hipStream_t st, const PhiDpEventArgs &A);
 void phi_launch_dp_block_paths(hipStream_t st, const PhiDpEventArgs &A);
+void phi_launch_walk_chain(hipStream_t st, const int32_t *rows, int32_t n_blk, int32_t n_walks, int32_t *blk_S);
 void phi_launch_anchor_prep(hipStream_t st, const uint32_t *tri, int64_t n, const int64_t *walk_off, int32_t n_walks, phi_ent_t *a_e1, uint8_t *a_span,
                             unsigned long long *walk_cnt, unsigned long long *out);
 void phi_launch_vertex_most(hipStream_t st, const int64_t *g_off, int64_t n_entries, const int32_t *walk_vtx, int32_t *vmax);
 void phi_launch_sum_i32(hipStream_t st, const int32_t *v, int64_t n, unsigned long long *out);
 void phi_launch_repeat_walk(hipStream_t st, const uint32_t *tri, int64_t lo, int64_t hi, int32_t walk, int32_t *last, uint8_t *flags);
+void phi_launch_repeat_group(hipStream_t st, const uint32_t *tri, int64_t lo, int64_t hi, const int64_t *walk_off, int32_t n_walks, int32_t first_walk,
+                             unsigned long long *mask, uint8_t *flags);
 void phi_launch_weights(hipStream_t st, const uint32_t *tri, int64_t n, const uint8_t *in_s, uint8_t *wgt);
 void phi_launch_path_cover(hipStream_t st, bool clear, const phi_ent_t *segs, int32_t n_seg, const int64_t *g_off, const uint32_t *tri, const uint8_t *wgt,
                            int32_t *cov_all, int32_t *cov_w, unsigned long long *ctr, uint32_t *twice, int64_t twice_cap);
diff --git a/phi_amd/csrc/phi_solve.hip b/phi_amd/csrc/phi_solve.hip
--- a/phi_amd/csrc/phi_solve.hip
+++ b/phi_amd/csrc/phi_solve.hip
@@ -116,8 +116,8 @@
         PHICHK(phi_dev_ensure(c, c->d_blk_ncls, nbk * 4));
         PHICHK(phi_dev_ensure(c, c->d_rownew, nbk * nrow * 4));
         PHICHK(phi_dev_ensure(c, c->d_rowdiag, nbk * 64 * 4));
-        PHICHK(phi_dev_ensure(c, c->d_blk_bad, 64));
-    }
+    }
+    PHICHK(phi_dev_ensure(c, c->d_blk_bad, 64));
     HIPCHK(hipMemcpyAsync(c->d_blk_lo.p, c->h_blk_lo.data(), (nbk + 1) * 4, hipMemcpyHostToDevice, c->stream));
     phi_launch_blk_ev(c->stream, c->d_blk_lo.as<int32_t>(), c->n_blk, c->d_ev_e.as<phi_ent_t>(), c->d_ev_off.as<int64_t>(), c->n_walks,
                       c->d_walk_vtx.as<int32_t>(), c->d_cvtx.as<int32_t>(), c->d_blk_ev.as<int32_t>());
@@ -131,6 +131,8 @@
 struct DpHost {
     std::vector<int32_t> ends, bstart, ent_u, ent_h;
     std::vector<int32_t> rows, rowend, S, keys, carry;
+    bool chain_pending = false;
+    int32_t chain_bad[2] = {0, 0};
 };
 
 struct DpOut {
@@ -254,7 +256,28 @@
     return PHI_OK;
 }
 
-static int dp_blocks_on_walk_lanes(phi_ctx *c, PhiDpEventArgs &A, DpHost &H, PhiStageTimer &tr, DpRetry *want)
+static int dp_blocks_on_walk_lanes(phi_ctx *c, PhiDpEventArgs &A, DpHost &H, PhiStageTimer &tr)
+{
+    const int32_t nb = c->n_blk;
+    dp_block_args(c, A);
+    phi_launch_dp_block_rows(c->stream, A);
+    if (tr.on) { (void)hipStreamSynchronize(c->stream); tr.lap("block rows"); }
+    phi_launch_walk_chain(c->stream, A.row_out, nb, c->n_walks, c->d_blk_S.as<int32_t>());
+    if (tr.on) { (void)hipStreamSynchronize(c->stream); tr.lap("block chain"); }
+    phi_launch_dp_block_paths(c->stream, A);
+    H.chain_bad[0] = 0; H.chain_bad[1] = INT32_MAX;
+    HIPCHK(hipMemcpyAsync(c->d_blk_bad.p, H.chain_bad, 8, hipMemcpyHostToDevice, c->stream));
+    phi_launch_blk_check(c->stream, A.blk_keys_out, A.blk_S, nb, 64, c->n_walks, c->d_blk_bad.as<int32_t>());
+    H.carry.resize((size_t)nb * 64);
+    HIPCHK(hipMemcpyAsync(H.chain_bad, c->d_blk_bad.p, 8, hipMemcpyDeviceToHost, c->stream));
+    HIPCHK(hipMemcpyAsync(H.carry.data(), A.blk_carry, H.carry.size() * 4, hipMemcpyDeviceToHost, c->stream));
+    if (tr.on) { (void)hipStreamSynchronize(c->stream); tr.lap("block paths + check"); }
+    H.chain_pending = true;
+    return PHI_OK;
+}
+
+static bool dp_chain_on_host() { const char *e = getenv("PHI_DP_CHAIN_HOST"); return e && atoi(e) != 0; }
+static int dp_blocks_on_walk_lanes_host_chain(phi_ctx *c, PhiDpEventArgs &A, DpHost &H, PhiStageTimer &tr, DpRetry *want)
 {
     const int32_t nb = c->n_blk, nwk = c->n_walks, nrow = nwk + 1;
     dp_block_args(c, A);
@@ -311,6 +334,13 @@
     if (events) HIPCHK(hipMemcpyAsync(&kerr, c->d_scalars.as<uint64_t>() + S_ERR, 4, hipMemcpyDeviceToHost, c->stream));
     HIPCHK(hipStreamSynchronize(c->stream));
     tr.lap("kernel");
+    if (H.chain_pending) {
+        H.chain_pending = false;
+        if (kerr & PHI_KERR_DP_QUEUE) return dp_blocks_fallback(c, kerr, PHI_KERR_DP_QUEUE, want);
+        if (H.chain_bad[0])
+            return phi_fail(c, PHI_ERR_DEVICE, "DP blocks: %d keys leaving blocks (first in block %d) differ from the chained rows (internal error)", H.chain_bad[0], H.chain_bad[1]);
+        return PHI_OK;
+    }
     if (kerr & PHI_KERR_DP_QUEUE) {
         kerr &= ~PHI_KERR_DP_QUEUE;
         HIPCHK(phi_copy_sync(c, c->d_scalars.as<uint64_t>() + S_ERR, &kerr, 4, hipMemcpyHostToDevice));
@@ -424,6 +454,7 @@
         case DP_DENSE: c->dp_events = false; break;
         }
         want = DP_DONE;
+        H.chain_pending = false;
         const bool events = c->dp_events;
         const DpOut O = dp_out(c);
         PhiStageTimer tr("dp run");
@@ -432,7 +463,8 @@
             PhiDpEventArgs A{};
             PHICHK(dp_event_records(c, O, A, tr));
             if (c->dp_blocks && c->dp_cls) PHICHK(dp_blocks_on_class_lanes(c, A, tr, &want));
-            else if (c->dp_blocks) PHICHK(dp_blocks_on_walk_lanes(c, A, H, tr, &want));
+            else if (c->dp_blocks && dp_chain_on_host()) PHICHK(dp_blocks_on_walk_lanes_host_chain(c, A, H, tr, &want));
+            else if (c->dp_blocks) PHICHK(dp_blocks_on_walk_lanes(c, A, H, tr));
             else phi_launch_dp_events(c->stream, A);
             if (want != DP_DONE) continue;
         } else {
@@ -497,8 +529,6 @@
     if (c->dp_alloc_future.valid()) PHICHK(c->dp_alloc_future.get());
     PHICHK(phi_sync_check(c));
     S.tm = PhiStageTimer("solve");
-    uint64_t sc[S_N];
-    HIPCHK(phi_copy_sync(c, sc, c->d_scalars.p, sizeof sc, hipMemcpyDeviceToHost));
     uint64_t n_distinct = 0;
     PHICHK(phi_spectrum_count(c, &n_distinct));
     S.tm.lap("read spectrum (set from the log)");
@@ -635,7 +665,9 @@
     if (!S.anchors_prepped)
         phi_launch_anchor_prep(c->stream, c->d_anchors.as<uint32_t>(), n_kept, c->d_walk_off.as<int64_t>(), nw, c->d_a_e1.as<phi_ent_t>(), c->d_g_span.as<uint8_t>(), d_ctr + 8, d_ctr);
     std::vector<unsigned long long> hc((size_t)nw + 8);
+    uint64_t sc[S_N];
     HIPCHK(hipMemcpyAsync(hc.data(), d_ctr, hc.size() * 8, hipMemcpyDeviceToHost, c->stream));
+    HIPCHK(hipMemcpyAsync(sc, c->d_scalars.p, sizeof sc, hipMemcpyDeviceToHost, c->stream));
     HIPCHK(hipStreamSynchronize(c->stream));
     if (hc[1] & 1) return phi_fail(c, PHI_ERR_DEVICE, "dp anchors not sorted by last entry (internal error)");
     if (hc[1] & 2)
@@ -646,9 +678,7 @@
     int64_t dev_min = (int64_t)1 << 16;
     if (const char *e = getenv("PHI_SOLVE_DEVICE")) dev_min = atoi(e) ? 0 : INT64_MAX;
     S.dev = hc[0] == 0 && n_kept >= dev_min && n_kept > 0;
-    uint64_t sc[S_N];
-    HIPCHK(phi_copy_sync(c, sc, c->d_scalars.p, sizeof sc, hipMemcpyDeviceToHost));
-    S.filtered = (int64_t)sc[S_FILTERED]; S.in_model = (int64_t)sc[S_INMODEL];
+    S.filtered =(int64_t)sc[S_FILTERED]; S.in_model = (int64_t)sc[S_INMODEL];
     return PHI_OK;
 }
 
@@ -727,14 +757,7 @@
 {
     phi_ctx *c = S.c;
     const int32_t nw = c->n_walks;
-    HIPCHK(hipStreamSynchronize(c->stream));
-    {
-        std::vector<phi_ent_t> last(nw);
-        for (int32_t h = 0; h < nw; h++) last[h] = (phi_ent_t)(c->h_walk_off[h + 1] - 1);
-        PHICHK(phi_dev_ensure(c, c->d_walk_last, (size_t)nw * 4));
-        PHICHK(phi_dev_ensure(c, c->d_list3, (size_t)nw * 4));
-        HIPCHK(phi_copy_sync(c, c->d_walk_last.p, last.data(), (size_t)nw * 4, hipMemcpyHostToDevice));
-    }
+    PHICHK(phi_dev_ensure(c, c->d_list3, (size_t)nw * 4));
     PHICHK(phi_dev_ensure(c, c->d_dmax, (size_t)c->n_entries * 4));
     PHICHK(phi_dev_ensure(c, c->d_bstart, (size_t)c->n_entries * 4));
     if (c->dp_events) {
@@ -800,13 +823,27 @@
     phi_ctx *c = S.c;
     const int64_t n_ids = c->n_unique;
     PHICHK(phi_dev_ensure(c, c->d_flags, (size_t)std::max<int64_t>(n_ids, 1)));
-    PHICHK(phi_dev_ensure(c, c->d_last_walk, (size_t)std::max<int64_t>(n_ids, 1) * 4));
-    HIPCHK(hipMemsetAsync(c->d_flags.p, 0, (size_t)std::max<int64_t>(n_ids, 1), c->stream));
-    HIPCHK(hipMemsetAsync(c->d_last_walk.p, 0xFF, (size_t)std::max<int64_t>(n_ids, 1) * 4, c->stream));
+    const size_t nid = (size_t)std::max<int64_t>(n_ids, 1);
+    PHICHK(phi_dev_ensure(c, c->d_rep_mask, nid * 8));
+    HIPCHK(hipMemsetAsync(c->d_flags.p, 0, nid, c->stream));
     int64_t lo = 0;
-    for (int32_t h = 0; h < c->n_walks; h++) {
-        phi_launch_repeat_walk(c->stream, c->d_anchors.as<uint32_t>(), lo, lo + c->h_n_anchors[h], h, c->d_last_walk.as<int32_t>(), c->d_flags.as<uint8_t>());
-        lo += c->h_n_anchors[h];
+    if (getenv("PHI_REPEAT_PER_WALK")) {
+        HIPCHK(hipMemsetAsync(c->d_rep_mask.p, 0xFF, nid * 4, c->stream));
+        for (int32_t h = 0; h < c->n_walks; h++) {
+            phi_launch_repeat_walk(c->stream, c->d_anchors.as<uint32_t>(), lo, lo + c->h_n_anchors[h], h, c->d_rep_mask.as<int32_t>(), c->d_flags.as<uint8_t>());
+            lo += c->h_n_anchors[h];
+        }
+    } else {
+        for (int32_t h0 = 0; h0 < c->n_walks; h0 += 64) {
+            int64_t hi = lo;
+            for (int32_t h = h0; h < std::min(h0 + 64, c->n_walks); h++) hi += c->h_n_anchors[h];
+            if (hi > lo) {
+                HIPCHK(hipMemsetAsync(c->d_rep_mask.p, 0, nid * 8, c->stream));
+                phi_launch_repeat_group(c->stream, c->d_anchors.as<uint32_t>(), lo, hi, c->d_walk_off.as<int64_t>(), c->n_walks, h0,
+                                        c->d_rep_mask.as<unsigned long long>(), c->d_flags.as<uint8_t>());
+            }
+            lo = hi;
+        }
     }
     if (lo != S.n_dp) return phi_fail(c, PHI_ERR_DEVICE, "anchors per walk do not add up (internal error)");
     int64_t n_rep = 0;
@@ -1138,3 +1175,14 @@
     PHICHK(search(S, &upper_bound));
     return decode(S, upper_bound);
 }
+
+int phi_chain_walk_rows(phi_ctx *c, const void *d_rows, int32_t n_blk, int32_t n_walks, void *d_S)
+{
+    if (!c) return PHI_ERR_INVALID;
+    if (n_blk < 1 || n_walks < 1 || n_walks > 64 || !d_rows || !d_S) return phi_fail(c, PHI_ERR_INVALID, "phi_chain_walk_rows: bad argument");
+    HIPCHK(hipSetDevice(c->device));
+    phi_launch_walk_chain(c->stream, static_cast<const int32_t *>(d_rows), n_blk, n_walks, static_cast<int32_t *>(d_S));
+    HIPCHK(hipGetLastError());
+    HIPCHK(hipStreamSynchronize(c->stream));
+    return PHI_OK;
+}
diff --git a/phi_amd/csrc/phi_wave.h b/phi_amd/csrc/phi_wave.h
--- a/phi_amd/csrc/phi_wave.h
+++ b/phi_amd/csrc/phi_wave.h
@@ -29,6 +29,21 @@
 }
 
 template <int NW, class T>
+__device__ __forceinline__ T phi_block_sum(T mine, T *s_w)
+{
+    const int lane = threadIdx.x & 63, wid = threadIdx.x >> 6;
+    T t = phi_wave_sum(mine);
+    if (lane == 0) s_w[wid] = t;
+    __syncthreads();
+    if (threadIdx.x == 0) {
+        t = 0;
+#pragma unroll
+        for (int i = 0; i < NW; i++) t += s_w[i];
+    }
+    return t;
+}
+
+template <int NW, class T>
 __device__ __forceinline__ T phi_block_excl_scan(T mine, T *s_w, T *total = nullptr)
 {
     const int lane = threadIdx.x & 63, wid = threadIdx.x >> 6;
diff --git a/phi_amd/csrc/set_graph.hip b/phi_amd/csrc/set_graph.hip
--- a/phi_amd/csrc/set_graph.hip
+++ b/phi_amd/csrc/set_graph.hip
@@ -279,6 +279,7 @@
     int32_t walk_err[4] = {0, 0, 0, 0};
     std::vector<int32_t> ends_own;
     const int32_t *walk_ends = nullptr;
+    std::vector<phi_ent_t> walk_last;
     PhiDpSteps steps;
     std::promise<int> edges_promise;
     std::future<int> edges_future = edges_promise.get_future();
@@ -343,6 +344,9 @@
         PHICHK(upload(c, c->d_seq_off, S.seq_off, (size_t)S.n_vtx + 1));
         if (!S.dev_walks) PHICHK(upload(c, c->d_walk_vtx, S.walk_vtx, (size_t)S.n_entries));
         PHICHK(upload(c, c->d_walk_off, S.walk_off, (size_t)S.n_walks + 1));
+        S.walk_last.resize((size_t)S.n_walks);
+        for (int32_t h = 0; h < S.n_walks; h++) S.walk_last[(size_t)h] = (phi_ent_t)(S.walk_off[h + 1] - 1);
+        PHICHK(upload(c, c->d_walk_last, S.walk_last.data(), (size_t)S.n_walks));
         PHICHK(upload(c, c->d_adj_off, S.adj_off, (size_t)S.n_vtx + 1));
         if (S.n_edges == 0) PHICHK(phi_dev_ensure(c, c->d_adj, 4));
         else PHICHK(upload(c, c->d_adj, S.adj, (size_t)S.n_edges));
diff --git a/phi_amd/csrc/solve_dev.hip b/phi_amd/csrc/solve_dev.hip
--- a/phi_amd/csrc/solve_dev.hip
+++ b/phi_amd/csrc/solve_dev.hip
@@ -1,6 +1,7 @@
 #include <hip/hip_runtime.h>
 #include "phi_dev.h"
 #include "phi_kernels.h"
+#include "phi_wave.h"
 
 static inline unsigned grid_for(int64_t n, int tpb)
 {
@@ -89,6 +90,23 @@
 {
     if (hi > lo) hipLaunchKernelGGL(phi_repeat_walk_kernel, dim3(grid_for(hi - lo, 256)), dim3(256), 0, st, tri, lo, hi, walk, last, flags);
 }
+__global__ void __launch_bounds__(256) phi_repeat_group_kernel(const uint32_t *__restrict__ tri, int64_t lo, int64_t hi, const int64_t *__restrict__ walk_off,
+                                                               int32_t n_walks, int32_t first_walk, unsigned long long *__restrict__ mask,
+                                                               uint8_t *__restrict__ flags)
+{
+    for (int64_t a = lo + (int64_t)blockIdx.x * blockDim.x + threadIdx.x; a < hi; a += (int64_t)gridDim.x * blockDim.x) {
+        const uint32_t id = tri[a * 3];
+        const int32_t h = walk_of_entry(walk_off, n_walks, (int64_t)tri[a * 3 + 1]) - first_walk;
+        if ((uint32_t)h >= 64u) continue;
+        const unsigned long long bit = 1ull << h;
+        if (atomicOr(&mask[id], bit) & bit) flags[id] = 1;
+    }
+}
+void phi_launch_repeat_group(hipStream_t st, const uint32_t *tri, int64_t lo, int64_t hi, const int64_t *walk_off, int32_t n_walks, int32_t first_walk,
+                             unsigned long long *mask, uint8_t *flags)
+{
+    if (hi > lo) hipLaunchKernelGGL(phi_repeat_group_kernel, dim3(grid_for(hi - lo, 256)), dim3(256), 0, st, tri, lo, hi, walk_off, n_walks, first_walk, mask, flags);
+}
 __global__ void __launch_bounds__(256) phi_weights_kernel(const uint32_t *__restrict__ tri, int64_t n, const uint8_t *__restrict__ in_s, uint8_t *__restrict__ wgt)
 {
     GRID_STRIDE(a, n) wgt[a] = in_s[tri[a * 3]] ? 0 : 1;
@@ -104,6 +122,8 @@
                                                              int32_t *__restrict__ cov_all, int32_t *__restrict__ cov_w,
                                                              unsigned long long *__restrict__ ctr, uint32_t *__restrict__ twice, int64_t twice_cap)
 {
+    __shared__ int s_w[4];
+    int n_w = 0, n_first = 0;
     for (int32_t q = blockIdx.y; q < n_seg; q += gridDim.y) {
         const phi_ent_t es = segs[2 * q], ee = segs[2 * q + 1];
         const int64_t lo = g_off[es], hi = g_off[(int64_t)ee + 1];
@@ -119,13 +139,21 @@
             const bool first = in && atomicAdd(&cov_all[s], 1) == 0;
             const bool w = in && wgt[a] != 0;
             const int32_t before = w ? atomicAdd(&cov_w[s], 1) : -1;
-            wave_count(w, &ctr[0]);
-            wave_count(first, &ctr[1]);
+            n_w += w;
+            n_first += first;
             if (before == 1) {
                 const unsigned long long at = atomicAdd(&ctr[2], 1ull);
                 if ((int64_t)at < twice_cap) twice[at] = s;
             }
         }
+    }
+    if (CLEAR) return;
+    n_w = phi_block_sum<4>(n_w, s_w);
+    __syncthreads();
+    n_first = phi_block_sum<4>(n_first, s_w);
+    if (threadIdx.x == 0) {
+        if (n_w) atomicAdd(&ctr[0], (unsigned long long)n_w);
+        if (n_first) atomicAdd(&ctr[1], (unsigned long long)n_first);
     }
 }
 void phi_launch_path_cover(hipStream_t st, bool clear, const phi_ent_t *segs, int32_t n_seg, const int64_t *g_off, const uint32_t *tri, const uint8_t *wgt,
diff --git a/phi_amd/csrc/table.hip b/phi_amd/csrc/table.hip
--- a/phi_amd/csrc/table.hip
+++ b/phi_amd/csrc/table.hip
@@ -361,16 +361,26 @@
 __global__ void __launch_bounds__(256) phi_count_flags_kernel(const uint8_t *__restrict__ flags, int64_t n,
                                                               unsigned long long *__restrict__ n_out)
 {
+    __shared__ int s_w[4];
+    const int64_t tid = (int64_t)blockIdx.x * blockDim.x + threadIdx.x, nthr = (int64_t)gridDim.x * blockDim.x;
+    const int64_t mis = (int64_t)((16 - ((uintptr_t)flags & 15)) & 15), head = mis < n ? mis : n;
+    const int64_t n16 = (n - head) >> 4, tail = head + (n16 << 4);
+    const uint4 *__restrict__ wide = reinterpret_cast<const uint4 *>(flags + head);
     int cnt = 0;
-    for (int64_t i = (int64_t)blockIdx.x * blockDim.x + threadIdx.x; i < n; i += (int64_t)gridDim.x * blockDim.x)
-        cnt += flags[i] != 0;
-    cnt = phi_wave_sum(cnt);
-    if ((threadIdx.x & 63) == 0 && cnt) atomicAdd(n_out, (unsigned long long)cnt);
+    auto nonzero_bytes = [](uint32_t w) { return __popc((((w & 0x7F7F7F7Fu) + 0x7F7F7F7Fu) | w) & 0x80808080u); };
+    for (int64_t i = tid; i < n16; i += nthr) {
+        const uint4 v = wide[i];
+        cnt += nonzero_bytes(v.x) + nonzero_bytes(v.y) + nonzero_bytes(v.z) + nonzero_bytes(v.w);
+    }
+    if (tid < head) cnt += flags[tid] != 0;
+    if (tail + tid < n && tid < 16) cnt += flags[tail + tid] != 0;
+    cnt = phi_block_sum<4>(cnt, s_w);
+    if (threadIdx.x == 0 && cnt) atomicAdd(n_out, (unsigned long long)cnt);
 }
 
 void phi_launch_count_flags(hipStream_t st, const uint8_t *flags, int64_t n, unsigned long long *n_out)
 {
-    if (n > 0) hipLaunchKernelGGL(phi_count_flags_kernel, dim3(grid_for(n, 256)), dim3(256), 0, st, flags, n, n_out);
+    if (n > 0) hipLaunchKernelGGL(phi_count_flags_kernel, dim3((unsigned)((n + 4095) / 4096 < 512 ? (n + 4095) / 4096 : 512)), dim3(256), 0, st, flags, n, n_out);
 }
 
 __global__ void __launch_bounds__(256) phi_spectrum_export_kernel(const uint64_t *__restrict__ sp_keys, int64_t cap,
```

Result: slower. 478.0 (-1.0%).
